# LordLiang/DrawingSpinUp

Measured on AMD Instinct MI355X. Metric: drawings/sec end-to-end (512x512, 6 views, 24 frames), higher is better.
Workload: dtype f16 (diffusion) / f16 table + f32 MLP (NSR) / f32 (stage-1 deformable convolutions, IS-Net, contour) / f32 with bf16 x 3 products (stage-2 convolutions; the reference: cuDNN TF32)

## Files before the change

### drawingspinup_amd/_lib.py

```python
import ctypes as C
import os

import torch

_HERE = os.path.dirname(os.path.abspath(__file__))
LIB_PATH = os.environ.get("DSU_HIP_LIB") or os.path.join(_HERE, "libdsu_hip.so")
MAX_LEVELS = 16
ABI_VERSION = 3

c_i32, c_i64, c_u32, c_f32, c_vp = C.c_int32, C.c_int64, C.c_uint32, C.c_float, C.c_void_p


class HashGridCfg(C.Structure):
    _fields_ = [("n_levels", c_u32), ("n_features", c_u32), ("log2_hashmap_size", c_u32),
                ("base_resolution", c_u32), ("per_level_scale", C.c_double)]


class HashGridLevels(C.Structure):
    _fields_ = [("offsets", c_u32 * (MAX_LEVELS + 1)), ("resolution", c_u32 * MAX_LEVELS),
                ("scale", c_f32 * MAX_LEVELS), ("hashed", c_u32 * MAX_LEVELS)]


class SdfMlp(C.Structure):
    _fields_ = [("w0", c_vp), ("b0", c_vp), ("w1", c_vp), ("b1", c_vp)]


class TexMlp(C.Structure):
    _fields_ = [("w0", c_vp), ("b0", c_vp), ("w1", c_vp), ("b1", c_vp), ("w2", c_vp),
                ("b2", c_vp)]


class PartialReduce(C.Structure):
    _fields_ = [("partials", c_vp), ("map", c_vp), ("base", c_vp), ("nblocks", c_i32),
                ("stride", c_i32), ("n", c_i32)]


class OccRefreshArgs(C.Structure):
    _fields_ = [("occs", c_vp), ("binary", c_vp), ("res", c_i32), ("all_cells", c_i32),
                ("aabb", C.POINTER(c_f32)), ("seed", C.c_uint64), ("step", c_i64),
                ("grid", C.POINTER(HashGridCfg)), ("table_img", c_vp), ("mlp", C.POINTER(SdfMlp)),
                ("inv_s", c_vp), ("radius", c_f32), ("render_step_size", c_f32),
                ("ema_decay", c_f32), ("occ_thre", c_f32), ("active_levels", c_u32),
                ("inj_count", c_i32), ("inj_cells", c_vp), ("inj_rand", c_vp), ("thre_out", c_vp),
                ("workspace", c_vp), ("workspace_bytes", c_i64), ("cells_out", c_vp),
                ("rand_out", c_vp)]


class RenderTexture(C.Structure):
    _fields_ = [("uv", c_vp), ("texels", c_vp), ("tex_size", c_i32), ("filter", c_i32)]


class NormCfg(C.Structure):
    _fields_ = [("batch", c_i32), ("channels", c_i32), ("hw", c_i32), ("instance", c_i32),
                ("act", c_i32), ("stat_updates", c_i32), ("eps", c_f32), ("momentum", c_f32)]


class RayLossCfg(C.Structure):
    _fields_ = [("rgb_p_ratio", C.c_double), ("normal_p_ratio", C.c_double),
                ("mask_p_ratio", C.c_double), ("lambda_rgb_mse", c_f32),
                ("lambda_rgb_l1", c_f32), ("lambda_normal", c_f32), ("lambda_mask", c_f32),
                ("geo_aware", c_i32), ("reserved", c_i32)]


P = c_vp
class AdamwTensor(C.Structure):
    _fields_ = [("p", C.c_void_p), ("g", C.c_void_p), ("m", C.c_void_p), ("v", C.c_void_p),
                ("n", C.c_int64), ("lr", C.c_float), ("bias_correction1", C.c_float),
                ("bias_correction2_sqrt", C.c_float), ("reserved", C.c_float)]


ADAMW_MAX_TENSORS = 24


class NsrDriverCfg(C.Structure):
    _fields_ = [("grid", HashGridCfg), ("radius", c_f32), ("render_step_size", c_f32),
                ("cap_points", c_i32), ("cap_rays", c_i32), ("n_random", c_i32),
                ("sort_bits", c_i32), ("dynamic_ray_sampling", c_i32),
                ("train_num_samples", c_i32),
                ("c2w", c_vp), ("origins", c_vp), ("directions", c_vp), ("images", c_vp),
                ("normals", c_vp), ("masks", c_vp), ("view_weights", c_vp),
                ("V", c_i32), ("H", c_i32), ("W", c_i32), ("image_channels", c_i32),
                ("w0_v", c_vp), ("w0_g", c_vp), ("b0", c_vp), ("w1_v", c_vp), ("w1_g", c_vp),
                ("b1", c_vp), ("tex", c_vp * 6), ("variance", c_vp),
                ("ray_loss", RayLossCfg),
                ("lambda_eikonal", c_f32), ("lambda_sparsity", c_f32), ("sparsity_scale", c_f32),
                ("lambda_smooth", c_f32),
                ("beta1", c_f32), ("beta2", c_f32), ("adam_eps", c_f32), ("weight_decay", c_f32),
                ("seed", C.c_uint64), ("workspace", c_vp), ("workspace_bytes", c_i64)]


class NsrStepArgs(C.Structure):
    _fields_ = [("step", c_i64), ("n_rays", c_i32), ("prefetch_next", c_i32),
                ("active_levels", c_u32), ("eps", c_f32), ("cos_anneal_ratio", c_f32),
                ("lr_geometry", c_f32), ("lr_texture", c_f32), ("lr_variance", c_f32),
                ("adam_step", c_i32), ("randomized", c_i32), ("refresh_effective", c_i32),
                ("occ_res", c_i32), ("occ_binary", c_vp), ("table_img", c_vp),
                ("table_grad", c_vp),
                ("inj_index", c_vp), ("inj_x", c_vp), ("inj_y", c_vp), ("inj_jitter", c_vp),
                ("inj_pts_random", c_vp), ("inj_perturb", c_vp),
                ("inj_rays", c_vp), ("inj_rgb", c_vp), ("inj_normal", c_vp), ("inj_mask", c_vp),
                ("inj_cosines", c_vp), ("inj_view_weights", c_vp),
                ("table_p", c_vp), ("table_m", c_vp), ("table_v", c_vp), ("table_n", c_i64),
                ("table_lr", c_f32), ("table_bc1", c_f32), ("table_bc2_sqrt", c_f32),
                ("table_eps", c_f32), ("table_wd", c_f32),
                ("out_n_samples", c_i32), ("out_max_count", c_i32), ("out_next_n_rays", c_i32),
                ("terms_out", c_vp)]


_PROTOS = {
    "dsu_abi_version": [],
    "dsu_hashgrid_make_levels": [C.POINTER(HashGridCfg), C.POINTER(HashGridLevels)],
    "dsu_hashgrid_encode_fwd": [C.POINTER(HashGridCfg), P, P, c_i64, c_u32, P, P],
    "dsu_hashgrid_encode_bwd": [C.POINTER(HashGridCfg), P, P, c_i64, c_u32, P, P],
    "dsu_sdf_fwd": [C.POINTER(HashGridCfg), P, C.POINTER(SdfMlp), P, c_i64, c_f32, c_u32, c_u32,
                    P, P],
    "dsu_sdf_fd_bwd_workspace_bytes": [C.POINTER(HashGridCfg), c_i64],
    "dsu_sdf_fd_enc_cache_bytes": [c_i64, c_u32],
    "dsu_sdf_fd_fwd_sorted": [C.POINTER(HashGridCfg), P, C.POINTER(SdfMlp), P, P, c_i64, c_f32,
                              c_f32, c_u32, P, P, P, P, P, P],
    "dsu_sdf_fd_bwd_sorted": [C.POINTER(HashGridCfg), P, C.POINTER(SdfMlp), P, P, c_i64, c_f32,
                              c_f32, c_u32, P, P, P, P, P, P, P, P, P, P, c_i64, P, P],
    "dsu_sdf_fd_bwd_sorted_fold": [C.POINTER(HashGridCfg), P, C.POINTER(SdfMlp), P, P, c_i64, c_f32,
                                   c_f32, c_u32, P, P, P, P, P, P, P, P, P, P, c_i64, P, P,
                                   C.POINTER(PartialReduce), P],
    "dsu_texture_partial_map": [P],
    "dsu_texture_bwd_shaded_partials_m": [C.POINTER(TexMlp), P, P, P, P, P, c_i64, c_i64, P, P, P, P, c_i64,
                                          C.POINTER(PartialReduce), P],
    "dsu_texture_bwd_shaded_partials_live": [C.POINTER(TexMlp), P, P, P, P, P, c_i64, c_i64, P, P, P, P, P,
                                             c_i64, C.POINTER(PartialReduce), P],
    "dsu_texture_live_partition": [P, c_i64, c_i32, c_i32, P],
    "dsu_texture_fwd_shaded_m": [C.POINTER(TexMlp), P, P, c_i64, P, P, P, P],
    "dsu_occgrid_refresh_workspace_bytes": [c_i32],
    "dsu_occgrid_refresh": [C.POINTER(OccRefreshArgs), P],
    "dsu_nsr_driver_occ_refresh": [P, C.POINTER(OccRefreshArgs), P],
    "dsu_inpaint_telea_u8c3": [P, P, c_i32, c_i32, c_i32, P],
    "dsu_table_adamw": [P, P, P, P, P, c_i64, c_f32, c_f32, c_f32, c_f32, c_f32, c_f32, c_f32, P],
    "dsu_table_decay": [P, P, c_i64, c_f32, P],
    "dsu_adamw_multi": [P, c_i32, c_f32, c_f32, c_f32, c_f32, P],
    "dsu_smooth_iterate": [P, c_i64, P, P, C.c_double, c_i32, P, P, P],
    "dsu_smooth_energy": [P, c_i64, P, P, P, P],
    "dsu_smooth_energy_partials": [],
    "dsu_smooth_brick_side": [],
    "dsu_smooth_bricks_flags": [P, c_i32, c_i32, c_i32, P, P],
    "dsu_smooth_bricks_gather": [P, P, c_i32, c_i32, c_i32, P, P, c_i32, P, c_i32, P, P, P, P, P, P, P],
    "dsu_smooth_bricks_iterate": [P, P, c_i32, P, P, P, c_i32, C.c_double, c_i32, c_i32, P, P, P],
    "dsu_smooth_bricks_energy": [P, P, c_i32, P, P, P],
    "dsu_smooth_bricks_scatter": [P, P, P, c_i32, c_i32, c_i32, c_i32, P, P],
    "dsu_set_onewave_grid_cap": [c_i32],
    "dsu_set_scatter_grid_cap": [c_i32],
    "dsu_set_nsr_side_stream_priority": [c_i32],
    "dsu_set_nsr_side_stream_pooling": [c_i32],
    "dsu_volume_band_distance_workspace_bytes": [c_i32, c_i32, c_i32],
    "dsu_volume_band_distance": [P, c_i32, c_i32, c_i32, c_i32, P, P, P, P, P, c_i64, P],
    "dsu_mc_cube_index": [P, c_i32, c_i32, c_i32, C.c_double, P, P],
    "dsu_sdf_fwd_lattice": [P, P, P, P, c_i32, c_i32, c_i32, P, P, c_f32, c_u32, P, P],
    "dsu_zgrid_count": [P, c_i64, c_f32, c_f32, c_f32, c_i32, P, P],
    "dsu_zgrid_fill": [P, c_i64, c_f32, c_f32, c_f32, c_i32, P, P, P, P],
    "dsu_zray_cast": [P, P, c_i64, c_f32, c_f32, c_f32, c_i32, P, P, P, c_i64, c_i32, P, P, P, P, P,
                      P, P],
    "dsu_raster_mask": [P, c_i64, c_f32, c_i32, P, P],
    "dsu_erode_ellipse_u8": [P, c_i32, c_i32, c_i32, P, P],
    "dsu_mesh_render_ortho_workspace_bytes": [c_i32, c_i32],
    "dsu_mesh_render_ortho": [c_i32, P, P, P, P, C.POINTER(RenderTexture), c_i32, c_i64, c_i64, C.c_double,
                              C.c_double, C.c_double, c_i32, c_i32, P, c_i64, P, c_i64, P, P, P, P, P, P, P],
    "dsu_mip_levels": [c_i32],
    "dsu_mip_pyramid_texels": [c_i32],
    "dsu_mip_workspace_bytes": [c_i32],
    "dsu_mip_pyramid_build": [P, P, c_i32, c_i32, P, P, c_i64, P],
    "dsu_mip_sample_host": [P, c_i32, P, P, P, c_i64, P],
    "dsu_pos_edge_u8": [P, c_i32, c_i32, c_i32, P, P],
    "dsu_uv_face_labels": [P, P, c_i64, c_i64, P, P, P, P],
    "dsu_uv_components": [P, P, c_i64, P, P, c_i32, c_i32, C.POINTER(c_i32), P],
    "dsu_uv_bake_workspace_bytes": [c_i32],
    "dsu_uv_bake": [c_i32, P, P, P, P, c_i64, c_i64, c_i32, P, c_i64, P, c_i64, P, P, P, P],
    "dsu_uv_dilate": [P, P, c_i32, P, P, P],
    "dsu_uv_project": [P, P, P, c_i64, c_i64, c_i32, P, P, c_f32, c_f32, c_f32, c_i32, P, P, P, P, P, P, c_i32,
                       C.c_double, P, P, P],
    "dsu_uv_field_points": [P, P, P, c_i64, c_i64, c_i32, P, P, c_i64, c_i32, P, P, P],
    "dsu_uv_field_resolve": [P, P, P, c_i64, c_i32, c_i32, P, P],
    "dsu_uv_field_points_host": [P, P, P, c_i64, c_i64, c_i32, P, P, c_i64, c_i32, P, P],
    "dsu_uv_field_resolve_host": [P, P, P, c_i64, c_i32, c_i32, P],
    "dsu_uv_seam_gather": [P, P, P, c_i64, c_i64, c_i64, c_i32, P, P, P, P, P, P, P],
    "dsu_uv_seam_apply": [P, P, P, c_i64, c_i64, c_i64, c_i32, P, P, P, P, P, P, P],
    "dsu_uv_seam_gather_host": [P, P, P, c_i64, c_i64, c_i64, c_i32, P, P, P, P, P, P],
    "dsu_uv_seam_apply_host": [P, P, P, c_i64, c_i64, c_i64, c_i32, P, P, P, P, P, P],
    "dsu_bone_visibility_workspace_bytes": [c_i32, c_i32, c_i32],
    "dsu_bone_visibility": [c_i32, P, P, P, c_i64, c_i64, c_i32, P, C.c_double, C.c_double, C.c_double,
                            C.c_double, c_i32, c_i32, c_i32, P, c_i64, P, c_i64, P, P, P],
    "dsu_spd_cg_block_workspace_bytes": [c_i64, c_i32],
    "dsu_spd_cg_block": [P, P, P, c_i64, c_i64, c_i32, P, P, C.c_double, c_i32, P, c_i64,
                         C.POINTER(c_i32), C.POINTER(C.c_double), P],
    "dsu_skin_lbs": [P, P, P, P, c_i64, c_i32, c_i32, c_i32, P, P],
    "dsu_skin_dqs": [P, P, P, P, c_i64, c_i32, c_i32, c_i32, P, P],
    "dsu_skin_dqs_host": [P, P, P, P, c_i64, c_i32, c_i32, c_i32, P],
    "dsu_corrective_smooth_workspace_bytes": [c_i64, c_i32],
    "dsu_corrective_bind": [P, P, P, c_i64, P, P, c_i64, P, c_i64, c_i64, C.c_double, c_i32, P, c_i64, P, P, P],
    "dsu_corrective_smooth": [P, P, P, P, c_i64, P, P, c_i64, P, c_i64, P, P, c_i64, c_i32, C.c_double, c_i32,
                              P, c_i64, P, P],
    "dsu_corrective_bind_host": [P, P, P, c_i64, P, P, c_i64, P, c_i64, c_i64, C.c_double, c_i32, P, c_i64, P, P],
    "dsu_corrective_smooth_host": [P, P, P, P, c_i64, P, P, c_i64, P, c_i64, P, P, c_i64, c_i32, C.c_double,
                                   c_i32, P, c_i64, P],
    "dsu_point_bin_count": [P, c_i64, c_f32, c_f32, c_f32, c_i32, P, P],
    "dsu_point_bin_fill": [P, c_i64, c_f32, c_f32, c_f32, c_i32, P, P, P, P],
    "dsu_knn8_blend": [P, c_i64, P, P, c_i64, c_f32, c_f32, c_f32, c_i32, P, P, P, P],
    "dsu_umbrella_implicit_solve": [P, P, c_i64, C.c_double, P, P, P, c_i32, P],
    "dsu_mesh_decimate_quadric": [P, c_i64, P, c_i64, c_i64, C.c_double, c_i32, P, P, P, P],
    "dsu_mesh_decimate_quadric_q": [P, c_i64, P, c_i64, c_i64, C.c_double, c_i32, P, P, P, P, P],
    "dsu_mesh_decimate_parallel_workspace_bytes": [c_i64, c_i64],
    "dsu_mesh_decimate_parallel": [P, c_i64, P, c_i64, c_i64, c_i64, C.c_double, c_i32, c_i32, P, P, P, P,
                                   c_i64, P],
    "dsu_distance_transform_l2_5x5": [P, c_i32, c_i32, P],
    "dsu_skeletonize_lee_2d": [P, c_i32, c_i32, P],
    "dsu_nsr_draws": [C.c_uint64, c_i64, c_i32, c_i32, c_i32, c_i32, P, P, P, P, c_i32, P, P, P],
    "dsu_nsr_driver_workspace_bytes": [C.POINTER(NsrDriverCfg)],
    "dsu_nsr_driver_create": [C.POINTER(NsrDriverCfg), C.POINTER(c_vp)],
    "dsu_nsr_driver_destroy": [c_vp],
    "dsu_nsr_driver_step": [c_vp, C.POINTER(NsrStepArgs), P],
    "dsu_nsr_driver_terms": [c_vp],
    "dsu_nsr_driver_adam_moments": [c_vp, c_i32],
    "dsu_nsr_driver_live_halves": [c_vp, c_i64],
    "dsu_nsr_driver_timing": [c_vp, c_i32],
    "dsu_nsr_driver_timing_read": [c_vp, c_i32, C.POINTER(c_i64), C.POINTER(C.c_double),
                                   C.POINTER(C.c_double)],
    "dsu_nsr_driver_timing_flops": [c_vp, c_i32, C.POINTER(C.c_double)],
    "dsu_spatial_sort": [P, c_i64, c_f32, c_i32, P, P, P, c_i64, P],
    "dsu_spatial_sort_workspace_bytes": [c_i64, c_i32],
    "dsu_ray_aabb": [P, P, c_i64, P, P, c_f32, P, P, P],
    "dsu_ray_march_scratch": [P, P, P, P, c_i64, P, P, c_i32, c_f32, c_i32, P, P, P, P],
    "dsu_ray_compact": [P, P, c_i32, P, P, c_i64, P, P, P, P],
    "dsu_ray_compact_points": [P, P, c_i32, P, P, c_i64, P, P, P, P, P, P],
    "dsu_ray_compact_points_cap": [P, P, c_i32, P, P, c_i64, P, P, P, P, P, c_i64, P],
    "dsu_points_tail": [P, c_i64, P, P, P, c_i64, c_f32, P],
    "dsu_spatial_sort_dev": [P, c_i64, P, c_i64, c_f32, c_i32, P, P, P, c_i64, P],
    "dsu_ray_offsets": [P, c_i64, P, P, P],
    "dsu_ortho_ray_batch": [P, P, P, c_i64, P, P, P, P, c_i32, P, P, P, c_i32, c_i32, P, P, P, P, P,
                            P, P],
    "dsu_ortho_ray_batch_split": [P, P, P, c_i64, P, P, P, P, c_i32, P, P, P, c_i32, c_i32, P, P, P, P, P,
                            P, P, P, P],
    "dsu_ray_losses": [P, P, P, P, P, P, c_i32, C.POINTER(RayLossCfg), P, P, P],
    "dsu_sample_losses": [P, P, c_i64, c_i64, c_f32, c_f32, c_f32, c_f32, c_i32, P, P, P, P],
    "dsu_texture_fwd": [C.POINTER(TexMlp), P, c_i64, P, P],
    "dsu_texture_bwd_workspace_bytes": [c_i64],
    "dsu_texture_bwd": [C.POINTER(TexMlp), P, P, P, c_i64, P, P, P, P, P, P, P, P, c_i64, P],
    "dsu_texture_bwd_shaded": [C.POINTER(TexMlp), P, P, P, P, P, c_i64, c_i64, P, P, P, P, P, P, P, P,
                               P, c_i64, P],
    "dsu_weights_from_alpha_fwd": [P, P, P, c_i64, P, P],
    "dsu_weights_from_alpha_bwd": [P, P, P, P, P, c_i64, P, P],
    "dsu_accumulate_fwd": [P, P, c_i32, P, P, c_i64, P, P],
    "dsu_neus_composite_fwd": [P, P, P, P, P, P, P, P, c_i64, P, c_f32, P, P, P, P],
    "dsu_neus_composite_bwd": [P, P, P, P, P, P, P, P, c_i64, P, c_f32, P, P, P, P, P, P, P,
                               P, P],
    "dsu_neus_composite_bwd_live": [P, P, P, P, P, P, P, P, c_i64, P, c_f32, P, P, P, P, P, P, P,
                                    P, P, P],
    "dsu_shade_prep_fwd": [P, P, c_i64, P, P, P],
    "dsu_shade_prep_bwd": [P, P, P, c_i64, P, P, P],
    "dsu_occgrid_ema": [P, P, P, c_i64, c_f32, P, P],
    "dsu_occgrid_binarize": [P, c_i64, c_f32, P, P],
    "dsu_ric_offsets": [c_i32, c_i32, P, P],
    "dsu_deform_conv3x3_fwd": [P, P, c_i64, P, c_i32, c_i32, c_i32, c_i32, c_i32, c_i32, P, P,
                               c_i32, P, P, P],
    "dsu_mv_attention_fwd": [P, P, P, P, P, c_i32, c_i32, c_i32, c_i32, c_i32, c_i32,
                             C.POINTER(c_i64), C.POINTER(c_i64), C.POINTER(c_i64),
                             C.POINTER(c_i64), c_f32, P],
    "dsu_conv2d_nhwc_f16_fwd_fx": [P, P, P, c_i32, c_i32, c_i32, c_i32, c_i32, c_i32, c_i32, c_i32,
                                   c_i32, P, P, P, c_i32, P, c_i64, P, c_i64, P],
    "dsu_gemm_f16_fwd_fx": [P, P, P, c_i64, c_i32, c_i32, P, P, c_i32, c_i32, P, c_i64, P, c_i64, P],
    "dsu_conv2d_nhwc_f16_split_k": [c_i32] * 9,
    "dsu_conv2d_nhwc_f16_workspace_bytes": [c_i32] * 9,
    "dsu_gemm_f16_split_k": [c_i64, c_i32, c_i32],
    "dsu_gemm_f16_workspace_bytes": [c_i64, c_i32, c_i32],
    "dsu_gemm_geglu_fwd": [P, P, P, c_i64, c_i32, c_i32, P, P],
    "dsu_groupnorm_nhwc_f16": [P, P, P, c_i32, c_i32, c_i32, c_i32, c_f32, c_i32, P, P, P],
    "dsu_layernorm_f16": [P, P, P, c_i64, c_i32, c_f32, P, P],
    "dsu_geglu_f16": [P, c_i64, c_i32, P, P],
    "dsu_cfg_model_input": [P, P, c_i32, c_i64, P, P],
    "dsu_ddim_cfg_step": [P, P, P, c_i64, c_f32, c_f32, c_f32, c_f32, c_f32, P, P],
    "dsu_deform_tap_table_bytes": [c_i32, c_i32],
    "dsu_deform_tap_table": [P, c_i32, c_i32, P, P],
    "dsu_conv2d_wgrad_workspace_bytes": [c_i32, c_i32, c_i32, c_i32, c_i32, c_i32, c_i32],
    "dsu_conv2d_wgrad": [P, P, P, c_i32, c_i32, c_i32, c_i32, c_i32, c_i32, c_i32, c_i32, P, P,
                         c_i32, P],
    "dsu_deform_conv3x3_dgrad_gather": [P, P, P, P, c_i64, c_i32, P, P],
    "dsu_norm_train_fwd": [C.POINTER(NormCfg), P, P, P, P, P, P, P, P, P],
    "dsu_norm_train_bwd": [C.POINTER(NormCfg), P, P, P, P, P, P, P, P, P, P],
    "dsu_channel_sum": [P, c_i32, c_i32, c_i32, P, P],
    "dsu_act_fwd": [P, P, c_i64, c_i32, P],
    "dsu_act_bwd": [P, P, P, c_i64, c_i32, P],
    "dsu_maxpool2_fwd": [P, P, c_i64, c_i32, c_i32, P],
    "dsu_maxpool2_bwd": [P, P, P, c_i64, c_i32, c_i32, P],
    "dsu_upsample2_fwd": [P, P, c_i64, c_i32, c_i32, P],
    "dsu_upsample2_bwd": [P, P, c_i64, c_i32, c_i32, P],
    "dsu_pair_loss": [P, P, c_f32, c_i64, c_i32, c_f32, P, P, P],
    "dsu_conv_x3_packed_elems": [c_i32, c_i32, c_i32],
    "dsu_conv_x3_pack_weights": [P, c_i32, c_i32, c_i32, P, P, P],
    "dsu_deform_conv3x3_fwd_x3": [P, P, c_i64, P, P, c_i32, c_i32, c_i32, c_i32, c_i32, c_i32,
                                  P, P, c_i32, P, P, P],
    "dsu_conv2d_fwd_x3": [P, P, P, P, c_i32, c_i32, c_i32, c_i32, c_i32, c_i32, c_i32, c_i32,
                          c_i32, P, P, c_i32, P, P, P],
    "dsu_conv_f32p_pack_weights": [P, c_i32, c_i32, c_i32, P, P],
    "dsu_deform_conv3x3_fwd_f32p": [P, P, c_i64, P, c_i32, c_i32, c_i32, c_i32, c_i32, c_i32,
                                    P, P, c_i32, P, P, P],
    "dsu_conv2d_fwd_f32p": [P, P, P, c_i32, c_i32, c_i32, c_i32, c_i32, c_i32, c_i32, c_i32, c_i32,
                            P, P, c_i32, P, P, P],
    "dsu_conv2d_fwd": [P, P, P, c_i32, c_i32, c_i32, c_i32, c_i32, c_i32, c_i32, c_i32, c_i32,
                       P, P, c_i32, P, P, P],
}

_RESTYPES = {"dsu_nsr_driver_destroy": None, "dsu_nsr_driver_terms": c_vp,
             "dsu_nsr_driver_adam_moments": c_vp, "dsu_nsr_driver_live_halves": c_vp,
             "dsu_conv_x3_packed_elems": C.c_int64, "dsu_mip_pyramid_texels": C.c_int64}

_lib = None


class DsuError(RuntimeError):
    pass


def lib():
    global _lib
    if _lib is None:
        if not os.path.exists(LIB_PATH):
            raise DsuError(
                f"{LIB_PATH} is missing: the HIP extension is not built "
                "(run `python -m drawingspinup_amd.build`). There is no CPU fallback.")
        h = C.CDLL(LIB_PATH)
        h.dsu_strerror.restype = C.c_char_p
        h.dsu_strerror.argtypes = [C.c_int]
        if h.dsu_abi_version() != ABI_VERSION:
            raise DsuError(f"{LIB_PATH} has ABI version {h.dsu_abi_version()}, this package binds version "
                           f"{ABI_VERSION}: rebuild it (`python -m drawingspinup_amd.build`).")
        for name, args in _PROTOS.items():
            fn = getattr(h, name)
            fn.restype = _RESTYPES.get(name, C.c_int64 if name.endswith("_bytes") else C.c_int)
            fn.argtypes = args
        _lib = h
# ... 40 lines not shown
```

### drawingspinup_amd/csrc/capi.hip

```cpp
#include "common.h"
#include <math.h>

int dsu_mv_cfg_model_input_launch(const void* latents, const void* image_latents, int32_t B,
                                  int64_t row_elems, void* out, void* stream);
int dsu_mv_ddim_cfg_step_launch(const void* noise_pred, const void* latents,
                                const void* variance_noise, int64_t n, float guidance_scale,
                                float sqrt_a_t, float sqrt_1m_a_t, float sqrt_a_prev, double dir,
                                float std_dev, void* out, void* stream);

extern "C" {

const char* dsu_strerror(int code) {
  switch (code) {
    case DSU_OK: return "ok";
    case DSU_EINVAL: return "invalid argument";
    case DSU_ELAUNCH: return "HIP launch/runtime error";
    case DSU_EUNSUP: return "configuration not supported by the gfx950 kernels";
    default: return "unknown dsu error";
  }
}

int dsu_abi_version(void) { return 3; }

int32_t dsu_onewave_grid_cap_value = 0;
int32_t dsu_scatter_grid_cap_value = 0;
int dsu_set_scatter_grid_cap(int32_t workgroups) {
  if (workgroups < 0 || workgroups > 4096) return DSU_EINVAL;
  dsu_scatter_grid_cap_value = workgroups;
  return DSU_OK;
}
int32_t dsu_nsr_side_priority_value = 1;
int dsu_set_nsr_side_stream_priority(int32_t level) {
  if (level < 0 || level > 2) return DSU_EINVAL;
  dsu_nsr_side_priority_value = level;
  return DSU_OK;
}
int32_t dsu_nsr_side_pool_value = 0;
int dsu_set_nsr_side_stream_pooling(int32_t on) {
  if (on < 0 || on > 1) return DSU_EINVAL;
  dsu_nsr_side_pool_value = on;
  return DSU_OK;
}
int dsu_set_onewave_grid_cap(int32_t cus) {
  if (cus < 0 || cus > 256) return DSU_EINVAL;
  dsu_onewave_grid_cap_value = cus;
  return DSU_OK;
}

int dsu_cfg_model_input(const void* latents, const void* image_latents, int32_t B,
                        int64_t row_elems, void* out, void* stream) {
  if (!latents || !image_latents || !out || B < 0 || row_elems < 0) return DSU_EINVAL;
  if (out == latents || out == image_latents) return DSU_EINVAL;
  if (B == 0 || row_elems == 0) return DSU_OK;
  if (row_elems > INT64_MAX / 4 / B) return DSU_EINVAL;
  return dsu_mv_cfg_model_input_launch(latents, image_latents, B, row_elems, out, stream);
}

int dsu_ddim_cfg_step(const void* noise_pred, const void* latents, const void* variance_noise,
                      int64_t n, float guidance_scale, float sqrt_a_t, float sqrt_1m_a_t,
                      float sqrt_a_prev, float std_dev, void* out, void* stream) {
  if (!noise_pred || !latents || !out || n < 0 || n > INT64_MAX / 2) return DSU_EINVAL;
  if (out == noise_pred || out == latents || out == variance_noise) return DSU_EINVAL;
  if (!(sqrt_a_t > 0.0f) || !(std_dev >= 0.0f) || !isfinite(guidance_scale) ||
      !isfinite(sqrt_1m_a_t) || !isfinite(sqrt_a_prev))
    return DSU_EINVAL;
  const double rad = 1.0 - (double)sqrt_a_prev * sqrt_a_prev - (double)std_dev * std_dev;
  if (!(rad >= -1e-6)) return DSU_EINVAL;
  if (n == 0) return DSU_OK;
  return dsu_mv_ddim_cfg_step_launch(noise_pred, latents, variance_noise, n, guidance_scale,
                                     sqrt_a_t, sqrt_1m_a_t, sqrt_a_prev,
                                     sqrt(rad > 0.0 ? rad : 0.0), std_dev, out, stream);
}

}
```

### drawingspinup_amd/csrc/nsr_driver.hip

```cpp
#include "common.h"
#include "adamw_dev.h"

#include <math.h>
#include <string.h>

#include <mutex>
#include <vector>

namespace {

constexpr int N_GEO = 64 * 23 + 64 + 13 * 64 + 13;
constexpr int N_TEX = 64 * 16 + 64 + 64 * 64 + 64 + 3 * 64 + 3;
constexpr int N_SMALL = (64 * 23 + 64 + 64) + (13 * 64 + 13 + 13) + N_TEX + 1;

__device__ __forceinline__ uint4 philox(uint4 c, uint2 k) {
#pragma unroll
  for (int i = 0; i < 10; ++i) {
    const uint32_t hi0 = __umulhi(0xD2511F53u, c.x), lo0 = 0xD2511F53u * c.x;
    const uint32_t hi1 = __umulhi(0xCD9E8D57u, c.z), lo1 = 0xCD9E8D57u * c.z;
    c = make_uint4(hi1 ^ c.y ^ k.x, lo1, hi0 ^ c.w ^ k.y, lo0);
    k.x += 0x9E3779B9u;
    k.y += 0xBB67AE85u;
  }
  return c;
// ... 583 lines not shown
    ~Guard() {
      if (!ok) for (int k = 0; k < 3; ++k) d->pf_valid[k] = false;
    }
  } guard{d};
  if (d->initialised && a->step != d->last_step + 1) {
    DSU_HIP(hipMemsetAsync(terms + 4, 0, 3 * sizeof(float), s));
    DSU_HIP(hipMemsetAsync(L.live_halves[a->step & 1], 0, (size_t)L.live_words * sizeof(uint32_t), s));
  }
  if (!d->initialised) {
    DSU_HIP(hipMemsetAsync(L.live_halves[0], 0, 2 * (size_t)L.live_words * sizeof(uint32_t), s));
    DSU_HIP(hipMemsetAsync(L.g_geo, 0, (N_GEO + N_TEX + 1) * sizeof(float), s));
    DSU_HIP(hipMemsetAsync(L.adam_m, 0, N_SMALL * sizeof(float), s));
    DSU_HIP(hipMemsetAsync(L.adam_v, 0, N_SMALL * sizeof(float), s));
    DSU_HIP(hipMemsetAsync(L.terms, 0, 16 * sizeof(float), s));
  }
  if (!d->initialised || a->refresh_effective) {
    DSU_TRY(launch_small_update(d, a, 0, s));
    d->initialised = true;
  }
  const bool injected = a->inj_index || a->inj_x || a->inj_y || a->inj_jitter || a->inj_pts_random ||
                        a->inj_perturb || a->inj_rays;
  if (d->pf_valid[p] && d->pf_step[p] == a->step && d->pf_rays[p] == a->n_rays && !injected &&
      d->pf_randomized[p] == a->randomized && d->pf_occ[p] == a->occ_binary &&
      d->pf_occ_res[p] == a->occ_res) {
    DSU_HIP(hipEventSynchronize(d->ready[p]));
  } else {
    DSU_HIP(hipStreamSynchronize(d->side));
    for (int k = 0; k < 3; ++k) d->pf_valid[k] = false;
    DSU_TRY(enqueue_samples(d, p, a->step, a->n_rays, *a, injected, s));
    DSU_HIP(hipStreamSynchronize(s));
  }
  d->pf_valid[p] = false;
  const int32_t total = d->host_stats[2 * p], cmax = d->host_stats[2 * p + 1];
  a->out_n_samples = total;
  a->out_max_count = cmax;
  if (total > c.cap_points || cmax > d->rowcap) return DSU_EUNSUP;
  const int64_t n_s = total, n_r = c.n_random, n_all = n_s + 2 * n_r;
  int32_t next_rays = a->n_rays;
  if (c.dynamic_ray_sampling && n_s > 0) {
    const int tr = (int)((double)a->n_rays * ((double)c.train_num_samples / (double)n_s));
    const int nr2 = (int)((double)a->n_rays * 0.9 + (double)tr * 0.1);
    next_rays = nr2 < c.cap_rays ? nr2 : c.cap_rays;
    if (next_rays < 1) next_rays = 1;
  }
  a->out_next_n_rays = next_rays;
  if (a->prefetch_next) {
    const int q = (int)((a->step + 1) % 3);
    DSU_HIP(hipStreamWaitEvent(d->side, d->gate, 0));
    dsu_nsr_step_args na = *a;
    na.inj_index = na.inj_x = na.inj_y = nullptr;
    na.inj_jitter = na.inj_pts_random = na.inj_perturb = nullptr;
    na.inj_rays = nullptr;
    DSU_TRY(enqueue_march(d, q, a->step + 1, next_rays, na, false, d->side));
    d->pf_step[q] = a->step + 1;
    d->pf_rays[q] = next_rays;
    d->pf_randomized[q] = a->randomized;
    d->pf_occ[q] = a->occ_binary;
    d->pf_occ_res[q] = a->occ_res;
    DSU_TRY(enqueue_pack(d, q, next_rays, na, false, d->side));
    DSU_HIP(hipEventRecord(d->ready[q], d->side));
    d->pf_valid[q] = true;
  }

  const float* pts = c.sort_bits ? f.sorted : f.points;
  const int32_t* perm = c.sort_bits ? f.perm : nullptr;
  dsu_sdf_mlp mlp{L.w0_eff, c.b0, L.w1_eff, c.b1};
  const double alg_bytes = (double)n_all * (7.0 * a->active_levels * 8 * 4 + 12 + 72);
  const double l0 = 7.0 * 64 * (3 + 2 * a->active_levels), l1 = 64.0 * (13 + 6);
  const double fwd_flops = (double)n_all * 2.0 * (l0 + l1), bwd_flops = (double)n_all * 2.0 * 3.0 * (l0 + l1);
  DSU_TRY(mark(d, 0, s));
  DSU_TRY(dsu_sdf_fd_fwd_sorted(&c.grid, a->table_img, &mlp, pts, perm, n_all, c.radius, a->eps,
                                a->active_levels, L.a_sdf, L.a_grad, L.a_feat, nullptr, L.enc_cache, s));
  DSU_TRY(mark(d, 0, s));
  if (d->timing) { d->work[0] += alg_bytes; d->flops[0] += fwd_flops; }
  if (n_s > 0) {
    dsu_tex_mlp tex{c.tex[0], c.tex[1], c.tex[2], c.tex[3], c.tex[4], c.tex[5]};
    DSU_TRY(dsu_texture_fwd_shaded_m(&tex, L.a_feat, L.a_grad, n_s, L.normal, L.rgb, L.tex_mask, s));
    DSU_TRY(dsu_neus_composite_fwd(L.a_sdf, L.normal, L.rgb, f.rays_d, f.t_starts, f.t_ends,
                                   f.offsets, f.counts, a->n_rays, L.inv_s, a->cos_anneal_ratio,
                                   L.alpha, L.w, L.comp, s));
  } else {
    DSU_HIP(hipMemsetAsync(L.comp, 0, (size_t)a->n_rays * 8 * sizeof(float), s));
  }
  DSU_TRY(dsu_ray_losses(L.comp, f.rgb, f.normal, f.mask, f.cosines, f.vw, a->n_rays, &c.ray_loss,
                         terms, L.d_comp, s));
  dsu_partial_reduce tex_red{};
  bool have_tex_red = false;
  if (n_s > 0) {
    uint32_t* live = L.live_halves[a->step & 1];
    DSU_TRY(dsu_neus_composite_bwd_live(L.a_sdf, L.normal, L.rgb, f.rays_d, f.t_starts, f.t_ends,
                                        f.offsets, f.counts, a->n_rays, L.inv_s, a->cos_anneal_ratio,
                                        L.alpha, L.w, L.d_comp, nullptr, L.d_sdf_all, L.d_normal, L.d_rgb,
                                        L.d_inv, live, s));
    dsu_tex_mlp tex{c.tex[0], c.tex[1], c.tex[2], c.tex[3], c.tex[4], c.tex[5]};
    DSU_TRY(dsu_texture_bwd_shaded_partials_live(&tex, L.a_feat, L.a_grad, L.rgb, L.d_rgb, L.d_normal, n_s,
                                                 2 * n_r, L.d_grad_all, L.d_feat_all, L.tex_mask, live,
                                                 L.tex_ws, L.tex_ws_bytes, &tex_red, s));
    tex_red.map = L.tex_map;
    tex_red.base = L.g_tex;
    have_tex_red = true;
  } else {
    DSU_HIP(hipMemsetAsync(L.d_feat_all, 0, (size_t)(2 * n_r) * 13 * sizeof(float), s));
  }
  DSU_TRY(dsu_sample_losses(L.a_sdf, L.a_grad, n_s, n_r, c.lambda_eikonal, c.lambda_sparsity,
                            c.sparsity_scale, c.lambda_smooth, 1 | 2, L.d_sdf_all, L.d_grad_all,
                            terms + 4, s));
  float* gg = L.g_geo;
  DSU_TRY(mark(d, 1, s));
  DSU_TRY(dsu_sdf_fd_bwd_sorted_fold(&c.grid, a->table_img, &mlp, pts, perm, n_all, c.radius, a->eps,
                                     a->active_levels, L.d_sdf_all, L.d_grad_all, L.d_feat_all, nullptr,
                                     a->table_grad, gg, gg + 64 * 23, gg + 64 * 23 + 64,
                                     gg + 64 * 23 + 64 + 13 * 64, L.sdf_ws, L.sdf_ws_bytes,
                                     L.enc_cache, d->gate, have_tex_red ? &tex_red : nullptr, s));
  DSU_TRY(mark(d, 1, s));
  if (d->timing) { d->work[1] += alg_bytes; d->flops[1] += bwd_flops; }
  DSU_TRY(launch_small_update(d, a, 1, s));
  d->last_step = a->step;
  guard.ok = true;
  return DSU_OK;
}

int dsu_nsr_driver_occ_refresh(dsu_nsr_driver* d, const dsu_occgrid_refresh_args* args,
                               void* main_stream) {
  if (!d || !args) return DSU_EINVAL;
  if (!d->initialised) return DSU_EUNSUP;
  const dsu_nsr_driver_cfg& c = d->cfg;
  DSU_HIP(hipStreamSynchronize(d->side));
  for (int k = 0; k < 3; ++k) d->pf_valid[k] = false;
  dsu_occgrid_refresh_args a = *args;
  const dsu_sdf_mlp mlp{d->L.w0_eff, c.b0, d->L.w1_eff, c.b1};
  a.grid = &c.grid;
  a.mlp = &mlp;
  a.inv_s = d->L.inv_s;
  a.aabb = d->aabb;
  a.seed = c.seed;
  a.radius = c.radius;
  a.render_step_size = c.render_step_size;
  return dsu_occgrid_refresh(&a, main_stream);
}

int dsu_nsr_driver_timing(dsu_nsr_driver* d, int32_t enable) {
  if (!d) return DSU_EINVAL;
  for (int f = 0; f < 2; ++f) {
    for (hipEvent_t e : d->ev[f]) (void)hipEventDestroy(e);
    d->ev[f].clear();
    d->work[f] = 0.0;
    d->flops[f] = 0.0;
  }
  d->timing_stride = enable > 0 ? enable : 0;
  d->timing = false;
  return DSU_OK;
}

int dsu_nsr_driver_timing_read(dsu_nsr_driver* d, int32_t family, int64_t* launches,
                               double* total_ms, double* alg_bytes) {
  if (!d || family < 0 || family > 1 || !launches || !total_ms || !alg_bytes) return DSU_EINVAL;
  const std::vector<hipEvent_t>& ev = d->ev[family];
  double ms = 0.0;
  const size_t pairs = ev.size() / 2;
  for (size_t i = 0; i < pairs; ++i) {
    DSU_HIP(hipEventSynchronize(ev[2 * i + 1]));
    float t = 0.0f;
    DSU_HIP(hipEventElapsedTime(&t, ev[2 * i], ev[2 * i + 1]));
    ms += t;
  }
  *launches = (int64_t)pairs;
  *total_ms = ms;
  *alg_bytes = d->work[family];
  return DSU_OK;
}

int dsu_nsr_driver_timing_flops(dsu_nsr_driver* d, int32_t family, double* mlp_flops) {
  if (!d || family < 0 || family > 1 || !mlp_flops) return DSU_EINVAL;
  *mlp_flops = d->flops[family];
  return DSU_OK;
}

}
```

### drawingspinup_amd/csrc/nsr_render.hip

```cpp
#include "common.h"
#include <math.h>
#include <stdlib.h>

namespace {

struct Aabb {
  float mn[3];
  float mx[3];
  float inv_ext[3];
  int pow2;
};

template <bool P2>
__device__ __forceinline__ float div_ext(float x, const Aabb& a, int d) {
  return P2 ? x * a.inv_ext[d] : x / (a.mx[d] - a.mn[d]);
}
template <bool P2>
__device__ __forceinline__ float div_res(float x, const Aabb& a, int res, float inv_res) {
  return P2 ? x * inv_res : x / (float)res;
}

__device__ __forceinline__ float signf1(float x) { return copysignf(1.0f, x); }

template <bool P2>
// ... 326 lines not shown
  return v;
}
__device__ __forceinline__ float wave_sum(float v) {
#pragma unroll
  for (int o = 32; o > 0; o >>= 1) v += __shfl_xor(v, o);
  return v;
}
__device__ __forceinline__ float sigmoidf_(float x) { return 1.0f / (1.0f + expf(-x)); }

struct AlphaOut {
  float alpha, pc, nc, iter_cos, true_cos;
  bool clipped;
};

__device__ __forceinline__ AlphaOut neus_alpha(float sdf, const float n[3], const float d[3],
                                               float dist, float inv_s, float car) {
  AlphaOut a;
  a.true_cos = d[0] * n[0] + d[1] * n[1] + d[2] * n[2];
  a.iter_cos = -(fmaxf(-a.true_cos * 0.5f + 0.5f, 0.0f) * (1.0f - car) +
                 fmaxf(-a.true_cos, 0.0f) * car);
  const float nx = sdf + a.iter_cos * dist * 0.5f, pv = sdf - a.iter_cos * dist * 0.5f;
  a.pc = sigmoidf_(pv * inv_s);
  a.nc = sigmoidf_(nx * inv_s);
  const float raw = ((a.pc - a.nc) + 1e-5f) / (a.pc + 1e-5f);
  a.clipped = raw < 0.0f || raw > 1.0f;
  a.alpha = fminf(fmaxf(raw, 0.0f), 1.0f);
  return a;
}

__global__ __launch_bounds__(256) void composite_fwd_kernel(
    const float* __restrict__ sdf, const float* __restrict__ normal,
    const float* __restrict__ rgb, const float* __restrict__ rays_d,
    const float* __restrict__ t_starts, const float* __restrict__ t_ends,
    const int32_t* __restrict__ off, const int32_t* __restrict__ cnt, int64_t n_rays,
    const float* __restrict__ inv_s_p, float car, float* __restrict__ alpha_o,
    float* __restrict__ w_o, float* __restrict__ comp) {
  const float inv_s = fminf(fmaxf(*inv_s_p, 1e-6f), 1e6f);
  const int lane = threadIdx.x & 63;
  const int64_t r = blockIdx.x * 4 + (threadIdx.x >> 6);
  if (r >= n_rays) return;
  const int64_t b = off[r];
  const int c = cnt[r];
  const float d[3] = {rays_d[r * 3], rays_d[r * 3 + 1], rays_d[r * 3 + 2]};
  float T = 1.0f;
  float acc[8];
#pragma unroll
  for (int k = 0; k < 8; ++k) acc[k] = 0.0f;
  for (int j0 = 0; j0 < c; j0 += 64) {
    const int j = j0 + lane;
    const bool v = j < c;
    float al = 0.0f, mid = 0.0f, n[3] = {0.f, 0.f, 0.f}, col[3] = {0.f, 0.f, 0.f};
    if (v) {
      const int64_t i = b + j;
      n[0] = normal[i * 3]; n[1] = normal[i * 3 + 1]; n[2] = normal[i * 3 + 2];
      const float ts = t_starts[i], te = t_ends[i];
      mid = (ts + te) / 2.0f;
      al = neus_alpha(sdf[i], n, d, te - ts, inv_s, car).alpha;
      col[0] = rgb[i * 3]; col[1] = rgb[i * 3 + 1]; col[2] = rgb[i * 3 + 2];
    }
    const float incl = wave_incl_scan_mul(1.0f - al, lane);
    float excl = __shfl_up(incl, 1);
    if (lane == 0) excl = 1.0f;
    const float w = al * (T * excl);
    T *= __shfl(incl, 63);
    if (v) {
      alpha_o[b + j] = al;
      w_o[b + j] = w;
      acc[0] += w;
      acc[1] += w * mid;
      acc[2] += w * col[0]; acc[3] += w * col[1]; acc[4] += w * col[2];
      acc[5] += w * n[0]; acc[6] += w * n[1]; acc[7] += w * n[2];
    }
  }
#pragma unroll
  for (int k = 0; k < 8; ++k) acc[k] = wave_sum(acc[k]);
  if (lane < 8) {
    float v = acc[0];
#pragma unroll
    for (int k = 1; k < 8; ++k) v = lane == k ? acc[k] : v;
    comp[r * 8 + lane] = v;
  }
}

__global__ __launch_bounds__(256) void composite_bwd_kernel(
    const float* __restrict__ sdf, const float* __restrict__ normal,
    const float* __restrict__ rgb, const float* __restrict__ rays_d,
    const float* __restrict__ t_starts, const float* __restrict__ t_ends,
    const int32_t* __restrict__ off, const int32_t* __restrict__ cnt, int64_t n_rays,
    const float* __restrict__ inv_s_p, float car, const float* __restrict__ alpha_s,
    const float* __restrict__ w_s,
    const float* __restrict__ d_comp, const float* __restrict__ d_w_extra,
    float* __restrict__ d_sdf, float* __restrict__ d_normal, float* __restrict__ d_rgb,
    float* __restrict__ d_inv_s, uint32_t* __restrict__ live_halves) {
  const float inv_raw = *inv_s_p;
  const float inv_s = fminf(fmaxf(inv_raw, 1e-6f), 1e6f);
  const bool inv_pass = inv_raw >= 1e-6f && inv_raw <= 1e6f;
  const int lane = threadIdx.x & 63;
  const int64_t r = blockIdx.x * 4 + (threadIdx.x >> 6);
  float dinv = 0.0f;
  if (r < n_rays) {
    const int64_t b = off[r];
    const int c = cnt[r];
    const float d[3] = {rays_d[r * 3], rays_d[r * 3 + 1], rays_d[r * 3 + 2]};
    float dc[8];
#pragma unroll
    for (int k = 0; k < 8; ++k) dc[k] = d_comp[r * 8 + k];
    float total = 0.0f;
    for (int j = lane; j < c; j += 64) {
      const int64_t i = b + j;
      const float mid = (t_starts[i] + t_ends[i]) / 2.0f;
      float gw = dc[0] + dc[1] * mid + dc[2] * rgb[i * 3] + dc[3] * rgb[i * 3 + 1] +
                 dc[4] * rgb[i * 3 + 2] + dc[5] * normal[i * 3] + dc[6] * normal[i * 3 + 1] +
                 dc[7] * normal[i * 3 + 2];
      if (d_w_extra) gw += d_w_extra[i];
      total += gw * w_s[i];
    }
    total = wave_sum(total);
    float T = 1.0f, done = 0.0f;
    for (int j0 = 0; j0 < c; j0 += 64) {
      const int j = j0 + lane;
      const bool v = j < c;
      float al = 0.0f, w = 0.0f, gw = 0.0f, n[3] = {0.f, 0.f, 0.f};
      int64_t i = b + (v ? j : 0);
      float mid = 0.0f, dist = 0.0f, s = 0.0f;
      if (v) {
        al = alpha_s[i]; w = w_s[i];
        n[0] = normal[i * 3]; n[1] = normal[i * 3 + 1]; n[2] = normal[i * 3 + 2];
        const float ts = t_starts[i], te = t_ends[i];
        mid = (ts + te) / 2.0f; dist = te - ts; s = sdf[i];
        gw = dc[0] + dc[1] * mid + dc[2] * rgb[i * 3] + dc[3] * rgb[i * 3 + 1] +
             dc[4] * rgb[i * 3 + 2] + dc[5] * n[0] + dc[6] * n[1] + dc[7] * n[2];
        if (d_w_extra) gw += d_w_extra[i];
      }
      const float incl = wave_incl_scan_mul(1.0f - al, lane);
      float excl = __shfl_up(incl, 1);
      if (lane == 0) excl = 1.0f;
      const float Tj = T * excl;
      const float gww = gw * w;
      const float pin = wave_incl_scan_add(gww, lane);
      const float before = done + (pin - gww);
      T *= __shfl(incl, 63);
      done += __shfl(pin, 63);
      bool lit = false;
      if (v) {
        const float accum = total - before;
        const float galpha = (gw * Tj - accum) / fmaxf(1.0f - al, 1e-10f);
        const AlphaOut a = neus_alpha(s, n, d, dist, inv_s, car);
        float dsdf = 0.0f, dn[3] = {0.f, 0.f, 0.f};
        if (!a.clipped) {
          const float den = a.pc + 1e-5f;
          const float d_pc = galpha * (1.0f / den - ((a.pc - a.nc) + 1e-5f) / (den * den));
          const float d_nc = -galpha / den;
          const float d_pv = d_pc * a.pc * (1.0f - a.pc);
          const float d_nx = d_nc * a.nc * (1.0f - a.nc);
          const float pv = s - a.iter_cos * dist * 0.5f, nx = s + a.iter_cos * dist * 0.5f;
          dinv += d_pv * pv + d_nx * nx;
          dsdf = (d_pv + d_nx) * inv_s;
          const float d_ic = (d_nx - d_pv) * inv_s * dist * 0.5f;
          float d_tc = 0.0f;
          if (-a.true_cos * 0.5f + 0.5f > 0.0f) d_tc += 0.5f * (1.0f - car);
          if (-a.true_cos > 0.0f) d_tc += car;
          d_tc *= d_ic;
          dn[0] = d_tc * d[0]; dn[1] = d_tc * d[1]; dn[2] = d_tc * d[2];
        }
        d_sdf[i] = dsdf;
        d_normal[i * 3] = dn[0] + w * dc[5];
        d_normal[i * 3 + 1] = dn[1] + w * dc[6];
        d_normal[i * 3 + 2] = dn[2] + w * dc[7];
        const float c0 = w * dc[2], c1 = w * dc[3], c2 = w * dc[4];
        d_rgb[i * 3] = c0; d_rgb[i * 3 + 1] = c1; d_rgb[i * 3 + 2] = c2;
        lit = c0 != 0.0f || c1 != 0.0f || c2 != 0.0f;
      }
      if (live_halves) {
        const uint64_t m = __ballot(lit);
        if (v && (lane == 0 || (i & 31) == 0)) {
          const int span = 32 - (int)(i & 31);
          const uint64_t part = span >= 64 - lane ? ~0ull << lane : ((1ull << span) - 1ull) << lane;
          if (m & part) atomicOr(&live_halves[i >> 10], 1u << ((i >> 5) & 31));
        }
      }
    }
  }
  dinv = wave_sum(dinv);
  if (lane == 0 && dinv != 0.0f && inv_pass) unsafeAtomicAdd(d_inv_s, dinv);
}

__global__ void shade_prep_fwd_kernel(const float* __restrict__ grad,
                                      const float* __restrict__ feat, int64_t n,
                                      float* __restrict__ normal, float* __restrict__ tex_in) {
  const int64_t i = blockIdx.x * (int64_t)blockDim.x + threadIdx.x;
  if (i >= n) return;
  const float g0 = grad[i * 3], g1 = grad[i * 3 + 1], g2 = grad[i * 3 + 2];
  const float inv = 1.0f / fmaxf(sqrtf(g0 * g0 + g1 * g1 + g2 * g2), 1e-12f);
  const float n0 = g0 * inv, n1 = g1 * inv, n2 = g2 * inv;
  normal[i * 3] = n0; normal[i * 3 + 1] = n1; normal[i * 3 + 2] = n2;
#pragma unroll
  for (int k = 0; k < 13; ++k) tex_in[i * 16 + k] = feat[i * 13 + k];
  tex_in[i * 16 + 13] = n0; tex_in[i * 16 + 14] = n1; tex_in[i * 16 + 15] = n2;
}

__global__ void shade_prep_bwd_kernel(const float* __restrict__ grad,
                                      const float* __restrict__ d_normal,
                                      const float* __restrict__ d_tex_in, int64_t n,
                                      int64_t tail, float* __restrict__ d_grad,
                                      float* __restrict__ d_feat) {
  const int64_t i = blockIdx.x * (int64_t)blockDim.x + threadIdx.x;
  if (i >= n) {
    if (i < n + tail)
      for (int k = 0; k < 13; ++k) d_feat[i * 13 + k] = 0.0f;
    return;
  }
  const float g0 = grad[i * 3], g1 = grad[i * 3 + 1], g2 = grad[i * 3 + 2];
  const float len = sqrtf(g0 * g0 + g1 * g1 + g2 * g2);
  const float inv = 1.0f / fmaxf(len, 1e-12f);
  const float n0 = g0 * inv, n1 = g1 * inv, n2 = g2 * inv;
  float d0 = d_tex_in[i * 16 + 13], d1 = d_tex_in[i * 16 + 14], d2 = d_tex_in[i * 16 + 15];
  if (d_normal) { d0 += d_normal[i * 3]; d1 += d_normal[i * 3 + 1]; d2 += d_normal[i * 3 + 2]; }
  const float dot = n0 * d0 + n1 * d1 + n2 * d2;
  const bool ok = len > 1e-12f;
  d_grad[i * 3] = ok ? (d0 - n0 * dot) * inv : d0 * inv;
  d_grad[i * 3 + 1] = ok ? (d1 - n1 * dot) * inv : d1 * inv;
  d_grad[i * 3 + 2] = ok ? (d2 - n2 * dot) * inv : d2 * inv;
#pragma unroll
  for (int k = 0; k < 13; ++k) d_feat[i * 13 + k] = d_tex_in[i * 16 + k];
}

Aabb make_aabb(const float* a6, int res = 1) {
  Aabb a;
  a.pow2 = (res > 0 && (res & (res - 1)) == 0) ? 1 : 0;
  for (int d = 0; d < 3; ++d) {
    a.mn[d] = a6[d];
    a.mx[d] = a6[3 + d];
    const float ext = a.mx[d] - a.mn[d];
    a.inv_ext[d] = 1.0f / ext;
    if (!is_pow2f(ext)) a.pow2 = 0;
  }
  return a;
}

}

#define DSU_MARCH_ONE(O, P, nr, st, ...)                                                    \
  ray_march_kernel<O, P><<<dsu_blocks_for(nr, 256 / MARCH_G), 256, 0,                       \
                           (hipStream_t)st>>>(__VA_ARGS__)
#define DSU_LAUNCH_MARCH(nr, st, box, occp, ...)                                      \
  do {                                                                                \
    const bool p2_ = (box).pow2 != 0;                                                 \
    if (!(occp)) {                                                                    \
// ... 80 lines not shown
  if (n_rays < 0 || (n_rays && (!offsets || !counts))) return DSU_EINVAL;
  if (n_rays == 0) return DSU_OK;
  weights_fwd_kernel<<<dsu_blocks_for(n_rays, 64), 64, 0, (hipStream_t)stream>>>(
      alpha, offsets, counts, n_rays, weights);
  DSU_CHECK_LAUNCH();
  return DSU_OK;
}

int dsu_weights_from_alpha_bwd(const float* alpha, const float* weights, const float* d_weights,
                               const int32_t* offsets, const int32_t* counts, int64_t n_rays,
                               float* d_alpha, void* stream) {
  if (n_rays < 0 || (n_rays && (!offsets || !counts))) return DSU_EINVAL;
  if (n_rays == 0) return DSU_OK;
  weights_bwd_kernel<<<dsu_blocks_for(n_rays, 64), 64, 0, (hipStream_t)stream>>>(
      alpha, weights, d_weights, offsets, counts, n_rays, d_alpha);
  DSU_CHECK_LAUNCH();
  return DSU_OK;
}

int dsu_accumulate_fwd(const float* weights, const float* values, int32_t channels,
                       const int32_t* offsets, const int32_t* counts, int64_t n_rays,
                       float* out, void* stream) {
  if (n_rays < 0 || channels <= 0 || (n_rays && (!offsets || !counts || !out)))
    return DSU_EINVAL;
  if (n_rays == 0) return DSU_OK;
  accumulate_fwd_kernel<<<dsu_blocks_for(n_rays * channels, 64), 64, 0, (hipStream_t)stream>>>(
      weights, values, channels, offsets, counts, n_rays, out);
  DSU_CHECK_LAUNCH();
  return DSU_OK;
}

int dsu_occgrid_ema(float* occs, const int64_t* idx, const float* occ, int64_t n, float decay,
                    float* scratch, void* stream) {
  if (n < 0 || (n && (!occs || !occ)) || (n && idx && !scratch)) return DSU_EINVAL;
  if (n == 0) return DSU_OK;
  hipStream_t s = (hipStream_t)stream;
  const int blocks = dsu_capped_blocks(n, 256);
  if (!idx) {
    occ_ema_kernel<<<blocks, 256, 0, s>>>(occs, occ, n, decay);
  } else {
    occ_ema_candidates_kernel<<<blocks, 256, 0, s>>>(occs, idx, occ, n, decay, scratch);
    occ_ema_clear_kernel<<<blocks, 256, 0, s>>>(occs, idx, n);
    occ_ema_max_kernel<<<blocks, 256, 0, s>>>(occs, idx, scratch, n);
  }
  DSU_CHECK_LAUNCH();
  return DSU_OK;
}

int dsu_occgrid_binarize(const float* occs, int64_t n_cells, float thre, uint8_t* binary,
                         void* stream) {
  if (n_cells < 0 || (n_cells && (!occs || !binary))) return DSU_EINVAL;
  if (n_cells == 0) return DSU_OK;
  occ_bin_kernel<<<dsu_capped_blocks(n_cells, 256), 256, 0, (hipStream_t)stream>>>(
      occs, n_cells, thre, binary);
  DSU_CHECK_LAUNCH();
  return DSU_OK;
}

int dsu_neus_composite_fwd(const float* sdf, const float* normal, const float* rgb,
                           const float* rays_d, const float* t_starts, const float* t_ends,
                           const int32_t* offsets, const int32_t* counts, int64_t n_rays,
                           const float* inv_s, float cos_anneal_ratio, float* alpha,
                           float* weights, float* comp, void* stream) {
  if (n_rays < 0 || !inv_s || (n_rays && (!rays_d || !offsets || !counts || !comp)))
    return DSU_EINVAL;
  if (n_rays == 0) return DSU_OK;
  composite_fwd_kernel<<<(unsigned)((n_rays + 3) / 4), 256, 0, (hipStream_t)stream>>>(
      sdf, normal, rgb, rays_d, t_starts, t_ends, offsets, counts, n_rays, inv_s,
      cos_anneal_ratio, alpha, weights, comp);
  DSU_CHECK_LAUNCH();
  return DSU_OK;
}

int dsu_neus_composite_bwd(const float* sdf, const float* normal, const float* rgb,
                           const float* rays_d, const float* t_starts, const float* t_ends,
                           const int32_t* offsets, const int32_t* counts, int64_t n_rays,
                           const float* inv_s, float cos_anneal_ratio, const float* alpha,
                           const float* weights, const float* d_comp, const float* d_weights,
                           float* d_sdf, float* d_normal, float* d_rgb, float* d_inv_s,
                           void* stream) {
  if (n_rays < 0 || !inv_s || (n_rays && (!rays_d || !offsets || !counts || !d_comp || !d_inv_s)))
    return DSU_EINVAL;
  if (n_rays == 0) return DSU_OK;
  composite_bwd_kernel<<<(unsigned)((n_rays + 3) / 4), 256, 0, (hipStream_t)stream>>>(
      sdf, normal, rgb, rays_d, t_starts, t_ends, offsets, counts, n_rays, inv_s,
      cos_anneal_ratio, alpha, weights, d_comp, d_weights, d_sdf, d_normal, d_rgb, d_inv_s, nullptr);
  DSU_CHECK_LAUNCH();
  return DSU_OK;
}

int dsu_neus_composite_bwd_live(const float* sdf, const float* normal, const float* rgb,
                                const float* rays_d, const float* t_starts, const float* t_ends,
                                const int32_t* offsets, const int32_t* counts, int64_t n_rays,
                                const float* inv_s, float cos_anneal_ratio, const float* alpha,
                                const float* weights, const float* d_comp, const float* d_weights,
                                float* d_sdf, float* d_normal, float* d_rgb, float* d_inv_s,
                                uint32_t* live_halves, void* stream) {
  if (n_rays < 0 || !inv_s || !live_halves ||
      (n_rays && (!rays_d || !offsets || !counts || !d_comp || !d_inv_s)))
    return DSU_EINVAL;
  if (n_rays == 0) return DSU_OK;
  composite_bwd_kernel<<<(unsigned)((n_rays + 3) / 4), 256, 0, (hipStream_t)stream>>>(
      sdf, normal, rgb, rays_d, t_starts, t_ends, offsets, counts, n_rays, inv_s,
      cos_anneal_ratio, alpha, weights, d_comp, d_weights, d_sdf, d_normal, d_rgb, d_inv_s,
      live_halves);
  DSU_CHECK_LAUNCH();
  return DSU_OK;
}

int dsu_shade_prep_fwd(const float* grad, const float* feature, int64_t n, float* normal,
                       float* tex_in, void* stream) {
  if (n < 0 || (n && (!grad || !feature || !normal || !tex_in))) return DSU_EINVAL;
  if (n == 0) return DSU_OK;
  shade_prep_fwd_kernel<<<dsu_blocks_for(n, 256), 256, 0, (hipStream_t)stream>>>(grad, feature, n,
                                                                               normal, tex_in);
  DSU_CHECK_LAUNCH();
  return DSU_OK;
}

int dsu_shade_prep_bwd(const float* grad, const float* d_normal, const float* d_tex_in, int64_t n,
                       float* d_grad, float* d_feature, void* stream) {
  if (n < 0 || (n && (!grad || !d_tex_in || !d_grad || !d_feature))) return DSU_EINVAL;
  if (n == 0) return DSU_OK;
  shade_prep_bwd_kernel<<<dsu_blocks_for(n, 256), 256, 0, (hipStream_t)stream>>>(
      grad, d_normal, d_tex_in, n,  0, d_grad, d_feature);
  DSU_CHECK_LAUNCH();
  return DSU_OK;
}

}
```

### drawingspinup_amd/csrc/nsr_step.hip

```cpp
#include "common.h"
#include "adamw_dev.h"
#include <math.h>

namespace {

constexpr int RL_THREADS = 1024;

__device__ __forceinline__ uint32_t flipf(float f) {
  const uint32_t u = __float_as_uint(f);
  return (u & 0x80000000u) ? ~u : (u | 0x80000000u);
}
__device__ __forceinline__ float unflipf(uint32_t k) {
  return __uint_as_float((k & 0x80000000u) ? (k & 0x7fffffffu) : ~k);
}

__device__ __forceinline__ float wave_sum(float v) {
#pragma unroll
  for (int o = 32; o > 0; o >>= 1) v += __shfl_xor(v, o);
  return v;
}
__device__ __forceinline__ int wave_sum_i(int v) {
#pragma unroll
  for (int o = 32; o > 0; o >>= 1) v += __shfl_xor(v, o);
  return v;
}

__device__ __forceinline__ float block_sum(float v, float* red) {
  const int lane = threadIdx.x & 63, wave = threadIdx.x >> 6, nw = blockDim.x >> 6;
  v = wave_sum(v);
  __syncthreads();
  if (lane == 0) red[wave] = v;
  __syncthreads();
  float t = 0.0f;
  for (int w = 0; w < nw; ++w) t += red[w];
  return t;
}

__device__ __forceinline__ int block_excl_scan(int v, int* red, int* total) {
  const int lane = threadIdx.x & 63, wave = threadIdx.x >> 6, nw = blockDim.x >> 6;
  int inc = v;
#pragma unroll
  for (int o = 1; o < 64; o <<= 1) {
    const int t = __shfl_up(inc, o);
    if (lane >= o) inc += t;
  }
  __syncthreads();
  if (lane == 63) red[wave] = inc;
  __syncthreads();
  int before = 0, all = 0;
  for (int w = 0; w < nw; ++w) {
    const int t = red[w];
    if (w < wave) before += t;
    all += t;
  }
  *total = all;
  return before + inc - v;
}

__device__ void bitonic_sort(uint64_t* keys, int P) {
  for (int k = 2; k <= P; k <<= 1) {
    for (int j = k >> 1; j > 0; j >>= 1) {
      for (int t = threadIdx.x; t < (P >> 1); t += blockDim.x) {
        const int i = ((t & ~(j - 1)) << 1) | (t & (j - 1));
        const int l = i | j;
        const uint64_t a = keys[i], b = keys[l];
        const bool up = (i & k) == 0;
        if ((a > b) == up) {
          keys[i] = b;
          keys[l] = a;
        }
      }
      __syncthreads();
    }
  }
}

struct RankLds {
  uint64_t* keys;
  int* pos;
  float* gerr;
  float* redf;
  int* redi;
};

template <class ErrF>
__device__ float rank_select(ErrF errf, const float* __restrict__ vw, int R, int P, double ratio,
                             bool mean, const RankLds& lds, int64_t* k_out) {
  for (int i = threadIdx.x; i < P; i += blockDim.x) {
    float e = 0.0f;
    bool valid = false;
    if (i < R) errf(i, e, valid);
    lds.keys[i] = ((uint64_t)flipf(valid ? e : INFINITY) << 32) | (uint32_t)i;
    lds.pos[i] = valid ? 1 : 0;
    lds.gerr[i] = 0.0f;
  }
  __syncthreads();
  const int E = P / blockDim.x;
  int c = 0;
  for (int q = 0; q < E; ++q) c += lds.pos[threadIdx.x * E + q];
  int nvalid;
  int run = block_excl_scan(c, lds.redi, &nvalid);
  for (int q = 0; q < E; ++q) {
    const int i = threadIdx.x * E + q;
    run += lds.pos[i];
    lds.pos[i] = run - 1;
  }
  __syncthreads();
  bitonic_sort(lds.keys, P);
  const int64_t kk = (int64_t)floor(ratio * (double)nvalid);
  float total = 0.0f;
  for (int64_t j = threadIdx.x; j < kk; j += blockDim.x) {
    const uint32_t idx = (uint32_t)lds.keys[j];
    int pj = lds.pos[idx];
    pj = pj < 0 ? 0 : pj;
    const uint64_t kt = lds.keys[pj];
    const float val = unflipf((uint32_t)(kt >> 32));
    const float w = vw ? vw[idx] : 1.0f;
    total += val * w;
    atomicAdd(&lds.gerr[(uint32_t)kt], w);
  }
  total = block_sum(total, lds.redf);
  *k_out = kk;
  return mean ? total / (float)kk : total;
}

__device__ __forceinline__ float signf0(float x) { return x > 0.0f ? 1.0f : (x < 0.0f ? -1.0f : 0.0f); }

__global__ __launch_bounds__(RL_THREADS) void ray_losses_kernel(
    const float* __restrict__ comp, const float* __restrict__ rgb, const float* __restrict__ normal,
    const float* __restrict__ maskf, const float* __restrict__ cosines,
    const float* __restrict__ vw, int R, int P, dsu_ray_loss_cfg cfg, float* __restrict__ terms,
    float* __restrict__ d_comp) {
  extern __shared__ __attribute__((aligned(16))) unsigned char smem[];
  RankLds lds;
  lds.keys = reinterpret_cast<uint64_t*>(smem);
  lds.pos = reinterpret_cast<int*>(smem + (size_t)P * 8);
  lds.gerr = reinterpret_cast<float*>(smem + (size_t)P * 12);
  lds.redf = reinterpret_cast<float*>(smem + (size_t)P * 16);
  lds.redi = reinterpret_cast<int*>(smem + (size_t)P * 16 + 128);
  const int term = blockIdx.x;

  auto fg = [&](int i) {
    const float cb = cosines[i] > -0.1f ? 0.0f : cosines[i];
    return maskf[i] > 0.0f && cb < -0.1f;
  };

  if (term == 0) {
    auto mse = [&](int i, float& e, bool& valid) {
      const float d0 = comp[i * 8 + 2] - rgb[i * 3], d1 = comp[i * 8 + 3] - rgb[i * 3 + 1],
                  d2 = comp[i * 8 + 4] - rgb[i * 3 + 2];
      e = (d0 * d0 + d1 * d1) + d2 * d2;
      valid = fg(i);
    };
    int64_t kk;
    float t = rank_select(mse, nullptr, R, P, cfg.rgb_p_ratio, true, lds, &kk) * cfg.lambda_rgb_mse;
    if (threadIdx.x == 0) terms[0] = t;
    __syncthreads();
    const float c = kk > 0 ? cfg.lambda_rgb_mse / (float)kk : 0.0f;
    for (int i = threadIdx.x; i < R; i += blockDim.x) {
      const float g = lds.gerr[i] * c;
#pragma unroll
      for (int ch = 0; ch < 3; ++ch)
        d_comp[i * 8 + 2 + ch] = 2.0f * (comp[i * 8 + 2 + ch] - rgb[i * 3 + ch]) * g;
    }
    float t1 = 0.0f;
    if (cfg.lambda_rgb_l1 != 0.0f) {
      __syncthreads();
      auto l1 = [&](int i, float& e, bool& valid) {
        const float d0 = comp[i * 8 + 2] - rgb[i * 3], d1 = comp[i * 8 + 3] - rgb[i * 3 + 1],
                    d2 = comp[i * 8 + 4] - rgb[i * 3 + 2];
        e = (fabsf(d0) + fabsf(d1)) + fabsf(d2);
        valid = fg(i);
      };
      t1 = rank_select(l1, nullptr, R, P, cfg.rgb_p_ratio, true, lds, &kk) * cfg.lambda_rgb_l1;
      __syncthreads();
      const float c1 = kk > 0 ? cfg.lambda_rgb_l1 / (float)kk : 0.0f;
      for (int i = threadIdx.x; i < R; i += blockDim.x) {
        const float g = lds.gerr[i] * c1;
#pragma unroll
        for (int ch = 0; ch < 3; ++ch)
          d_comp[i * 8 + 2 + ch] += signf0(comp[i * 8 + 2 + ch] - rgb[i * 3 + ch]) * g;
      }
    }
    if (threadIdx.x == 0) terms[1] = t1;
  } else if (term == 1) {
    float S = 1.0f;
    if (cfg.geo_aware) {
      float s = 0.0f;
      for (int i = threadIdx.x; i < R; i += blockDim.x) {
        const float cb = cosines[i] > -0.1f ? 0.0f : cosines[i];
        s += expf(fabsf(cb));
      }
      S = block_sum(s, lds.redf);
      __syncthreads();
    }
    auto cosim = [&](int i, float& cs, float u[3], float gh[3], float& nn, float& a, float n[3]) {
      const float v0 = comp[i * 8 + 5], v1 = comp[i * 8 + 6], v2 = comp[i * 8 + 7];
      const float nv = sqrtf((v0 * v0 + v1 * v1) + v2 * v2);
      a = fmaxf(nv, 1e-12f);
      n[0] = v0 / a; n[1] = v1 / a; n[2] = v2 / a;
      nn = fmaxf(sqrtf((n[0] * n[0] + n[1] * n[1]) + n[2] * n[2]), 1e-8f);
      const float g0 = normal[i * 3], g1 = normal[i * 3 + 1], g2 = normal[i * 3 + 2];
      const float gn = fmaxf(sqrtf((g0 * g0 + g1 * g1) + g2 * g2), 1e-8f);
      u[0] = n[0] / nn; u[1] = n[1] / nn; u[2] = n[2] / nn;
      gh[0] = g0 / gn; gh[1] = g1 / gn; gh[2] = g2 / gn;
      cs = (u[0] * gh[0] + u[1] * gh[1]) + u[2] * gh[2];
    };
    auto nerr = [&](int i, float& e, bool& valid) {
      float cs, u[3], gh[3], nn, a, n[3];
      cosim(i, cs, u, gh, nn, a, n);
      e = 1.0f - cs;
      if (cfg.geo_aware) {
        const float cb = cosines[i] > -0.1f ? 0.0f : cosines[i];
        e = e * expf(fabsf(cb)) / S;
      }
      valid = fg(i);
    };
    int64_t kk;
    const bool mean = !cfg.geo_aware;
    float t = rank_select(nerr, vw, R, P, cfg.normal_p_ratio, mean, lds, &kk) * cfg.lambda_normal;
    if (threadIdx.x == 0) terms[2] = t;
    __syncthreads();
    const float c = mean ? (kk > 0 ? cfg.lambda_normal / (float)kk : 0.0f) : cfg.lambda_normal;
    for (int i = threadIdx.x; i < R; i += blockDim.x) {
      float cs, u[3], gh[3], nn, a, n[3];
      cosim(i, cs, u, gh, nn, a, n);
      float de = lds.gerr[i] * c;
      if (cfg.geo_aware) {
        const float cb = cosines[i] > -0.1f ? 0.0f : cosines[i];
        de = de / S * expf(fabsf(cb));
      }
      const float dcs = -de;
      const float nv = sqrtf((comp[i * 8 + 5] * comp[i * 8 + 5] + comp[i * 8 + 6] * comp[i * 8 + 6]) +
                             comp[i * 8 + 7] * comp[i * 8 + 7]);
      float dv[3] = {0.0f, 0.0f, 0.0f};
      if (nv > 1e-12f && dcs != 0.0f) {
        float tn[3];
#pragma unroll
        for (int ch = 0; ch < 3; ++ch) tn[ch] = (gh[ch] - cs * u[ch]) / nn * dcs;
        const float nt = (n[0] * tn[0] + n[1] * tn[1]) + n[2] * tn[2];
#pragma unroll
        for (int ch = 0; ch < 3; ++ch) dv[ch] = (tn[ch] - n[ch] * nt) / a;
      }
      d_comp[i * 8 + 5] = dv[0];
      d_comp[i * 8 + 6] = dv[1];
      d_comp[i * 8 + 7] = dv[2];
    }
  } else {
    auto bce = [&](int i, float& e, bool& valid) {
      const float oc = fminf(fmaxf(comp[i * 8], 1e-3f), 1.0f - 1e-3f);
      const float m = maskf[i];
      e = -(m * logf(oc) + (1.0f - m) * logf(1.0f - oc));
      valid = true;
    };
    int64_t kk;
    float t = rank_select(bce, vw, R, P, cfg.mask_p_ratio, true, lds, &kk) * cfg.lambda_mask;
    if (threadIdx.x == 0) terms[3] = t;
    __syncthreads();
    const float c = kk > 0 ? cfg.lambda_mask / (float)kk : 0.0f;
    for (int i = threadIdx.x; i < R; i += blockDim.x) {
      const float o = comp[i * 8];
      const float oc = fminf(fmaxf(o, 1e-3f), 1.0f - 1e-3f);
      const float m = maskf[i];
      const bool pass = o >= 1e-3f && o <= 1.0f - 1e-3f;
      const float g = lds.gerr[i] * c;
      d_comp[i * 8] = pass ? g * (-(m / oc) + (1.0f - m) / (1.0f - oc)) : 0.0f;
      d_comp[i * 8 + 1] = 0.0f;
    }
  }
}

__global__ __launch_bounds__(256) void sample_losses_kernel(
    const float* __restrict__ sdf, const float* __restrict__ grad, int64_t n_s, int64_t n_r,
    float lambda_eik, float lambda_sp, float sp_scale, float lambda_sm, int accumulate_prefix,
    float* __restrict__ d_sdf, float* __restrict__ d_grad, float* __restrict__ terms) {
  float s_eik = 0.0f, s_sp = 0.0f, s_sm = 0.0f;
  const int64_t n = n_s + n_r;
  const float inv_ns = n_s > 0 ? 1.0f / (float)n_s : 0.0f;
  const float inv_nr = n_r > 0 ? 1.0f / (float)n_r : 0.0f;
  const float inv_3nr = n_r > 0 ? 1.0f / (float)(3 * n_r) : 0.0f;
  for (int64_t i = blockIdx.x * (int64_t)blockDim.x + threadIdx.x; i < n;
       i += (int64_t)gridDim.x * blockDim.x) {
    if (i < n_s) {
      const float g0 = grad[i * 3], g1 = grad[i * 3 + 1], g2 = grad[i * 3 + 2];
      const float nrm = sqrtf((g0 * g0 + g1 * g1) + g2 * g2);
      const float dl = nrm - 1.0f;
      s_eik += dl * dl;
      const float cf = nrm > 0.0f ? lambda_eik * 2.0f * dl * inv_ns / nrm : 0.0f;
      if (accumulate_prefix) {
        d_grad[i * 3] += cf * g0;
        d_grad[i * 3 + 1] += cf * g1;
        d_grad[i * 3 + 2] += cf * g2;
      } else {
        d_grad[i * 3] = cf * g0;
        d_grad[i * 3 + 1] = cf * g1;
        d_grad[i * 3 + 2] = cf * g2;
        d_sdf[i] = 0.0f;
      }
    } else {
      const int64_t a = i, b = i + n_r;
      const float x = sdf[a];
      const float ex = expf(-sp_scale * fabsf(x));
      s_sp += ex;
      d_sdf[a] = lambda_sp * inv_nr * ex * (-sp_scale) * signf0(x);
      d_sdf[b] = 0.0f;
#pragma unroll
      for (int c = 0; c < 3; ++c) {
        const float df = grad[a * 3 + c] - grad[b * 3 + c];
        s_sm += fabsf(df);
        const float sg = lambda_sm * inv_3nr * signf0(df);
        d_grad[a * 3 + c] = sg;
        d_grad[b * 3 + c] = -sg;
      }
    }
  }
  __shared__ float red[3][4];
  s_eik = wave_sum(s_eik);
  s_sp = wave_sum(s_sp);
  s_sm = wave_sum(s_sm);
  const int lane = threadIdx.x & 63, wave = threadIdx.x >> 6;
  if (lane == 0) {
    red[0][wave] = s_eik;
    red[1][wave] = s_sp;
    red[2][wave] = s_sm;
  }
  __syncthreads();
  if (threadIdx.x < 3) {
    const float t = (red[threadIdx.x][0] + red[threadIdx.x][1]) +
                    (red[threadIdx.x][2] + red[threadIdx.x][3]);
    const float sc = threadIdx.x == 0 ? inv_ns * lambda_eik
                                      : (threadIdx.x == 1 ? inv_nr * lambda_sp : inv_3nr * lambda_sm);
    if (t != 0.0f) atomicAdd(&terms[threadIdx.x], t * sc);
  }
}

__global__ __launch_bounds__(1024) void ray_offsets_kernel(const int32_t* __restrict__ counts,
                                                           int64_t n, int32_t* __restrict__ offsets,
                                                           int32_t* __restrict__ stats) {
  __shared__ int red[32];
  constexpr int PER = 8;
  int carry = 0, mx = 0;
  for (int64_t base = 0; base < n; base += (int64_t)blockDim.x * PER) {
    const int64_t i0 = base + (int64_t)threadIdx.x * PER;
    int c[PER], tsum = 0;
#pragma unroll
    for (int k = 0; k < PER; ++k) {
      c[k] = i0 + k < n ? counts[i0 + k] : 0;
      mx = max(mx, c[k]);
      tsum += c[k];
    }
    int total;
    int ex = carry + block_excl_scan(tsum, red, &total);
#pragma unroll
    for (int k = 0; k < PER; ++k) {
      if (i0 + k < n) offsets[i0 + k] = ex;
      ex += c[k];
    }
    carry += total;
  }
#pragma unroll
  for (int o = 32; o > 0; o >>= 1) mx = max(mx, __shfl_xor(mx, o));
  __syncthreads();
  if ((threadIdx.x & 63) == 0) red[threadIdx.x >> 6] = mx;
  __syncthreads();
  if (threadIdx.x == 0) {
    int m = 0;
    for (int w = 0; w < (int)(blockDim.x >> 6); ++w) m = max(m, red[w]);
    stats[0] = carry;
    stats[1] = m;
  }
}

__global__ __launch_bounds__(256) void ortho_ray_batch_kernel(
    const int64_t* __restrict__ index, const int64_t* __restrict__ px, const int64_t* __restrict__ py,
    int64_t n, const float* __restrict__ c2w , const float* __restrict__ origins,
    const float* __restrict__ directions, const float* __restrict__ images, int img_c,
    const float* __restrict__ normals, const float* __restrict__ masks,
    const float* __restrict__ vweights, int H, int W, float* __restrict__ rays ,
    float* __restrict__ rgb, float* __restrict__ normal, float* __restrict__ mask,
    float* __restrict__ cosines, float* __restrict__ vw, float* __restrict__ rays_o ,
    float* __restrict__ rays_d) {
  const int64_t i = blockIdx.x * (int64_t)blockDim.x + threadIdx.x;
  if (i >= n) return;
  const int64_t v = index[i];
  const int64_t pix = (v * H + py[i]) * W + px[i];
  const float* M = c2w + v * 12;
  const float o0 = origins[pix * 3], o1 = origins[pix * 3 + 1], o2 = origins[pix * 3 + 2];
  const float d0 = directions[pix * 3], d1 = directions[pix * 3 + 1], d2 = directions[pix * 3 + 2];
  float ro[3], rd[3];
#pragma unroll
  for (int r = 0; r < 3; ++r) {
    rd[r] = (M[r * 4] * d0 + M[r * 4 + 1] * d1) + M[r * 4 + 2] * d2;
    ro[r] = M[r * 4 + 3] + ((M[r * 4] * o0 + M[r * 4 + 1] * o1) + M[r * 4 + 2] * o2);
  }
  const float nx = normals[pix * 3], ny = normals[pix * 3 + 1], nz = normals[pix * 3 + 2];
  const float dn = sqrtf((rd[0] * rd[0] + rd[1] * rd[1]) + rd[2] * rd[2]);
  const float nn = sqrtf((nx * nx + ny * ny) + nz * nz);
  const float da = fmaxf(dn, 1e-6f), na = fmaxf(nn, 1e-6f);
  cosines[i] = ((rd[0] / da) * (nx / na) + (rd[1] / da) * (ny / na)) + (rd[2] / da) * (nz / na);
  const float dz = fmaxf(dn, 1e-12f);
  rays[i * 6 + 0] = ro[0]; rays[i * 6 + 1] = ro[1]; rays[i * 6 + 2] = ro[2];
  rays[i * 6 + 3] = rd[0] / dz; rays[i * 6 + 4] = rd[1] / dz; rays[i * 6 + 5] = rd[2] / dz;
  if (rays_o) {
    rays_o[i * 3] = ro[0]; rays_o[i * 3 + 1] = ro[1]; rays_o[i * 3 + 2] = ro[2];
    rays_d[i * 3] = rd[0] / dz; rays_d[i * 3 + 1] = rd[1] / dz; rays_d[i * 3 + 2] = rd[2] / dz;
  }
  for (int c = 0; c < img_c; ++c) rgb[i * img_c + c] = images[pix * img_c + c];
  normal[i * 3] = nx; normal[i * 3 + 1] = ny; normal[i * 3 + 2] = nz;
  mask[i] = masks[pix];
  vw[i] = vweights[pix];
}


__global__ __launch_bounds__(256) void table_adamw_kernel(dsu_table_adamw_args a) {
  dsu_table_adamw_range(a, blockIdx.x * (int64_t)blockDim.x + threadIdx.x,
// ... 48 lines not shown
      dsu_table_adamw_args{(float4*)p, (float4*)g, (float4*)m, (float4*)v, (__half2*)img_f16, n / 4,
                           lr, beta1, beta2, eps, weight_decay, bias_correction1,
                           bias_correction2_sqrt});
  DSU_CHECK_LAUNCH();
  return DSU_OK;
}

int dsu_adamw_multi(const dsu_adamw_tensor* tensors, int32_t count, float beta1, float beta2,
                    float eps, float weight_decay, void* stream) {
  if (count < 0 || count > DSU_ADAMW_MAX_TENSORS || (count && !tensors)) return DSU_EINVAL;
  if (count == 0) return DSU_OK;
  AdamwMultiArgs a;
  int64_t nmax = 0;
  for (int i = 0; i < count; ++i) {
    const dsu_adamw_tensor& t = tensors[i];
    if (t.n < 0 || (t.n && (!t.p || !t.g || !t.m || !t.v))) return DSU_EINVAL;
    if (!(t.bias_correction1 > 0.0f) || !(t.bias_correction2_sqrt > 0.0f)) return DSU_EINVAL;
    a.t[i] = t;
    if (t.n > nmax) nmax = t.n;
  }
  a.beta1 = beta1; a.beta2 = beta2; a.eps = eps; a.wd = weight_decay;
  if (nmax == 0) return DSU_OK;
  adamw_multi_kernel<<<dim3(dsu_capped_blocks(nmax, 256, 64), count), 256, 0, (hipStream_t)stream>>>(a);
  DSU_CHECK_LAUNCH();
  return DSU_OK;
}

int dsu_table_decay(float* p, void* img_f16, int64_t n, float factor, void* stream) {
  if (n < 0 || (n & 3) || (n && (!p || !img_f16))) return DSU_EINVAL;
  if (n == 0) return DSU_OK;
  table_decay_kernel<<<dsu_capped_blocks(n / 4, 256, 2048), 256, 0, (hipStream_t)stream>>>(
      (float4*)p, (__half2*)img_f16, n / 4, factor);
  DSU_CHECK_LAUNCH();
  return DSU_OK;
}

int dsu_ortho_ray_batch(const int64_t* index, const int64_t* x, const int64_t* y, int64_t n,
                        const float* c2w, const float* origins, const float* directions,
                        const float* images, int32_t image_channels, const float* normals,
                        const float* masks, const float* view_weights, int32_t H, int32_t W,
                        float* rays, float* rgb, float* normal, float* mask, float* cosines,
                        float* vw, void* stream) {
  return dsu_ortho_ray_batch_split(index, x, y, n, c2w, origins, directions, images, image_channels,
                                   normals, masks, view_weights, H, W, rays, rgb, normal, mask,
                                   cosines, vw, nullptr, nullptr, stream);
}

int dsu_ortho_ray_batch_split(const int64_t* index, const int64_t* x, const int64_t* y, int64_t n,
                              const float* c2w, const float* origins, const float* directions,
                              const float* images, int32_t image_channels, const float* normals,
                              const float* masks, const float* view_weights, int32_t H, int32_t W,
                              float* rays, float* rgb, float* normal, float* mask, float* cosines,
                              float* vw, float* rays_o, float* rays_d, void* stream) {
  if (n < 0 || H <= 0 || W <= 0 || image_channels <= 0) return DSU_EINVAL;
  if ((rays_o == nullptr) != (rays_d == nullptr)) return DSU_EINVAL;
  if (n == 0) return DSU_OK;
  if (!index || !x || !y || !c2w || !origins || !directions || !images || !normals || !masks ||
      !view_weights || !rays || !rgb || !normal || !mask || !cosines || !vw)
    return DSU_EINVAL;
  ortho_ray_batch_kernel<<<dsu_blocks_for(n, 256), 256, 0, (hipStream_t)stream>>>(
      index, x, y, n, c2w, origins, directions, images, image_channels, normals, masks, view_weights,
      H, W, rays, rgb, normal, mask, cosines, vw, rays_o, rays_d);
  DSU_CHECK_LAUNCH();
  return DSU_OK;
}

int dsu_ray_losses(const float* comp, const float* rgb, const float* normal, const float* mask,
                   const float* cosines, const float* view_weights, int32_t n_rays,
                   const dsu_ray_loss_cfg* cfg, float* terms, float* d_comp, void* stream) {
  if (!cfg || !terms || n_rays < 0) return DSU_EINVAL;
  if (n_rays && (!comp || !rgb || !normal || !mask || !cosines || !view_weights || !d_comp))
    return DSU_EINVAL;
  if (n_rays > DSU_RAY_LOSS_MAX_RAYS) return DSU_EUNSUP;
  int P = RL_THREADS;
  while (P < n_rays) P <<= 1;
  const size_t shm = (size_t)P * 16 + 256;
  DSU_ENSURE_DYN_LDS(ray_losses_kernel, shm);
  ray_losses_kernel<<<3, RL_THREADS, shm, (hipStream_t)stream>>>(
      comp, rgb, normal, mask, cosines, view_weights, n_rays, P, *cfg, terms, d_comp);
  DSU_CHECK_LAUNCH();
  return DSU_OK;
}

int dsu_sample_losses(const float* sdf_all, const float* grad_all, int64_t n_samples,
                      int64_t n_random, float lambda_eikonal, float lambda_sparsity,
                      float sparsity_scale, float lambda_smooth, int32_t accumulate_prefix,
                      float* d_sdf_all, float* d_grad_all, float* terms, void* stream) {
  if (n_samples < 0 || n_random < 0 || !terms) return DSU_EINVAL;
  const int64_t n = n_samples + n_random;
  if (n && (!sdf_all || !grad_all || !d_sdf_all || !d_grad_all)) return DSU_EINVAL;
  hipStream_t s = (hipStream_t)stream;
  if (!(accumulate_prefix & 2) && hipMemsetAsync(terms, 0, 3 * sizeof(float), s) != hipSuccess)
    return DSU_ELAUNCH;
  if (n == 0) return DSU_OK;
  sample_losses_kernel<<<dsu_capped_blocks(n, 256, 512), 256, 0, s>>>(
      sdf_all, grad_all, n_samples, n_random, lambda_eikonal, lambda_sparsity, sparsity_scale,
      lambda_smooth, accumulate_prefix & 1, d_sdf_all, d_grad_all, terms);
  DSU_CHECK_LAUNCH();
  return DSU_OK;
}

int dsu_ray_offsets(const int32_t* counts, int64_t n_rays, int32_t* offsets, int32_t* stats,
                    void* stream) {
  if (n_rays < 0 || !stats || (n_rays && (!counts || !offsets))) return DSU_EINVAL;
  ray_offsets_kernel<<<1, 1024, 0, (hipStream_t)stream>>>(counts, n_rays, offsets, stats);
  DSU_CHECK_LAUNCH();
  return DSU_OK;
}

}
```

### drawingspinup_amd/csrc/texture_mlp.hip

```cpp
#include <vector>
#include "common.h"
#include "tr_stage.h"
#include "tex_partition.h"

namespace {

typedef float f32x16 __attribute__((ext_vector_type(16)));
typedef __bf16 bf16x8 __attribute__((ext_vector_type(8)));

__device__ __forceinline__ void bf16_split8(const float* x, bf16x8& hi, bf16x8& mid) {
#pragma unroll
  for (int i = 0; i < 8; ++i) {
    const __bf16 hh = (__bf16)x[i];
    hi[i] = hh;
    mid[i] = (__bf16)(x[i] - (float)hh);
  }
}

constexpr int TIN = 16, THID = 64, TOUT = 3;
constexpr int W1_ROW = 65;
constexpr int W0_ROW = 17;
constexpr int L_W1 = 0;
constexpr int L_W0 = L_W1 + THID * W1_ROW;
constexpr int L_W2P = L_W0 + THID * W0_ROW;
// ... 230 lines not shown
    if (valid) {
#pragma unroll
      for (int o = 0; o < TOUT; ++o) rgb[i * TOUT + o] = sigmoidf(out[o] + lds[L_B2 + o]);
    }
  }
}

__device__ __forceinline__ void stage_units_T(uint32_t st, const f32x16 (&X)[2]) {
#pragma unroll
  for (int T = 0; T < 2; ++T)
#pragma unroll
    for (int g = 0; g < 4; ++g) {
      trs::bf16x4 hi, mid;
#pragma unroll
      for (int c = 0; c < 4; ++c) {
        const float x = X[T][4 * g + c];
        const __bf16 hh = (__bf16)x;
        hi[c] = hh;
        mid[c] = (__bf16)(x - (float)hh);
      }
      trs::store_slot(st, 8 * T + 2 * g, 0, hi);
      trs::store_slot(st, 8 * T + 2 * g, ImgU::PART_B, mid);
    }
}
__device__ __forceinline__ void stage_cols_S(uint32_t st, int s, float v0, float v1, float v2, float v3) {
  const float v[4] = {v0, v1, v2, v3};
  trs::bf16x4 hi, mid;
#pragma unroll
  for (int c = 0; c < 4; ++c) {
    const __bf16 hh = (__bf16)v[c];
    hi[c] = hh;
    mid[c] = (__bf16)(v[c] - (float)hh);
  }
  trs::store_slot(st, s, 0, hi);
  trs::store_slot(st, s, ImgS::PART_B, mid);
}
template <int NJ>
__device__ __forceinline__ void gemm_samples_T(f32x16 (&acc0)[NJ], f32x16 (&acc1)[NJ], uint32_t rdA,
                                               uint32_t rdB, int cols_b, int l31) {
  constexpr int CB = 32 * NJ;
  bf16x8 z;
#pragma unroll
  for (int e = 0; e < 8; ++e) z[e] = (__bf16)0.0f;
#pragma unroll
  for (int ks = 0; ks < 2; ++ks) {
    bf16x8 ah[2], am[2], bh[NJ], bm[NJ];
#pragma unroll
    for (int Ti = 0; Ti < 2; ++Ti) {
      ah[Ti] = trs::frag_tr<64>(rdA, ks, Ti);
      am[Ti] = trs::frag_tr<64>(rdA, ks, Ti, ImgU::PART_B);
    }
#pragma unroll
    for (int Tj = 0; Tj < NJ; ++Tj) {
      const bool real = 32 * Tj + l31 < cols_b;
      const bf16x8 vh = trs::frag_tr<CB>(rdB, ks, Tj), vm = trs::frag_tr<CB>(rdB, ks, Tj, trs::Img<CB>::PART_B);
      bh[Tj] = real ? vh : z;
      bm[Tj] = real ? vm : z;
    }
#pragma unroll
    for (int Tj = 0; Tj < NJ; ++Tj) {
      acc0[Tj] = __builtin_amdgcn_mfma_f32_32x32x16_bf16(ah[0], bh[Tj], acc0[Tj], 0, 0, 0);
      acc1[Tj] = __builtin_amdgcn_mfma_f32_32x32x16_bf16(ah[1], bh[Tj], acc1[Tj], 0, 0, 0);
      acc0[Tj] = __builtin_amdgcn_mfma_f32_32x32x16_bf16(ah[0], bm[Tj], acc0[Tj], 0, 0, 0);
      acc1[Tj] = __builtin_amdgcn_mfma_f32_32x32x16_bf16(ah[1], bm[Tj], acc1[Tj], 0, 0, 0);
      acc0[Tj] = __builtin_amdgcn_mfma_f32_32x32x16_bf16(am[0], bh[Tj], acc0[Tj], 0, 0, 0);
      acc1[Tj] = __builtin_amdgcn_mfma_f32_32x32x16_bf16(am[1], bh[Tj], acc1[Tj], 0, 0, 0);
    }
  }
}

struct ShadeOut {
  const float* d_normal;
  float* d_grad;
  float* d_feature;
  int64_t tail;
};

__device__ __forceinline__ int64_t dsu_uniform64(int64_t v) {
  const uint32_t lo = __builtin_amdgcn_readfirstlane((uint32_t)v);
  const uint32_t hi = __builtin_amdgcn_readfirstlane((uint32_t)((uint64_t)v >> 32));
  return (int64_t)(((uint64_t)hi << 32) | lo);
}

__device__ __forceinline__ void shade_grad_out(const ShadeIn& sh, const ShadeOut& so, int64_t si,
                                               float d0, float d1, float d2) {
  const float g0 = sh.grad[si * 3], g1 = sh.grad[si * 3 + 1], g2 = sh.grad[si * 3 + 2];
  const float len = sqrtf(g0 * g0 + g1 * g1 + g2 * g2);
  const float inv = 1.0f / fmaxf(len, 1e-12f);
  const float n0 = g0 * inv, n1 = g1 * inv, n2 = g2 * inv;
  if (so.d_normal) {
    d0 += so.d_normal[si * 3]; d1 += so.d_normal[si * 3 + 1]; d2 += so.d_normal[si * 3 + 2];
  }
  const float dot = n0 * d0 + n1 * d1 + n2 * d2;
  const bool ok = len > 1e-12f;
  so.d_grad[si * 3] = ok ? (d0 - n0 * dot) * inv : d0 * inv;
  so.d_grad[si * 3 + 1] = ok ? (d1 - n1 * dot) * inv : d1 * inv;
  so.d_grad[si * 3 + 2] = ok ? (d2 - n2 * dot) * inv : d2 * inv;
}

template <bool SHADE>
__device__ __forceinline__ void dead_sample_out(const ShadeIn& sh, const ShadeOut& so, float* __restrict__ d_x,
                                                int64_t i) {
  if (SHADE) {
#pragma unroll
    for (int k = 0; k < 13; ++k) so.d_feature[i * 13 + k] = 0.0f;
    shade_grad_out(sh, so, i, 0.0f, 0.0f, 0.0f);
  } else {
#pragma unroll
    for (int q = 0; q < 4; ++q)
      *reinterpret_cast<float4*>(d_x + i * TIN + 4 * q) = make_float4(0.0f, 0.0f, 0.0f, 0.0f);
  }
}

__global__ __launch_bounds__(1024) void texture_live_kernel(const float* __restrict__ d_rgb, int64_t n,
                                                            uint32_t* __restrict__ live_halves) {
  __shared__ uint32_t word;
  if (threadIdx.x == 0) word = 0u;
  __syncthreads();
  const int64_t i = (int64_t)blockIdx.x * 1024 + threadIdx.x;
  const bool lit = i < n && (d_rgb[i * 3] != 0.0f || d_rgb[i * 3 + 1] != 0.0f || d_rgb[i * 3 + 2] != 0.0f);
  const uint64_t m = __ballot(lit);
  if ((threadIdx.x & 63) == 0) {
    const uint32_t two = ((uint32_t)m != 0u ? 1u : 0u) | ((uint32_t)(m >> 32) != 0u ? 2u : 0u);
    if (two) atomicOr(&word, two << (2 * (threadIdx.x >> 6)));
  }
  __syncthreads();
  if (threadIdx.x == 0) live_halves[blockIdx.x] = word;
}

template <bool SHADE, bool L1_MASK = false>
__global__ __launch_bounds__(256) void texture_bwd_kernel(
    dsu_tex_mlp m, const float* __restrict__ x, ShadeIn sh, ShadeOut so,
    const float* __restrict__ rgb, const float* __restrict__ d_rgb, int64_t n,
    float* __restrict__ d_x, float* __restrict__ partials,
    const uint32_t* __restrict__ h1_mask, const uint32_t* __restrict__ live_halves) {
  extern __shared__ __attribute__((aligned(128))) float lds[];
  const int lane = threadIdx.x & 63, wave = threadIdx.x >> 6, l31 = lane & 31, h = lane >> 5;
  asm volatile("" ::: "a223");
  const int64_t halves = (n + 31) / 32;
  const bool scanned = live_halves != nullptr && halves <= 32 * (int64_t)texpart::MAX_WORDS;
  uint32_t* sbits = reinterpret_cast<uint32_t*>(lds + L_SCAN);
  uint32_t* spre = sbits + texpart::MAX_WORDS;
  const int words = scanned ? (int)((halves + 31) / 32) : 0;
  for (int w = threadIdx.x; w < words; w += blockDim.x)
    sbits[w] = texpart::clip_word(live_halves[w], w, (int)halves);
  const uint32_t stg = trs::lds_addr(lds + L_STAGE + wave * STAGE_F);
  const uint32_t stX = stg + SB_X + (ImgU::store_base(l31) ^ (8 * h)), stY = stX + (SB_Y - SB_X);
  const uint32_t stS = stg + SB_S + ImgS::store_base(l31);
  const uint32_t rdX = stg + SB_X + ImgU::read_base(lane), rdY = rdX + (SB_Y - SB_X);
  const uint32_t rdS = stg + SB_S + ImgS::read_base(lane);
  const uint32_t colY = stg + SB_Y + ImgU::col_base(lane);
  load_weights(lds, m);
  __syncthreads();
  if (scanned && wave == 0) {
    const int chunk = (words + 63) / 64, w0 = lane * chunk;
    int sum = 0;
    for (int k = 0; k < chunk; ++k)
      if (w0 + k < words) sum += __popc(sbits[w0 + k]);
    int incl = sum;
#pragma unroll
    for (int d = 1; d < 64; d <<= 1) {
      const int up = __shfl_up(incl, d);
      if (lane >= d) incl += up;
    }
    int before = incl - sum;
    for (int k = 0; k < chunk; ++k)
      if (w0 + k < words) {
        spre[w0 + k] = (uint32_t)before;
        before += __popc(sbits[w0 + k]);
      }
    if (lane == 63) spre[words] = (uint32_t)incl;
  }
  {
    bf16x8* img1 = reinterpret_cast<bf16x8*>(lds + L_IMG1);
    bf16x8* img0 = reinterpret_cast<bf16x8*>(lds + L_IMG0);
    for (int f = threadIdx.x; f < 8 * 64; f += blockDim.x) {
      const int ln = f & 63, c = f >> 6, g = c & 1, Tin = (c >> 1) & 1, To = c >> 2;
      float w[8];
#pragma unroll
      for (int t = 0; t < 8; ++t)
        w[t] = lds[L_W1 + feat_of(Tin, 8 * g + t, ln >> 5) * W1_ROW + 32 * To + (ln & 31)];
      bf16_split8(w, img1[f], img1[8 * 64 + f]);
    }
    for (int f = threadIdx.x; f < 4 * 64; f += blockDim.x) {
      const int ln = f & 63, c = f >> 6, g = c & 1, T = c >> 1;
      float w[8];
#pragma unroll
      for (int t = 0; t < 8; ++t)
        w[t] = (ln & 31) < TIN ? lds[L_W0 + feat_of(T, 8 * g + t, ln >> 5) * W0_ROW + (ln & 31)] : 0.0f;
      bf16_split8(w, img0[f], img0[4 * 64 + f]);
    }
    if constexpr (L1_MASK) {
      bf16x8* imgf = reinterpret_cast<bf16x8*>(lds + L_IMGF);
      for (int f = threadIdx.x; f < 8 * 64; f += blockDim.x) {
        const int ln = f & 63, c = f >> 6, g = c & 1, Tin = (c >> 1) & 1, To = c >> 2;
        float w[8];
#pragma unroll
        for (int t = 0; t < 8; ++t)
          w[t] = lds[L_W1 + (32 * To + (ln & 31)) * W1_ROW + feat_of(Tin, 8 * g + t, ln >> 5)];
        bf16_split8(w, imgf[f], imgf[8 * 64 + f]);
      }
    }
  }
  __syncthreads();

  if (SHADE) {
    for (int64_t t = blockIdx.x * (int64_t)blockDim.x + threadIdx.x; t < so.tail * 13;
         t += (int64_t)gridDim.x * blockDim.x)
      so.d_feature[n * 13 + t] = 0.0f;
  }
  f32x16 gw1[2][2], gw0[2], gw2[2];
  float gb1row = 0.0f;
  float gb2[TOUT] = {0.0f, 0.0f, 0.0f};
#pragma unroll
  for (int T = 0; T < 2; ++T)
#pragma unroll
    for (int r = 0; r < 16; ++r) {
      gw1[T][0][r] = gw1[T][1][r] = 0.0f;
      gw0[T][r] = gw2[T][r] = 0.0f;
    }

  if (scanned) {
    for (int64_t t = blockIdx.x * (int64_t)blockDim.x + threadIdx.x; t < n; t += (int64_t)gridDim.x * blockDim.x) {
      const int64_t hf = t >> 5;
      if (!((sbits[hf >> 5] >> (hf & 31)) & 1u)) dead_sample_out<SHADE>(sh, so, d_x, t);
    }
  }
  int64_t wh0, wh1;
  if (scanned) {
    const texpart::Scan sc{sbits, spre, words, (int)halves};
    const texpart::Run wg = texpart::split(sc, texpart::whole(sc), (int)gridDim.x, (int)blockIdx.x);
    const texpart::Run wr = texpart::split(sc, wg, 4, wave);
    wh0 = wr.h0; wh1 = wr.h1;
  } else {
    const int64_t per = (halves + gridDim.x - 1) / gridDim.x;
    const int64_t b0 = blockIdx.x * per < halves ? blockIdx.x * per : halves;
    const int64_t len = (b0 + per < halves ? b0 + per : halves) - b0;
    wh0 = b0 + wave * len / 4; wh1 = b0 + (wave + 1) * len / 4;
  }
  const int64_t r0 = 32 * dsu_uniform64(wh0);
  const int64_t r1 = 32 * dsu_uniform64(wh1) < n ? 32 * dsu_uniform64(wh1) : n;
  for (int64_t wave_first = r0; wave_first < r1; wave_first += 64) {
    const int64_t i = wave_first + lane;
    const bool valid = i < r1;
    const int64_t ii = valid ? i : r1 - 1;
    bool live0 = true, live1 = true;
    if (scanned) {
      const int64_t hf = wave_first >> 5;
      const uint32_t b0 = sbits[hf >> 5] >> (hf & 31), b1 = hf + 1 < halves ? sbits[(hf + 1) >> 5] >> ((hf + 1) & 31) : 0u;
      live0 = (__builtin_amdgcn_readfirstlane(b0) & 1u) != 0u;
      live1 = (__builtin_amdgcn_readfirstlane(b1) & 1u) != 0u;
      if (!live0 && !live1) continue;
    }
    float dr[TOUT];
#pragma unroll
    for (int o = 0; o < TOUT; ++o) dr[o] = d_rgb[ii * TOUT + o];
    if (!scanned) {
      const uint64_t lit = __ballot(valid && (dr[0] != 0.0f || dr[1] != 0.0f || dr[2] != 0.0f));
      live0 = (uint32_t)lit != 0u;
      live1 = (uint32_t)(lit >> 32) != 0u;
      if (valid && !(h ? live1 : live0)) dead_sample_out<SHADE>(sh, so, d_x, i);
      if (lit == 0ull) continue;
    }
    float in[TIN];
    if (SHADE) {
      float inv_len;
      load_shaded(sh, ii, in, inv_len);
    } else {
#pragma unroll
      for (int q = 0; q < 4; ++q) {
        const float4 v = *reinterpret_cast<const float4*>(x + ii * TIN + 4 * q);
        in[4 * q] = v.x; in[4 * q + 1] = v.y; in[4 * q + 2] = v.z; in[4 * q + 3] = v.w;
      }
    }
    float dz[TOUT];
#pragma unroll
    for (int o = 0; o < TOUT; ++o) {
      const float s = rgb[ii * TOUT + o];
      dz[o] = valid ? dr[o] * s * (1.0f - s) : 0.0f;
      gb2[o] += dz[o];
    }
    uint32_t mk2[2] = {0u, 0u};
    if constexpr (L1_MASK) {
#pragma unroll
      for (int a_ = 0; a_ < 2; ++a_) {
        int64_t si = wave_first + a_ * 32 + l31;
        si = si < r1 ? si : r1 - 1;
        mk2[a_] = h1_mask[si * 2 + h];
      }
    }
#pragma unroll 1
    for (int a = 0; a < 2; ++a) {
      if (wave_first + a * 32 >= r1 || !(a ? live1 : live0)) continue;
      f32x16 H0[2], H1[2];
      forward_half<L1_MASK>(lds, in, a, l31, h, H0, H1);
      const uint32_t mk = a ? mk2[1] : mk2[0];
      if constexpr (L1_MASK) {
#pragma unroll
        for (int T = 0; T < 2; ++T)
#pragma unroll
          for (int r = 0; r < 16; ++r) H1[T][r] = ((mk >> (16 * T + r)) & 1u) ? H1[T][r] : 0.0f;
      }
      float dza[TOUT];
#pragma unroll
      for (int o = 0; o < TOUT; ++o) {
        const float other = __shfl_xor(dz[o], 32);
        dza[o] = h == a ? dz[o] : other;
      }
      f32x16 D1[2];
#pragma unroll
      for (int T = 0; T < 2; ++T)
#pragma unroll
        for (int r = 0; r < 16; ++r) {
          float v = 0.0f;
#pragma unroll
          for (int o = 0; o < TOUT; ++o)
            v = fmaf(lds[L_W2P + (h * TOUT + o) * 32 + T * 16 + r], dza[o], v);
          D1[T][r] = (L1_MASK ? ((mk >> (16 * T + r)) & 1u) != 0u : H1[T][r] > 0.0f) ? v : 0.0f;
        }
      __builtin_amdgcn_wave_barrier();
      stage_units_T(stX, H1);
      if (h == a) stage_cols_S(stS, 0, dz[0], dz[1], dz[2], 0.0f);
      __builtin_amdgcn_wave_barrier();
      {
        f32x16 (&g0)[1] = *reinterpret_cast<f32x16 (*)[1]>(&gw2[0]);
        f32x16 (&g1)[1] = *reinterpret_cast<f32x16 (*)[1]>(&gw2[1]);
        gemm_samples_T<1>(g0, g1, rdX, rdS, TOUT, l31);
      }
      __builtin_amdgcn_wave_barrier();
      stage_units_T(stY, D1);
      stage_units_T(stX, H0);
      __builtin_amdgcn_wave_barrier();
      {
        float srow = 0.0f;
#pragma unroll
        for (int P0 = 0; P0 < 32; P0 += 4) {
          const uint32_t a4 = (colY ^ (uint32_t)ImgU::col_xor(P0)) + P0 * ImgU::ROW_B;
          const trs::bf16x4 vh = trs::read_tr(a4), vm = trs::read_tr(a4 + ImgU::PART_B);
#pragma unroll
          for (int e = 0; e < 4; ++e) srow += (float)vh[e] + (float)vm[e];
        }
        gb1row += srow;
      }
      gemm_samples_T<2>(gw1[0], gw1[1], rdY, rdX, 64, l31);
      f32x16 D0[2];
#pragma unroll
      for (int T = 0; T < 2; ++T)
#pragma unroll
        for (int r = 0; r < 16; ++r) D0[T][r] = 0.0f;
      {
        const bf16x8* img1 = reinterpret_cast<const bf16x8*>(lds + L_IMG1);
        bf16x8 bh[2][2], bm[2][2];
#pragma unroll
        for (int Tin = 0; Tin < 2; ++Tin)
#pragma unroll
          for (int g = 0; g < 2; ++g) {
            float v[8];
#pragma unroll
            for (int t = 0; t < 8; ++t) v[t] = D1[Tin][8 * g + t];
            bf16_split8(v, bh[Tin][g], bm[Tin][g]);
          }
#pragma unroll
        for (int To = 0; To < 2; ++To)
#pragma unroll
          for (int Tin = 0; Tin < 2; ++Tin)
#pragma unroll
            for (int g = 0; g < 2; ++g) {
              const int f = ((To * 2 + Tin) * 2 + g) * 64 + lane;
              const bf16x8 ah = img1[f], am = img1[8 * 64 + f];
              D0[To] = __builtin_amdgcn_mfma_f32_32x32x16_bf16(ah, bh[Tin][g], D0[To], 0, 0, 0);
              D0[To] = __builtin_amdgcn_mfma_f32_32x32x16_bf16(ah, bm[Tin][g], D0[To], 0, 0, 0);
              D0[To] = __builtin_amdgcn_mfma_f32_32x32x16_bf16(am, bh[Tin][g], D0[To], 0, 0, 0);
            }
      }
#pragma unroll
      for (int T = 0; T < 2; ++T)
#pragma unroll
        for (int r = 0; r < 16; ++r) D0[T][r] = H0[T][r] > 0.0f ? D0[T][r] : 0.0f;
      __builtin_amdgcn_wave_barrier();
      stage_units_T(stY, D0);
      if (h == a) {
#pragma unroll
        for (int s = 0; s < TIN / 4; ++s) stage_cols_S(stS, s, in[4 * s], in[4 * s + 1], in[4 * s + 2], in[4 * s + 3]);
        stage_cols_S(stS, TIN / 4, 1.0f, 0.0f, 0.0f, 0.0f);
      }
      __builtin_amdgcn_wave_barrier();
      {
        f32x16 (&g0)[1] = *reinterpret_cast<f32x16 (*)[1]>(&gw0[0]);
        f32x16 (&g1)[1] = *reinterpret_cast<f32x16 (*)[1]>(&gw0[1]);
        gemm_samples_T<1>(g0, g1, rdY, rdS, TIN + 1, l31);
      }
      f32x16 din;
#pragma unroll
      for (int r = 0; r < 16; ++r) din[r] = 0.0f;
      {
        const bf16x8* img0 = reinterpret_cast<const bf16x8*>(lds + L_IMG0);
#pragma unroll
        for (int T = 0; T < 2; ++T)
#pragma unroll
          for (int g = 0; g < 2; ++g) {
            float v[8];
#pragma unroll
            for (int t = 0; t < 8; ++t) v[t] = D0[T][8 * g + t];
            bf16x8 bh, bm;
            bf16_split8(v, bh, bm);
            const int f = (T * 2 + g) * 64 + lane;
            const bf16x8 ah = img0[f], am = img0[4 * 64 + f];
            din = __builtin_amdgcn_mfma_f32_32x32x16_bf16(ah, bh, din, 0, 0, 0);
            din = __builtin_amdgcn_mfma_f32_32x32x16_bf16(ah, bm, din, 0, 0, 0);
            din = __builtin_amdgcn_mfma_f32_32x32x16_bf16(am, bh, din, 0, 0, 0);
          }
      }
      const int64_t si = wave_first + a * 32 + l31;
      if (si < r1) {
        if (SHADE) {
#pragma unroll
          for (int q = 0; q < 2; ++q)
#pragma unroll
            for (int e = 0; e < 4; ++e) {
              const int comp = 8 * q + 4 * h + e;
              if (comp < 13) so.d_feature[si * 13 + comp] = din[4 * q + e];
            }
          if (h == 1) shade_grad_out(sh, so, si, din[5], din[6], din[7]);
        } else {
#pragma unroll
          for (int q = 0; q < 2; ++q)
            *reinterpret_cast<float4*>(d_x + si * TIN + 8 * q + 4 * h) =
                make_float4(din[4 * q], din[4 * q + 1], din[4 * q + 2], din[4 * q + 3]);
        }
      }
    }
  }

  __syncthreads();
  static_assert(4 * PART_STRIDE <= BWD_LDS_F, "four partial images fit the kernel's LDS");
  float gb2s[TOUT];
#pragma unroll
  for (int o = 0; o < TOUT; ++o) {
    float s_ = gb2[o];
#pragma unroll
    for (int k = 32; k > 0; k >>= 1) s_ += __shfl_xor(s_, k);
    gb2s[o] = s_;
  }
  auto store_own = [&](float* dst) {
#pragma unroll
    for (int T = 0; T < 2; ++T)
#pragma unroll
      for (int r = 0; r < 16; ++r) {
        const int row = feat_of(T, r, h);
        dst[P_GW1 + row * 64 + l31] = gw1[T][0][r];
        dst[P_GW1 + row * 64 + 32 + l31] = gw1[T][1][r];
        dst[P_GW0 + row * 32 + l31] = gw0[T][r];
        dst[P_GW2 + row * 32 + l31] = gw2[T][r];
      }
    dst[P_GB1 + lane] = gb1row;
    if (lane == 0) {
#pragma unroll
      for (int o = 0; o < TOUT; ++o) dst[P_GB2 + o] = gb2s[o];
    }
  };
  store_own(lds + wave * PART_STRIDE);
  __syncthreads();
  float* part = partials + (size_t)blockIdx.x * PART_STRIDE;
  for (int v = threadIdx.x; v < PART_N; v += blockDim.x)
    part[v] = (lds[v] + lds[PART_STRIDE + v]) + (lds[2 * PART_STRIDE + v] + lds[3 * PART_STRIDE + v]);
}

__global__ void texture_reduce_kernel(const float* __restrict__ partials, int nblocks,
                                      float* __restrict__ g_w0, float* __restrict__ g_b0,
                                      float* __restrict__ g_w1, float* __restrict__ g_b1,
                                      float* __restrict__ g_w2, float* __restrict__ g_b2) {
  __shared__ float red[16][64];
  const int e = threadIdx.x & 63, sl = threadIdx.x >> 6;
  const int v = blockIdx.x * 64 + e;
  const bool in_range = v < PART_N;
  float acc = 0.0f;
  if (in_range)
    for (int b = sl; b < nblocks; b += 16) acc += partials[(size_t)b * PART_STRIDE + v];
  red[sl][e] = acc;
  __syncthreads();
  if (sl != 0 || !in_range) return;
  float s = 0.0f;
#pragma unroll
  for (int k = 0; k < 16; ++k) s += red[k][e];
  if (v < P_GW0) {
    g_w1[v] += s;
  } else if (v < P_GW2) {
    const int i = (v - P_GW0) >> 5, k = (v - P_GW0) & 31;
    if (k < TIN) g_w0[i * TIN + k] += s;
    else if (k == TIN) g_b0[i] += s;
  } else if (v < P_GB1) {
    const int i = (v - P_GW2) >> 5, o = (v - P_GW2) & 31;
    if (o < TOUT) g_w2[o * THID + i] += s;
  } else if (v < P_GB2) {
    g_b1[v - P_GB1] += s;
  } else {
    g_b2[v - P_GB2] += s;
  }
}

int64_t live_words(int64_t n) { return (n + 1023) / 1024; }

bool mlp_ok(const dsu_tex_mlp* m) {
  return m && m->w0 && m->b0 && m->w1 && m->b1 && m->w2 && m->b2;
}

template <bool SHADE, bool L1_MASK>
int launch_bwd(const dsu_tex_mlp* mlp, const float* x, ShadeIn sh, ShadeOut so, const float* rgb,
               const float* d_rgb, int64_t n, float* d_x, const uint32_t* h1_mask, const uint32_t* live,
               void* workspace, int64_t workspace_bytes, hipStream_t s, int* blocks) {
  if (!workspace || workspace_bytes < dsu_texture_bwd_workspace_bytes(n)) return DSU_EINVAL;
  *blocks = dsu_onewave_blocks(n, 256, TEX_MAX_BLOCKS, 1);
  const int64_t words = live_words(n);
  if (words > texpart::MAX_WORDS) {
    live = nullptr;
  } else if (!live) {
    uint32_t* own = reinterpret_cast<uint32_t*>((float*)workspace +
                                                (size_t)dsu_capped_blocks(n, 256, TEX_MAX_BLOCKS) * PART_STRIDE);
    texture_live_kernel<<<(unsigned)words, 1024, 0, s>>>(d_rgb, n, own);
    live = own;
  }
  const size_t shm = (size_t)BWD_LDS_ALL_F * sizeof(float);
  DSU_ENSURE_DYN_LDS((texture_bwd_kernel<SHADE, L1_MASK>), shm);
  texture_bwd_kernel<SHADE, L1_MASK><<<*blocks, 256, shm, s>>>(*mlp, x, sh, so, rgb, d_rgb, n, d_x,
                                                              (float*)workspace, h1_mask, live);
  return DSU_OK;
}

void launch_reduce(const void* workspace, int blocks, float* g_w0, float* g_b0, float* g_w1,
                   float* g_b1, float* g_w2, float* g_b2, hipStream_t s) {
  texture_reduce_kernel<<<(PART_N + 63) / 64, 1024, 0, s>>>((const float*)workspace, blocks, g_w0,
                                                           g_b0, g_w1, g_b1, g_w2, g_b2);
}

}

extern "C" {

int dsu_texture_fwd(const dsu_tex_mlp* mlp, const float* tex_in, int64_t n, float* rgb,
                    void* stream) {
  if (!mlp_ok(mlp) || n < 0 || (n && (!tex_in || !rgb))) return DSU_EINVAL;
  if (n == 0) return DSU_OK;
  texture_fwd_kernel<false><<<dsu_capped_blocks(n, 256, 2048), 256, 0, (hipStream_t)stream>>>(
      *mlp, tex_in, ShadeIn{nullptr, nullptr}, nullptr, n, rgb, nullptr);
  DSU_CHECK_LAUNCH();
  return DSU_OK;
}

int dsu_texture_fwd_shaded_m(const dsu_tex_mlp* mlp, const float* feature, const float* grad,
                             int64_t n, float* normal, float* rgb, uint32_t* h1_mask, void* stream) {
  if (!mlp_ok(mlp) || n < 0 || (n && (!feature || !grad || !normal || !rgb))) return DSU_EINVAL;
  if (n == 0) return DSU_OK;
  texture_fwd_kernel<true><<<dsu_capped_blocks(n, 256, 2048), 256, 0, (hipStream_t)stream>>>(
      *mlp, nullptr, ShadeIn{feature, grad}, normal, n, rgb, h1_mask);
  DSU_CHECK_LAUNCH();
  return DSU_OK;
}

int64_t dsu_texture_bwd_workspace_bytes(int64_t n) {
  if (n < 0) return DSU_EINVAL;
  const int64_t words = live_words(n) <= texpart::MAX_WORDS ? live_words(n) : 0;
  return ((int64_t)dsu_capped_blocks(n, 256, TEX_MAX_BLOCKS) * PART_STRIDE + words) * (int64_t)sizeof(float);
}

int dsu_texture_bwd(const dsu_tex_mlp* mlp, const float* tex_in, const float* rgb,
                    const float* d_rgb, int64_t n, float* d_tex_in, float* g_w0, float* g_b0,
                    float* g_w1, float* g_b1, float* g_w2, float* g_b2, void* workspace,
                    int64_t workspace_bytes, void* stream) {
  if (!mlp_ok(mlp) || n < 0) return DSU_EINVAL;
  if (!g_w0 || !g_b0 || !g_w1 || !g_b1 || !g_w2 || !g_b2) return DSU_EINVAL;
  if (n && (!tex_in || !rgb || !d_rgb || !d_tex_in)) return DSU_EINVAL;
  if (n == 0) return DSU_OK;
  int blocks;
  const int rc = launch_bwd<false, false>(mlp, tex_in, ShadeIn{nullptr, nullptr},
                                          ShadeOut{nullptr, nullptr, nullptr, 0}, rgb, d_rgb, n, d_tex_in,
                                          nullptr, nullptr, workspace, workspace_bytes, (hipStream_t)stream,
                                          &blocks);
  if (rc != DSU_OK) return rc;
  launch_reduce(workspace, blocks, g_w0, g_b0, g_w1, g_b1, g_w2, g_b2, (hipStream_t)stream);
  DSU_CHECK_LAUNCH();
  return DSU_OK;
}

int dsu_texture_bwd_shaded(const dsu_tex_mlp* mlp, const float* feature, const float* grad,
                           const float* rgb, const float* d_rgb, const float* d_normal, int64_t n,
                           int64_t tail_rows, float* d_grad, float* d_feature, float* g_w0,
                           float* g_b0, float* g_w1,
                           float* g_b1, float* g_w2, float* g_b2, void* workspace,
                           int64_t workspace_bytes, void* stream) {
  if (!mlp_ok(mlp) || n < 0) return DSU_EINVAL;
  if (!g_w0 || !g_b0 || !g_w1 || !g_b1 || !g_w2 || !g_b2) return DSU_EINVAL;
  if (tail_rows < 0 || (n && (!feature || !grad || !rgb || !d_rgb || !d_grad || !d_feature)))
    return DSU_EINVAL;
  if (n == 0) return DSU_EUNSUP;
  int blocks;
  const int rc = launch_bwd<true, false>(mlp, nullptr, ShadeIn{feature, grad},
                                         ShadeOut{d_normal, d_grad, d_feature, tail_rows}, rgb, d_rgb, n,
                                         nullptr, nullptr, nullptr, workspace, workspace_bytes,
                                         (hipStream_t)stream, &blocks);
  if (rc != DSU_OK) return rc;
  launch_reduce(workspace, blocks, g_w0, g_b0, g_w1, g_b1, g_w2, g_b2, (hipStream_t)stream);
  DSU_CHECK_LAUNCH();
  return DSU_OK;
}

int32_t dsu_texture_partial_map(int32_t* map_host) {
  if (map_host) {
    constexpr int O_W0 = 0, O_B0 = THID * TIN, O_W1 = O_B0 + THID, O_B1 = O_W1 + THID * THID,
                  O_W2 = O_B1 + THID, O_B2 = O_W2 + TOUT * THID;
    for (int v = 0; v < PART_N; ++v) {
      int d = -1;
      if (v < P_GW0) {
        d = O_W1 + v;
      } else if (v < P_GW2) {
        const int i = (v - P_GW0) >> 5, k = (v - P_GW0) & 31;
        if (k < TIN) d = O_W0 + i * TIN + k;
        else if (k == TIN) d = O_B0 + i;
      } else if (v < P_GB1) {
        const int i = (v - P_GW2) >> 5, o = (v - P_GW2) & 31;
        if (o < TOUT) d = O_W2 + o * THID + i;
      } else if (v < P_GB2) {
        d = O_B1 + (v - P_GB1);
      } else {
        d = O_B2 + (v - P_GB2);
      }
      map_host[v] = d;
    }
  }
  return PART_N;
}

static int shaded_partials(const dsu_tex_mlp* mlp, const float* feature, const float* grad,
                           const float* rgb, const float* d_rgb, const float* d_normal,
                           int64_t n, int64_t tail_rows, float* d_grad, float* d_feature,
                           const uint32_t* h1_mask, const uint32_t* live, void* workspace,
                           int64_t workspace_bytes, dsu_partial_reduce* red, void* stream) {
  if (!mlp_ok(mlp) || n < 0 || !red) return DSU_EINVAL;
  if (tail_rows < 0 || (n && (!feature || !grad || !rgb || !d_rgb || !d_grad || !d_feature)))
    return DSU_EINVAL;
  if (n == 0) return DSU_EUNSUP;
  const ShadeIn sh{feature, grad};
  const ShadeOut so{d_normal, d_grad, d_feature, tail_rows};
  int blocks;
  const int rc = h1_mask ? launch_bwd<true, true>(mlp, nullptr, sh, so, rgb, d_rgb, n, nullptr, h1_mask, live,
                                                  workspace, workspace_bytes, (hipStream_t)stream, &blocks)
                         : launch_bwd<true, false>(mlp, nullptr, sh, so, rgb, d_rgb, n, nullptr, nullptr, live,
                                                   workspace, workspace_bytes, (hipStream_t)stream, &blocks);
  if (rc != DSU_OK) return rc;
  DSU_CHECK_LAUNCH();
  red->partials = (const float*)workspace;
  red->nblocks = blocks;
  red->stride = PART_STRIDE;
  red->n = PART_N;
  return DSU_OK;
}

int dsu_texture_bwd_shaded_partials_live(const dsu_tex_mlp* mlp, const float* feature, const float* grad,
                                         const float* rgb, const float* d_rgb, const float* d_normal,
                                         int64_t n, int64_t tail_rows, float* d_grad, float* d_feature,
                                         const uint32_t* h1_mask, const uint32_t* live_halves,
                                         void* workspace, int64_t workspace_bytes,
                                         dsu_partial_reduce* red, void* stream) {
  if (!live_halves) return DSU_EINVAL;
  return shaded_partials(mlp, feature, grad, rgb, d_rgb, d_normal, n, tail_rows, d_grad, d_feature, h1_mask,
                         live_halves, workspace, workspace_bytes, red, stream);
}

int dsu_texture_bwd_shaded_partials_m(const dsu_tex_mlp* mlp, const float* feature, const float* grad,
                                      const float* rgb, const float* d_rgb, const float* d_normal,
                                      int64_t n, int64_t tail_rows, float* d_grad, float* d_feature,
                                      const uint32_t* h1_mask, void* workspace, int64_t workspace_bytes,
                                      dsu_partial_reduce* red, void* stream) {
  return shaded_partials(mlp, feature, grad, rgb, d_rgb, d_normal, n, tail_rows, d_grad, d_feature, h1_mask,
                         nullptr, workspace, workspace_bytes, red, stream);
}

int dsu_texture_live_partition(const uint32_t* live_halves, int64_t n_halves, int32_t parts,
                               int32_t waves, int32_t* runs) {
  if (!live_halves || !runs || n_halves < 1 || parts < 1 || waves < 1) return DSU_EINVAL;
  const int64_t words = (n_halves + 31) / 32;
  if (words > texpart::MAX_WORDS) return DSU_EUNSUP;
  std::vector<uint32_t> bits((size_t)words), pre((size_t)words + 1);
  pre[0] = 0;
  for (int64_t w = 0; w < words; ++w) {
    bits[w] = texpart::clip_word(live_halves[w], (int)w, (int)n_halves);
    pre[w + 1] = pre[w] + (uint32_t)texpart::popc(bits[w]);
  }
  const texpart::Scan sc{bits.data(), pre.data(), (int)words, (int)n_halves};
  const texpart::Run all = texpart::whole(sc);
  for (int b = 0; b < parts; ++b) {
    const texpart::Run wg = texpart::split(sc, all, parts, b);
    for (int w = 0; w < waves; ++w) {
      const texpart::Run r = texpart::split(sc, wg, waves, w);
      runs[2 * (b * waves + w)] = r.h0;
      runs[2 * (b * waves + w) + 1] = r.h1;
    }
  }
  return DSU_OK;
}

}
```

### drawingspinup_amd/ops.py

```python
import ctypes as C
from dataclasses import dataclass

import torch

from . import _lib
from ._lib import DsuError, HashGridCfg, NormCfg, SdfMlp, check, lib, ptr, stream


@dataclass(frozen=True)
class HashGridConfig:
    n_levels: int = 10
    n_features_per_level: int = 2
    log2_hashmap_size: int = 19
    base_resolution: int = 32
    per_level_scale: float = 1.3195079107728942

    def c(self):
        return HashGridCfg(self.n_levels, self.n_features_per_level, self.log2_hashmap_size,
                           self.base_resolution, self.per_level_scale)

    def levels(self):
        return _lib.hashgrid_levels(self.c())

    @property
# ... 458 lines not shown
class DeferredSum:

    def __init__(self, record, keep):
        self.record, self.keep = record, keep


def texture_bwd_shaded_partials(params, feature, grad, rgb, d_rgb, d_normal, tail_rows=0, h1_mask=None):
    from ._lib import PartialReduce
    feature, grad, rgb, d_rgb = _f32c(feature), _f32c(grad), _f32c(rgb), _f32c(d_rgb)
    n = rgb.shape[0]
    dev = rgb.device
    d_grad = torch.empty((n, 3), dtype=torch.float32, device=dev)
    d_feat = torch.empty((n + tail_rows, 13), dtype=torch.float32, device=dev)
    flat = torch.zeros(sum(t.numel() for t in params), dtype=torch.float32, device=dev)
    wbytes = int(lib().dsu_texture_bwd_workspace_bytes(n))
    ws = torch.empty(max(wbytes, 4) // 4, dtype=torch.float32, device=dev)
    m = _tex_struct(params)
    dn = None if d_normal is None else _f32c(d_normal)
    rec = PartialReduce()
    check(lib().dsu_texture_bwd_shaded_partials_m(C.byref(m), ptr(feature), ptr(grad), ptr(rgb),
                                                  ptr(d_rgb), ptr(dn), n, int(tail_rows), ptr(d_grad),
                                                  ptr(d_feat), ptr(h1_mask, torch.int32), ptr(ws), wbytes,
                                                  C.byref(rec), stream()),
          "dsu_texture_bwd_shaded_partials_m")
    tmap = torch.from_numpy(texture_partial_map()).to(dev)
    rec.map, rec.base = tmap.data_ptr(), flat.data_ptr()
    return d_grad, d_feat, flat, DeferredSum(rec, (ws, tmap, flat))


def ortho_ray_batch(index, x, y, c2w, origins, directions, images, normals, masks, view_weights):
    n = index.shape[0]
    dev = images.device
    V, H, W, ch = images.shape
    f = lambda *shape: torch.empty(*shape, dtype=torch.float32, device=dev)
    out = {"rays": f(n, 6), "rgb": f(n, ch), "normal": f(n, 3), "mask": f(n), "cosines": f(n),
           "view_weights": f(n)}
    i64 = torch.int64
    check(lib().dsu_ortho_ray_batch(ptr(index, i64), ptr(x, i64), ptr(y, i64), n, ptr(_f32c(c2w)),
                                    ptr(origins, torch.float32), ptr(directions, torch.float32),
                                    ptr(images, torch.float32), ch, ptr(normals, torch.float32),
                                    ptr(masks, torch.float32), ptr(view_weights, torch.float32), H,
                                    W, ptr(out["rays"]), ptr(out["rgb"]), ptr(out["normal"]),
                                    ptr(out["mask"]), ptr(out["cosines"]), ptr(out["view_weights"]),
                                    stream()), "dsu_ortho_ray_batch")
    return out


RAY_LOSS_MAX_RAYS = 8192


def ray_losses(comp, rgb, normal, mask, cosines, view_weights, cfg):
    from ._lib import RayLossCfg
    comp = _f32c(comp)
    r = comp.shape[0]
    c = RayLossCfg(float(cfg["rgb_p_ratio"]), float(cfg["normal_p_ratio"]),
                   float(cfg["mask_p_ratio"]), float(cfg["lambda_rgb_mse"]),
                   float(cfg["lambda_rgb_l1"]), float(cfg["lambda_normal"]),
                   float(cfg["lambda_mask"]), int(bool(cfg["geo_aware"])), 0)
    terms = torch.empty(4, dtype=torch.float32, device=comp.device)
    d_comp = torch.empty_like(comp)
    check(lib().dsu_ray_losses(ptr(comp), ptr(_f32c(rgb)), ptr(_f32c(normal)), ptr(_f32c(mask)),
                               ptr(_f32c(cosines)), ptr(_f32c(view_weights)), r, C.byref(c),
                               ptr(terms), ptr(d_comp), stream()), "dsu_ray_losses")
    return terms, d_comp


def sample_losses(sdf_all, grad_all, n_samples, n_random, lambda_eikonal, lambda_sparsity,
                  sparsity_scale, lambda_smooth, d_sdf_all=None, d_grad_all=None):
    sdf_all, grad_all = _f32c(sdf_all), _f32c(grad_all)
    acc = d_sdf_all is not None
    if not acc:
        d_sdf_all = torch.empty_like(sdf_all)
        d_grad_all = torch.empty_like(grad_all)
    assert sdf_all.shape[0] == n_samples + 2 * n_random
    terms = torch.empty(3, dtype=torch.float32, device=sdf_all.device)
    check(lib().dsu_sample_losses(ptr(sdf_all), ptr(grad_all), n_samples, n_random,
                                  float(lambda_eikonal), float(lambda_sparsity),
                                  float(sparsity_scale), float(lambda_smooth), int(acc),
                                  ptr(d_sdf_all, torch.float32), ptr(d_grad_all, torch.float32),
                                  ptr(terms), stream()), "dsu_sample_losses")
    return terms, d_sdf_all, d_grad_all


def weights_from_alpha_fwd(alpha, offsets, counts):
    alpha = _f32c(alpha)
    w = torch.empty_like(alpha)
    check(lib().dsu_weights_from_alpha_fwd(ptr(alpha), ptr(offsets, torch.int32),
                                           ptr(counts, torch.int32), offsets.shape[0], ptr(w),
                                           stream()), "dsu_weights_from_alpha_fwd")
    return w


def weights_from_alpha_bwd(alpha, weights, d_weights, offsets, counts):
    d_alpha = torch.empty_like(alpha)
    check(lib().dsu_weights_from_alpha_bwd(ptr(_f32c(alpha)), ptr(_f32c(weights)),
                                           ptr(_f32c(d_weights)), ptr(offsets, torch.int32),
                                           ptr(counts, torch.int32), offsets.shape[0],
                                           ptr(d_alpha), stream()), "dsu_weights_from_alpha_bwd")
    return d_alpha


def accumulate_fwd(weights, values, offsets, counts):
    weights = _f32c(weights)
    n_rays = offsets.shape[0]
    ch = 1 if values is None else values.shape[-1]
    v = None if values is None else _f32c(values)
    out = torch.empty((n_rays, ch), dtype=torch.float32, device=weights.device)
    check(lib().dsu_accumulate_fwd(ptr(weights), ptr(v), ch, ptr(offsets, torch.int32),
                                   ptr(counts, torch.int32), n_rays, ptr(out), stream()),
          "dsu_accumulate_fwd")
    return out


def occgrid_ema(occs, idx, occ, decay):
    scratch = torch.empty(occ.shape[0], dtype=torch.float32, device=occs.device) \
        if idx is not None else None
    check(lib().dsu_occgrid_ema(ptr(occs, torch.float32), ptr(idx, torch.int64) if idx is not None
                                else None, ptr(_f32c(occ)), occ.shape[0], float(decay),
                                ptr(scratch) if scratch is not None else None, stream()),
          "dsu_occgrid_ema")


def occgrid_binarize(occs, thre):
    out = torch.empty(occs.shape[0], dtype=torch.uint8, device=occs.device)
    check(lib().dsu_occgrid_binarize(ptr(occs, torch.float32), occs.shape[0], float(thre),
                                     ptr(out), stream()), "dsu_occgrid_binarize")
    return out


ACT = {"none": 0, None: 0, "relu": 1, "leaky_relu": 2, "tanh": 3}


def ric_offsets(H, W, device):
    out = torch.empty((18, H, W), dtype=torch.float32, device=device)
    check(lib().dsu_ric_offsets(H, W, ptr(out), stream()), "dsu_ric_offsets")
    return out


def deform_conv3x3(x, offset, weight, ep_scale=None, ep_shift=None, act=None, residual=None,
                   in_relu=False):
    x, weight, offset = _f32c(x), _f32c(weight), _f32c(offset)
    B, Cin, H, W = x.shape
    O = weight.shape[0]
    assert weight.shape[1:] == (Cin, 3, 3), "dsu deform conv: 3x3, groups=1 only"
    bstride = 0 if offset.dim() == 3 or offset.shape[0] == 1 else 18 * H * W
    out = torch.empty((B, O, H, W), dtype=torch.float32, device=x.device)
    check(lib().dsu_deform_conv3x3_fwd(ptr(x), ptr(offset), bstride, ptr(weight), B, Cin, H, W, O,
                                       int(in_relu), ptr(ep_scale), ptr(ep_shift), ACT[act],
                                       ptr(residual), ptr(out), stream()),
          "dsu_deform_conv3x3_fwd")
    return out


def conv2d(x, weight, bias=None, stride=1, padding=0, ep_scale=None, ep_shift=None, act=None,
           residual=None, in_relu=False):
    x, weight = _f32c(x), _f32c(weight)
    B, Cin, H, W = x.shape
    O, Cw, k, k2 = weight.shape
    assert Cw == Cin and k == k2
    OH = (H + 2 * padding - k) // stride + 1
    OW = (W + 2 * padding - k) // stride + 1
    out = torch.empty((B, O, OH, OW), dtype=torch.float32, device=x.device)
    check(lib().dsu_conv2d_fwd(ptr(x), ptr(weight), ptr(bias), B, Cin, H, W, O, k, stride,
                               padding, int(in_relu), ptr(ep_scale), ptr(ep_shift), ACT[act],
                               ptr(residual),
                               ptr(out), stream()), "dsu_conv2d_fwd")
# ... 438 lines not shown
                                  latents.numel(), float(guidance_scale), float(sqrt_a_t),
                                  float(sqrt_1m_a_t), float(sqrt_a_prev), float(std), ptr(out),
                                  stream()), "dsu_ddim_cfg_step")
    return out


def shade_prep_fwd(grad, feature):
    grad, feature = _f32c(grad), _f32c(feature)
    n = grad.shape[0]
    normal = torch.empty((n, 3), dtype=torch.float32, device=grad.device)
    tex_in = torch.empty((n, 16), dtype=torch.float32, device=grad.device)
    check(lib().dsu_shade_prep_fwd(ptr(grad), ptr(feature), n, ptr(normal), ptr(tex_in), stream()),
          "dsu_shade_prep_fwd")
    return normal, tex_in


def shade_prep_bwd(grad, d_normal, d_tex_in, out=None):
    grad = _f32c(grad)
    n = grad.shape[0]
    if out is None:
        d_grad = torch.empty((n, 3), dtype=torch.float32, device=grad.device)
        d_feat = torch.empty((n, 13), dtype=torch.float32, device=grad.device)
    else:
        d_grad, d_feat = out
        assert d_grad.shape == (n, 3) and d_feat.shape == (n, 13)
    dn = None if d_normal is None else _f32c(d_normal)
    check(lib().dsu_shade_prep_bwd(ptr(grad), ptr(dn), ptr(_f32c(d_tex_in)), n, ptr(d_grad),
                                   ptr(d_feat), stream()), "dsu_shade_prep_bwd")
    return d_grad, d_feat


def neus_composite_fwd(sdf, normal, rgb, rays_d, t_starts, t_ends, offsets, counts, inv_s, car):
    n, n_rays = sdf.shape[0], rays_d.shape[0]
    dev = sdf.device
    alpha = torch.empty(n, dtype=torch.float32, device=dev)
    w = torch.empty(n, dtype=torch.float32, device=dev)
    comp = torch.empty((n_rays, 8), dtype=torch.float32, device=dev)
    check(lib().dsu_neus_composite_fwd(ptr(_f32c(sdf)), ptr(_f32c(normal)), ptr(_f32c(rgb)),
                                       ptr(_f32c(rays_d)), ptr(_f32c(t_starts)), ptr(_f32c(t_ends)),
                                       ptr(offsets, torch.int32), ptr(counts, torch.int32), n_rays,
                                       ptr(inv_s, torch.float32), float(car), ptr(alpha), ptr(w),
                                       ptr(comp), stream()), "dsu_neus_composite_fwd")
    return comp, alpha, w


def neus_composite_bwd(sdf, normal, rgb, rays_d, t_starts, t_ends, offsets, counts, inv_s, car,
                       alpha, weights, d_comp, d_weights=None, d_sdf_out=None):
    n, n_rays = sdf.shape[0], rays_d.shape[0]
    dev = sdf.device
    d_sdf = torch.empty(n, dtype=torch.float32, device=dev) if d_sdf_out is None else d_sdf_out
    assert d_sdf.shape == (n,)
    d_normal = torch.empty((n, 3), dtype=torch.float32, device=dev)
    d_rgb = torch.empty((n, 3), dtype=torch.float32, device=dev)
    d_inv = torch.zeros(1, dtype=torch.float32, device=dev)
    dw = None if d_weights is None else _f32c(d_weights)
    check(lib().dsu_neus_composite_bwd(ptr(_f32c(sdf)), ptr(_f32c(normal)), ptr(_f32c(rgb)),
                                       ptr(_f32c(rays_d)), ptr(_f32c(t_starts)), ptr(_f32c(t_ends)),
                                       ptr(offsets, torch.int32), ptr(counts, torch.int32), n_rays,
                                       ptr(inv_s, torch.float32), float(car), ptr(alpha),
                                       ptr(weights), ptr(_f32c(d_comp)), ptr(dw), ptr(d_sdf),
                                       ptr(d_normal), ptr(d_rgb), ptr(d_inv), stream()),
          "dsu_neus_composite_bwd")
    return d_sdf, d_normal, d_rgb, d_inv


def neus_composite_bwd_live(sdf, normal, rgb, rays_d, t_starts, t_ends, offsets, counts, inv_s, car,
                            alpha, weights, d_comp):
    n, n_rays = sdf.shape[0], rays_d.shape[0]
    dev = sdf.device
    d_sdf = torch.empty(n, dtype=torch.float32, device=dev)
    d_normal = torch.empty((n, 3), dtype=torch.float32, device=dev)
    d_rgb = torch.empty((n, 3), dtype=torch.float32, device=dev)
    d_inv = torch.zeros(1, dtype=torch.float32, device=dev)
    live = torch.zeros((n + 1023) // 1024, dtype=torch.int32, device=dev)
    check(lib().dsu_neus_composite_bwd_live(ptr(_f32c(sdf)), ptr(_f32c(normal)), ptr(_f32c(rgb)),
                                            ptr(_f32c(rays_d)), ptr(_f32c(t_starts)), ptr(_f32c(t_ends)),
                                            ptr(offsets, torch.int32), ptr(counts, torch.int32), n_rays,
                                            ptr(inv_s, torch.float32), float(car), ptr(alpha),
                                            ptr(weights), ptr(_f32c(d_comp)), None, ptr(d_sdf),
                                            ptr(d_normal), ptr(d_rgb), ptr(d_inv), ptr(live, torch.int32),
                                            stream()),
          "dsu_neus_composite_bwd_live")
    return d_sdf, d_normal, d_rgb, d_inv, live


def texture_live_partition(live_words, n_halves, parts, waves=4):
    import numpy as np
    words = np.ascontiguousarray(live_words, dtype=np.uint32)
    assert words.size * 32 >= n_halves
    runs = np.empty((parts, waves, 2), dtype=np.int32)
    check(lib().dsu_texture_live_partition(words.ctypes.data_as(C.c_void_p), int(n_halves), int(parts),
                                           int(waves), runs.ctypes.data_as(C.c_void_p)),
          "dsu_texture_live_partition")
    return runs


class ZGrid:

    def __init__(self, data, lo, hi, points=False, cells_per_axis=None):
        import math
        dev = data.device
        n = data.shape[0]
        g = cells_per_axis or int(min(1024, max(8, math.sqrt(max(n, 1) / 2.0))))
        span = max(float(hi[0] - lo[0]), float(hi[1] - lo[1]), 1e-9)
        self.g, self.cell = g, span / g * (1.0 + 1e-6)
        self.x0, self.y0 = float(lo[0]), float(lo[1])
        count_fn = lib().dsu_point_bin_count if points else lib().dsu_zgrid_count
        fill_fn = lib().dsu_point_bin_fill if points else lib().dsu_zgrid_fill
        counts = torch.zeros(g * g, dtype=torch.int32, device=dev)
        check(count_fn(ptr(data, torch.float32), n, self.x0, self.y0, self.cell, g, ptr(counts),
                       stream()), "grid count")
        self.offsets = torch.zeros(g * g + 1, dtype=torch.int32, device=dev)
        self.offsets[1:] = torch.cumsum(counts, 0)
        total = int(self.offsets[-1])
        self.items = torch.empty(max(total, 1), dtype=torch.int32, device=dev)
        cursor = torch.zeros(g * g, dtype=torch.int32, device=dev)
        check(fill_fn(ptr(data, torch.float32), n, self.x0, self.y0, self.cell, g, ptr(self.offsets),
                      ptr(cursor), ptr(self.items), stream()), "grid fill")
        self.data = data

    def args(self):
        return (self.x0, self.y0, self.cell, self.g, ptr(self.offsets), ptr(self.items))


def zray_cast(grid, faces_i32, origins, sign, self_vertex=None):
    origins = _f32c(origins)
    n = origins.shape[0]
    dev = origins.device
    cnt = torch.empty(n, dtype=torch.int32, device=dev)
    fn, ff = torch.empty_like(cnt), torch.empty_like(cnt)
    tn, tf = torch.empty(n, device=dev), torch.empty(n, device=dev)
    x0, y0, cell, g, off, items = grid.args()
    check(lib().dsu_zray_cast(ptr(grid.data, torch.float32), ptr(faces_i32, torch.int32),
                              grid.data.shape[0], x0, y0, cell, g, off, items, ptr(origins), n,
                              int(sign), ptr(self_vertex, torch.int32), ptr(cnt), ptr(tn), ptr(fn),
                              ptr(tf), ptr(ff), stream()), "dsu_zray_cast")
    return cnt, tn, fn, tf, ff


def raster_mask(tris, scale, res):
    mask = torch.zeros(res, res, dtype=torch.uint8, device=tris.device)
    check(lib().dsu_raster_mask(ptr(tris, torch.float32), tris.shape[0], float(scale), int(res),
                                ptr(mask), stream()), "dsu_raster_mask")
    return mask


def erode_ellipse_u8(mask, ksize):
    out = torch.empty_like(mask)
    check(lib().dsu_erode_ellipse_u8(ptr(mask, torch.uint8), mask.shape[0], mask.shape[1], int(ksize),
                                     ptr(out), stream()), "dsu_erode_ellipse_u8")
    return out


def knn8_blend(query_xy, known_xy, known_rgb):
    q64 = query_xy.to(torch.float64).contiguous()
    k64 = known_xy.to(torch.float64).contiguous()
    known_rgb = _f32c(known_rgb)
    k32 = k64.to(torch.float32).contiguous()
    both = torch.cat([q64.to(torch.float32), k32], 0)
    grid = ZGrid(k32, both.amin(0).tolist(), both.amax(0).tolist(), points=True)
    out = torch.empty(q64.shape[0], 3, device=q64.device)
    x0, y0, cell, g, off, items = grid.args()
    check(lib().dsu_knn8_blend(ptr(q64, torch.float64), q64.shape[0], ptr(k64, torch.float64),
                               ptr(known_rgb), k64.shape[0], x0, y0, cell, g, off, items, ptr(out),
                               stream()), "dsu_knn8_blend")
    return out
# ... 547 lines not shown
```

### include/dsu_hip.h

```cpp
#ifndef DSU_HIP_H
#define DSU_HIP_H

#include <stdint.h>

#ifdef __cplusplus
extern "C" {
#endif

#define DSU_OK 0
#define DSU_EINVAL (-1)
#define DSU_ELAUNCH (-2)
#define DSU_EUNSUP (-3)

#define DSU_MAX_LEVELS 16

const char* dsu_strerror(int code);
int dsu_abi_version(void);
int dsu_set_onewave_grid_cap(int32_t cus);
int dsu_set_scatter_grid_cap(int32_t workgroups);
int dsu_set_nsr_side_stream_priority(int32_t level);
int dsu_set_nsr_side_stream_pooling(int32_t on);

typedef struct {
  uint32_t n_levels;
// ... 81 lines not shown
int dsu_ray_aabb(const float* rays_o, const float* rays_d, int64_t n_rays, const float* aabb6,
                 const float* jitter, float step, float* t_min, float* t_max, void* stream);

int dsu_ray_march_scratch(const float* rays_o, const float* rays_d, const float* t_min,
                          const float* t_max, int64_t n_rays, const float* aabb6,
                          const uint8_t* occ_binary, int32_t res, float step, int32_t capacity,
                          int32_t* num_steps, float* scratch_t_starts, float* scratch_t_ends,
                          void* stream);
int dsu_ray_compact(const float* scratch_t_starts, const float* scratch_t_ends, int32_t capacity,
                    const int32_t* offsets, const int32_t* counts, int64_t n_rays,
                    int64_t* ray_indices, float* t_starts, float* t_ends, void* stream);

int dsu_ray_compact_points(const float* scratch_t_starts, const float* scratch_t_ends,
                           int32_t capacity, const int32_t* offsets, const int32_t* counts,
                           int64_t n_rays, const float* rays_o, const float* rays_d,
                           float* t_starts, float* t_ends, float* positions, void* stream);
int dsu_ray_compact_points_cap(const float* scratch_t_starts, const float* scratch_t_ends,
                           int32_t capacity, const int32_t* offsets, const int32_t* counts,
                           int64_t n_rays, const float* rays_o, const float* rays_d,
                           float* t_starts, float* t_ends, float* positions, int64_t out_capacity,
                               void* stream);
int dsu_ray_offsets(const int32_t* counts, int64_t n_rays, int32_t* offsets, int32_t* stats,
                    void* stream);

int dsu_weights_from_alpha_fwd(const float* alpha, const int32_t* offsets, const int32_t* counts,
                               int64_t n_rays, float* weights, void* stream);
int dsu_weights_from_alpha_bwd(const float* alpha, const float* weights, const float* d_weights,
                               const int32_t* offsets, const int32_t* counts, int64_t n_rays,
                               float* d_alpha, void* stream);

int dsu_accumulate_fwd(const float* weights, const float* values, int32_t channels,
                       const int32_t* offsets, const int32_t* counts, int64_t n_rays,
                       float* out, void* stream);

int dsu_occgrid_ema(float* occs, const int64_t* idx, const float* occ, int64_t n, float decay,
                    float* scratch, void* stream);
int dsu_occgrid_binarize(const float* occs, int64_t n_cells, float thre, uint8_t* binary,
                         void* stream);

typedef struct dsu_occgrid_refresh_args {
  float* occs;
  uint8_t* binary;
  int32_t res, all_cells;
  const float* aabb;
  uint64_t seed;
  int64_t step;
  const dsu_hashgrid_cfg* grid;
  const void* table_img;
  const dsu_sdf_mlp* mlp;
  const float* inv_s;
  float radius, render_step_size, ema_decay, occ_thre;
  uint32_t active_levels;
  int32_t inj_count;
  const int32_t* inj_cells;
  const float* inj_rand;
  float* thre_out;
  void* workspace;
  int64_t workspace_bytes;
  int32_t* cells_out;
  float* rand_out;
} dsu_occgrid_refresh_args;
int64_t dsu_occgrid_refresh_workspace_bytes(int32_t res);
int dsu_occgrid_refresh(const dsu_occgrid_refresh_args* args, void* stream);

int dsu_neus_composite_fwd(const float* sdf, const float* normal, const float* rgb,
                           const float* rays_d, const float* t_starts, const float* t_ends,
                           const int32_t* offsets, const int32_t* counts, int64_t n_rays,
                           const float* inv_s, float cos_anneal_ratio, float* alpha,
                           float* weights, float* comp, void* stream);
int dsu_neus_composite_bwd(const float* sdf, const float* normal, const float* rgb,
                           const float* rays_d, const float* t_starts, const float* t_ends,
                           const int32_t* offsets, const int32_t* counts, int64_t n_rays,
                           const float* inv_s, float cos_anneal_ratio, const float* alpha,
                           const float* weights, const float* d_comp, const float* d_weights,
                           float* d_sdf, float* d_normal, float* d_rgb, float* d_inv_s,
                           void* stream);
int dsu_neus_composite_bwd_live(const float* sdf, const float* normal, const float* rgb,
                                const float* rays_d, const float* t_starts, const float* t_ends,
                                const int32_t* offsets, const int32_t* counts, int64_t n_rays,
                                const float* inv_s, float cos_anneal_ratio, const float* alpha,
                                const float* weights, const float* d_comp, const float* d_weights,
                                float* d_sdf, float* d_normal, float* d_rgb, float* d_inv_s,
                                uint32_t* live_halves, void* stream);
int dsu_shade_prep_fwd(const float* grad, const float* feature, int64_t n, float* normal,
                       float* tex_in, void* stream);
int dsu_shade_prep_bwd(const float* grad, const float* d_normal, const float* d_tex_in, int64_t n,
                       float* d_grad, float* d_feature, void* stream);

typedef struct dsu_tex_mlp {
  const float *w0, *b0, *w1, *b1, *w2, *b2;
} dsu_tex_mlp;
int dsu_texture_fwd(const dsu_tex_mlp* mlp, const float* tex_in, int64_t n, float* rgb,
                    void* stream);
int64_t dsu_texture_bwd_workspace_bytes(int64_t n);
int dsu_texture_bwd(const dsu_tex_mlp* mlp, const float* tex_in, const float* rgb,
                    const float* d_rgb, int64_t n, float* d_tex_in, float* g_w0, float* g_b0,
                    float* g_w1, float* g_b1, float* g_w2, float* g_b2, void* workspace,
                    int64_t workspace_bytes, void* stream);

int dsu_texture_fwd_shaded_m(const dsu_tex_mlp* mlp, const float* feature, const float* grad,
                             int64_t n, float* normal, float* rgb, uint32_t* h1_mask, void* stream);
int dsu_texture_bwd_shaded(const dsu_tex_mlp* mlp, const float* feature, const float* grad,
                           const float* rgb, const float* d_rgb, const float* d_normal, int64_t n,
                           int64_t tail_rows, float* d_grad, float* d_feature, float* g_w0,
                           float* g_b0, float* g_w1, float* g_b1, float* g_w2, float* g_b2,
                           void* workspace, int64_t workspace_bytes, void* stream);

int32_t dsu_texture_partial_map(int32_t* map_host);
int dsu_texture_bwd_shaded_partials_m(const dsu_tex_mlp* mlp, const float* feature, const float* grad,
                                      const float* rgb, const float* d_rgb, const float* d_normal,
                                      int64_t n, int64_t tail_rows, float* d_grad, float* d_feature,
                                      const uint32_t* h1_mask, void* workspace, int64_t workspace_bytes,
                                      dsu_partial_reduce* red, void* stream);
int dsu_texture_bwd_shaded_partials_live(const dsu_tex_mlp* mlp, const float* feature, const float* grad,
                                         const float* rgb, const float* d_rgb, const float* d_normal,
                                         int64_t n, int64_t tail_rows, float* d_grad, float* d_feature,
                                         const uint32_t* h1_mask, const uint32_t* live_halves,
                                         void* workspace, int64_t workspace_bytes,
                                         dsu_partial_reduce* red, void* stream);
int dsu_texture_live_partition(const uint32_t* live_halves, int64_t n_halves, int32_t parts,
                               int32_t waves, int32_t* runs);

int dsu_ortho_ray_batch(const int64_t* index, const int64_t* x, const int64_t* y, int64_t n,
                        const float* c2w, const float* origins, const float* directions,
                        const float* images, int32_t image_channels, const float* normals,
                        const float* masks, const float* view_weights, int32_t H, int32_t W,
                        float* rays, float* rgb, float* normal, float* mask, float* cosines,
                        float* vw, void* stream);

int dsu_ortho_ray_batch_split(const int64_t* index, const int64_t* x, const int64_t* y, int64_t n,
                              const float* c2w, const float* origins, const float* directions,
                              const float* images, int32_t image_channels, const float* normals,
                              const float* masks, const float* view_weights, int32_t H, int32_t W,
                              float* rays, float* rgb, float* normal, float* mask, float* cosines,
                              float* vw, float* rays_o, float* rays_d, void* stream);

#define DSU_RAY_LOSS_MAX_RAYS 8192
typedef struct dsu_ray_loss_cfg {
  double rgb_p_ratio, normal_p_ratio, mask_p_ratio;
  float lambda_rgb_mse, lambda_rgb_l1, lambda_normal, lambda_mask;
  int32_t geo_aware;
  int32_t reserved;
} dsu_ray_loss_cfg;
int dsu_ray_losses(const float* comp, const float* rgb, const float* normal, const float* mask,
                   const float* cosines, const float* view_weights, int32_t n_rays,
                   const dsu_ray_loss_cfg* cfg, float* terms, float* d_comp, void* stream);

int dsu_sample_losses(const float* sdf_all, const float* grad_all, int64_t n_samples,
                      int64_t n_random, float lambda_eikonal, float lambda_sparsity,
                      float sparsity_scale, float lambda_smooth, int32_t accumulate_prefix,
                      float* d_sdf_all, float* d_grad_all, float* terms, void* stream);


int dsu_ric_offsets(int32_t H, int32_t W, float* offsets, void* stream);

int dsu_deform_conv3x3_fwd(const float* input, const float* offset, int64_t offset_batch_stride,
                           const float* weight, int32_t B, int32_t C, int32_t H, int32_t W,
                           int32_t O, int32_t in_relu, const float* ep_scale,
                           const float* ep_shift, int32_t act, const float* residual, float* out,
                           void* stream);

int dsu_conv2d_fwd(const float* input, const float* weight, const float* bias, int32_t B,
                   int32_t C, int32_t H, int32_t W, int32_t O, int32_t k, int32_t stride,
                   int32_t pad, int32_t in_relu, const float* ep_scale, const float* ep_shift,
                   int32_t act, const float* residual, float* out, void* stream);

int64_t dsu_conv_x3_packed_elems(int32_t O, int32_t C, int32_t k);
int dsu_conv_x3_pack_weights(const float* weight, int32_t O, int32_t C, int32_t k, uint16_t* w_hi,
                             uint16_t* w_mid, void* stream);
int dsu_deform_conv3x3_fwd_x3(const float* input, const float* offset, int64_t offset_batch_stride,
                              const uint16_t* w_hi, const uint16_t* w_mid, int32_t B, int32_t C,
                              int32_t H, int32_t W, int32_t O, int32_t in_relu,
                              const float* ep_scale, const float* ep_shift, int32_t act,
                              const float* residual, float* out, void* stream);
int dsu_conv2d_fwd_x3(const float* input, const uint16_t* w_hi, const uint16_t* w_mid,
                      const float* bias, int32_t B, int32_t C, int32_t H, int32_t W, int32_t O,
                      int32_t k, int32_t stride, int32_t pad, int32_t in_relu,
                      const float* ep_scale, const float* ep_shift, int32_t act,
                      const float* residual, float* out, void* stream);

int dsu_conv_f32p_pack_weights(const float* weight, int32_t O, int32_t C, int32_t k, float* w_packed,
                               void* stream);
int dsu_deform_conv3x3_fwd_f32p(const float* input, const float* offset, int64_t offset_batch_stride,
                                const float* w_packed, int32_t B, int32_t C, int32_t H, int32_t W,
                                int32_t O, int32_t in_relu, const float* ep_scale,
                                const float* ep_shift, int32_t act, const float* residual, float* out,
                                void* stream);
int dsu_conv2d_fwd_f32p(const float* input, const float* w_packed, const float* bias, int32_t B,
                        int32_t C, int32_t H, int32_t W, int32_t O, int32_t k, int32_t stride,
                        int32_t pad, int32_t in_relu, const float* ep_scale, const float* ep_shift,
                        int32_t act, const float* residual, float* out, void* stream);


int64_t dsu_deform_tap_table_bytes(int32_t H, int32_t W);
int dsu_deform_tap_table(const float* offset, int32_t H, int32_t W, void* table, void* stream);

int64_t dsu_conv2d_wgrad_workspace_bytes(int32_t deform, int32_t B, int32_t C, int32_t O,
                                         int32_t OH, int32_t OW, int32_t k);
int dsu_conv2d_wgrad(const float* input, const float* dout, const void* tap_table, int32_t B,
                     int32_t C, int32_t H, int32_t W, int32_t O, int32_t k, int32_t stride,
                     int32_t pad, float* workspace, float* dweight, int32_t accumulate,
                     void* stream);

int dsu_deform_conv3x3_dgrad_gather(const float* dcol, const int32_t* rowptr, const int32_t* src,
                                    const float* wgt, int64_t planes, int32_t npix, float* dx,
                                    void* stream);

typedef struct dsu_norm_cfg {
  int32_t batch, channels, hw;
  int32_t instance;
  int32_t act;
  int32_t stat_updates;
  float eps;
  float momentum;
} dsu_norm_cfg;
int dsu_norm_train_fwd(const dsu_norm_cfg* cfg, const float* x, const float* gamma,
                       const float* beta, float* running_mean, float* running_var, float* y,
                       float* save_mean, float* save_invstd, void* stream);
int dsu_norm_train_bwd(const dsu_norm_cfg* cfg, const float* x, const float* y, const float* dy,
                       const float* gamma, const float* save_mean, const float* save_invstd,
                       float* dx, float* dgamma, float* dbeta, void* stream);

int dsu_channel_sum(const float* x, int32_t B, int32_t C, int32_t HW, float* out, void* stream);

int dsu_act_fwd(const float* x, float* y, int64_t n, int32_t act, void* stream);
int dsu_act_bwd(const float* dy, const float* y, float* dx, int64_t n, int32_t act, void* stream);

int dsu_maxpool2_fwd(const float* x, float* y, int64_t planes, int32_t H, int32_t W, void* stream);
int dsu_maxpool2_bwd(const float* x, const float* dy, float* dx, int64_t planes, int32_t H,
                     int32_t W, void* stream);

int dsu_upsample2_fwd(const float* x, float* y, int64_t planes, int32_t H, int32_t W,
                      void* stream);
int dsu_upsample2_bwd(const float* dy, float* dx, int64_t planes, int32_t H, int32_t W,
// ... 332 lines not shown
```

Before: 0.3828.

## Fuse sample losses into ray-loss launch and accumulate gradients in backward kernels

The sample-loss computation (eikonal, sparsity, smoothness) now runs inside the ray-loss launch. Its gradients are written first, and the composite backward and texture backward kernels add into them through new accumulate variants, so the separate sample-loss launch goes away. The rank-select sort in the ray losses also moves from an LDS bitonic sort to a register-resident bitonic sort using warp shuffles, touching shared memory only for long strides. The aims are fewer kernel launches, fewer passes over the gradient buffers and less LDS traffic, at the cost of more complex kernels and a read-modify-write ordering dependency between kernels.

```diff
diff --git a/drawingspinup_amd/_lib.py b/drawingspinup_amd/_lib.py
--- a/drawingspinup_amd/_lib.py
+++ b/drawingspinup_amd/_lib.py
@@ -6,7 +6,7 @@
 _HERE = os.path.dirname(os.path.abspath(__file__))
 LIB_PATH = os.environ.get("DSU_HIP_LIB") or os.path.join(_HERE, "libdsu_hip.so")
 MAX_LEVELS = 16
-ABI_VERSION = 3
+ABI_VERSION = 4
 
 c_i32, c_i64, c_u32, c_f32, c_vp = C.c_int32, C.c_int64, C.c_uint32, C.c_float, C.c_void_p
 
@@ -128,6 +128,8 @@
                                           C.POINTER(PartialReduce), P],
     "dsu_texture_bwd_shaded_partials_live": [C.POINTER(TexMlp), P, P, P, P, P, c_i64, c_i64, P, P, P, P, P,
                                              c_i64, C.POINTER(PartialReduce), P],
+    "dsu_texture_bwd_shaded_partials_live_acc": [C.POINTER(TexMlp), P, P, P, P, P, c_i64, c_i64, P, P, P, P,
+                                                 P, c_i64, C.POINTER(PartialReduce), P],
     "dsu_texture_live_partition": [P, c_i64, c_i32, c_i32, P],
     "dsu_texture_fwd_shaded_m": [C.POINTER(TexMlp), P, P, c_i64, P, P, P, P],
     "dsu_occgrid_refresh_workspace_bytes": [c_i32],
@@ -239,6 +241,8 @@
                             P, P, P, P],
     "dsu_ray_losses": [P, P, P, P, P, P, c_i32, C.POINTER(RayLossCfg), P, P, P],
     "dsu_sample_losses": [P, P, c_i64, c_i64, c_f32, c_f32, c_f32, c_f32, c_i32, P, P, P, P],
+    "dsu_ray_losses_with_samples": [P, P, P, P, P, P, c_i32, C.POINTER(RayLossCfg), P, P, P, P, c_i64,
+                                    c_i64, c_f32, c_f32, c_f32, c_f32, c_i32, P, P, P, P],
     "dsu_texture_fwd": [C.POINTER(TexMlp), P, c_i64, P, P],
     "dsu_texture_bwd_workspace_bytes": [c_i64],
     "dsu_texture_bwd": [C.POINTER(TexMlp), P, P, P, c_i64, P, P, P, P, P, P, P, P, c_i64, P],
@@ -252,6 +256,8 @@
                                P, P],
     "dsu_neus_composite_bwd_live": [P, P, P, P, P, P, P, P, c_i64, P, c_f32, P, P, P, P, P, P, P,
                                     P, P, P],
+    "dsu_neus_composite_bwd_live_acc": [P, P, P, P, P, P, P, P, c_i64, P, c_f32, P, P, P, P, P, P, P,
+                                        P, P, P],
     "dsu_shade_prep_fwd": [P, P, c_i64, P, P, P],
     "dsu_shade_prep_bwd": [P, P, P, c_i64, P, P, P],
     "dsu_occgrid_ema": [P, P, P, c_i64, c_f32, P, P],
diff --git a/drawingspinup_amd/csrc/capi.hip b/drawingspinup_amd/csrc/capi.hip
--- a/drawingspinup_amd/csrc/capi.hip
+++ b/drawingspinup_amd/csrc/capi.hip
@@ -20,7 +20,7 @@
   }
 }
 
-int dsu_abi_version(void) { return 3; }
+int dsu_abi_version(void) { return 4; }
 
 int32_t dsu_onewave_grid_cap_value = 0;
 int32_t dsu_scatter_grid_cap_value = 0;
diff --git a/drawingspinup_amd/csrc/nsr_driver.hip b/drawingspinup_amd/csrc/nsr_driver.hip
--- a/drawingspinup_amd/csrc/nsr_driver.hip
+++ b/drawingspinup_amd/csrc/nsr_driver.hip
@@ -689,29 +689,28 @@
   } else {
     DSU_HIP(hipMemsetAsync(L.comp, 0, (size_t)a->n_rays * 8 * sizeof(float), s));
   }
-  DSU_TRY(dsu_ray_losses(L.comp, f.rgb, f.normal, f.mask, f.cosines, f.vw, a->n_rays, &c.ray_loss,
-                         terms, L.d_comp, s));
+  DSU_TRY(dsu_ray_losses_with_samples(L.comp, f.rgb, f.normal, f.mask, f.cosines, f.vw, a->n_rays,
+                                      &c.ray_loss, terms, L.d_comp, L.a_sdf, L.a_grad, n_s, n_r,
+                                      c.lambda_eikonal, c.lambda_sparsity, c.sparsity_scale,
+                                      c.lambda_smooth, 1, L.d_sdf_all, L.d_grad_all, terms + 4, s));
   dsu_partial_reduce tex_red{};
   bool have_tex_red = false;
   if (n_s > 0) {
     uint32_t* live = L.live_halves[a->step & 1];
-    DSU_TRY(dsu_neus_composite_bwd_live(L.a_sdf, L.normal, L.rgb, f.rays_d, f.t_starts, f.t_ends,
-                                        f.offsets, f.counts, a->n_rays, L.inv_s, a->cos_anneal_ratio,
-                                        L.alpha, L.w, L.d_comp, nullptr, L.d_sdf_all, L.d_normal, L.d_rgb,
-                                        L.d_inv, live, s));
+    DSU_TRY(dsu_neus_composite_bwd_live_acc(L.a_sdf, L.normal, L.rgb, f.rays_d, f.t_starts, f.t_ends,
+                                            f.offsets, f.counts, a->n_rays, L.inv_s, a->cos_anneal_ratio,
+                                            L.alpha, L.w, L.d_comp, nullptr, L.d_sdf_all, L.d_normal,
+                                            L.d_rgb, L.d_inv, live, s));
     dsu_tex_mlp tex{c.tex[0], c.tex[1], c.tex[2], c.tex[3], c.tex[4], c.tex[5]};
-    DSU_TRY(dsu_texture_bwd_shaded_partials_live(&tex, L.a_feat, L.a_grad, L.rgb, L.d_rgb, L.d_normal, n_s,
-                                                 2 * n_r, L.d_grad_all, L.d_feat_all, L.tex_mask, live,
-                                                 L.tex_ws, L.tex_ws_bytes, &tex_red, s));
+    DSU_TRY(dsu_texture_bwd_shaded_partials_live_acc(&tex, L.a_feat, L.a_grad, L.rgb, L.d_rgb, L.d_normal,
+                                                     n_s, 2 * n_r, L.d_grad_all, L.d_feat_all, L.tex_mask,
+                                                     live, L.tex_ws, L.tex_ws_bytes, &tex_red, s));
     tex_red.map = L.tex_map;
     tex_red.base = L.g_tex;
     have_tex_red = true;
   } else {
     DSU_HIP(hipMemsetAsync(L.d_feat_all, 0, (size_t)(2 * n_r) * 13 * sizeof(float), s));
   }
-  DSU_TRY(dsu_sample_losses(L.a_sdf, L.a_grad, n_s, n_r, c.lambda_eikonal, c.lambda_sparsity,
-                            c.sparsity_scale, c.lambda_smooth, 1 | 2, L.d_sdf_all, L.d_grad_all,
-                            terms + 4, s));
   float* gg = L.g_geo;
   DSU_TRY(mark(d, 1, s));
   DSU_TRY(dsu_sdf_fd_bwd_sorted_fold(&c.grid, a->table_img, &mlp, pts, perm, n_all, c.radius, a->eps,
diff --git a/drawingspinup_amd/csrc/nsr_render.hip b/drawingspinup_amd/csrc/nsr_render.hip
--- a/drawingspinup_amd/csrc/nsr_render.hip
+++ b/drawingspinup_amd/csrc/nsr_render.hip
@@ -432,6 +432,7 @@
   }
 }
 
+template <bool ACC>
 __global__ __launch_bounds__(256) void composite_bwd_kernel(
     const float* __restrict__ sdf, const float* __restrict__ normal,
     const float* __restrict__ rgb, const float* __restrict__ rays_d,
@@ -513,7 +514,7 @@
           d_tc *= d_ic;
           dn[0] = d_tc * d[0]; dn[1] = d_tc * d[1]; dn[2] = d_tc * d[2];
         }
-        d_sdf[i] = dsdf;
+        d_sdf[i] = ACC ? d_sdf[i] + dsdf : dsdf;
         d_normal[i * 3] = dn[0] + w * dc[5];
         d_normal[i * 3 + 1] = dn[1] + w * dc[6];
         d_normal[i * 3 + 2] = dn[2] + w * dc[7];
@@ -760,7 +761,7 @@
   if (n_rays < 0 || !inv_s || (n_rays && (!rays_d || !offsets || !counts || !d_comp || !d_inv_s)))
     return DSU_EINVAL;
   if (n_rays == 0) return DSU_OK;
-  composite_bwd_kernel<<<(unsigned)((n_rays + 3) / 4), 256, 0, (hipStream_t)stream>>>(
+  composite_bwd_kernel<false><<<(unsigned)((n_rays + 3) / 4), 256, 0, (hipStream_t)stream>>>(
       sdf, normal, rgb, rays_d, t_starts, t_ends, offsets, counts, n_rays, inv_s,
       cos_anneal_ratio, alpha, weights, d_comp, d_weights, d_sdf, d_normal, d_rgb, d_inv_s, nullptr);
   DSU_CHECK_LAUNCH();
@@ -778,7 +779,26 @@
       (n_rays && (!rays_d || !offsets || !counts || !d_comp || !d_inv_s)))
     return DSU_EINVAL;
   if (n_rays == 0) return DSU_OK;
-  composite_bwd_kernel<<<(unsigned)((n_rays + 3) / 4), 256, 0, (hipStream_t)stream>>>(
+  composite_bwd_kernel<false><<<(unsigned)((n_rays + 3) / 4), 256, 0, (hipStream_t)stream>>>(
+      sdf, normal, rgb, rays_d, t_starts, t_ends, offsets, counts, n_rays, inv_s,
+      cos_anneal_ratio, alpha, weights, d_comp, d_weights, d_sdf, d_normal, d_rgb, d_inv_s,
+      live_halves);
+  DSU_CHECK_LAUNCH();
+  return DSU_OK;
+}
+
+int dsu_neus_composite_bwd_live_acc(const float* sdf, const float* normal, const float* rgb,
+                                    const float* rays_d, const float* t_starts, const float* t_ends,
+                                    const int32_t* offsets, const int32_t* counts, int64_t n_rays,
+                                    const float* inv_s, float cos_anneal_ratio, const float* alpha,
+                                    const float* weights, const float* d_comp, const float* d_weights,
+                                    float* d_sdf, float* d_normal, float* d_rgb, float* d_inv_s,
+                                    uint32_t* live_halves, void* stream) {
+  if (n_rays < 0 || !inv_s || !live_halves ||
+      (n_rays && (!rays_d || !offsets || !counts || !d_comp || !d_inv_s)))
+    return DSU_EINVAL;
+  if (n_rays == 0) return DSU_OK;
+  composite_bwd_kernel<true><<<(unsigned)((n_rays + 3) / 4), 256, 0, (hipStream_t)stream>>>(
       sdf, normal, rgb, rays_d, t_starts, t_ends, offsets, counts, n_rays, inv_s,
       cos_anneal_ratio, alpha, weights, d_comp, d_weights, d_sdf, d_normal, d_rgb, d_inv_s,
       live_halves);
diff --git a/drawingspinup_amd/csrc/nsr_step.hip b/drawingspinup_amd/csrc/nsr_step.hip
--- a/drawingspinup_amd/csrc/nsr_step.hip
+++ b/drawingspinup_amd/csrc/nsr_step.hip
@@ -75,6 +75,64 @@
   }
 }
 
+__device__ __forceinline__ void cmpx(uint64_t& lo, uint64_t& hi, bool up) {
+  const uint64_t a = lo, b = hi;
+  const bool sw = (a > b) == up;
+  lo = sw ? b : a;
+  hi = sw ? a : b;
+}
+
+template <int E, int J0>
+__device__ __forceinline__ void sort_in_thread(uint64_t (&v)[E], int base, int k) {
+#pragma unroll
+  for (int j = J0; j > 0; j >>= 1) {
+#pragma unroll
+    for (int q = 0; q < E; ++q)
+      if ((q & j) == 0) cmpx(v[q], v[q | j], ((base + q) & k) == 0);
+  }
+}
+
+template <int E>
+__device__ __forceinline__ void sort_in_registers(uint64_t (&v)[E], uint64_t* buf0, uint64_t* buf1, int P) {
+  const int base = (int)threadIdx.x * E;
+  sort_in_thread<E, 1>(v, base, 2);
+  if constexpr (E >= 4) sort_in_thread<E, 2>(v, base, 4);
+  if constexpr (E >= 8) sort_in_thread<E, 4>(v, base, 8);
+  static_assert(E == 2 || E == 4 || E == 8, "keys per thread");
+  int turn = 0;
+  for (int k = 2 * E; k <= P; k <<= 1) {
+    const bool up = (base & k) == 0;
+    for (int j = k >> 1; j >= E; j >>= 1) {
+      const bool low = (base & j) == 0;
+      const bool keep_min = low == up;
+      if (j >= 64 * E) {
+        uint64_t* buf = turn ? buf1 : buf0;
+        turn ^= 1;
+#pragma unroll
+        for (int q = 0; q < E; ++q) buf[q * RL_THREADS + threadIdx.x] = v[q];
+        __syncthreads();
+#pragma unroll
+        for (int q = 0; q < E; ++q) {
+          const uint64_t o = buf[q * RL_THREADS + (threadIdx.x ^ (j / E))];
+          const uint64_t mn = o < v[q] ? o : v[q], mx = o < v[q] ? v[q] : o;
+          v[q] = keep_min ? mn : mx;
+        }
+      } else {
+        const int m = j / E;
+#pragma unroll
+        for (int q = 0; q < E; ++q) {
+          const uint32_t olo = (uint32_t)__shfl_xor((int)(uint32_t)v[q], m);
+          const uint32_t ohi = (uint32_t)__shfl_xor((int)(uint32_t)(v[q] >> 32), m);
+          const uint64_t o = ((uint64_t)ohi << 32) | olo;
+          const uint64_t mn = o < v[q] ? o : v[q], mx = o < v[q] ? v[q] : o;
+          v[q] = keep_min ? mn : mx;
+        }
+      }
+    }
+    sort_in_thread<E, E / 2>(v, base, k);
+  }
+}
+
 struct RankLds {
   uint64_t* keys;
   int* pos;
@@ -83,30 +141,8 @@
   int* redi;
 };
 
-template <class ErrF>
-__device__ float rank_select(ErrF errf, const float* __restrict__ vw, int R, int P, double ratio,
-                             bool mean, const RankLds& lds, int64_t* k_out) {
-  for (int i = threadIdx.x; i < P; i += blockDim.x) {
-    float e = 0.0f;
-    bool valid = false;
-    if (i < R) errf(i, e, valid);
-    lds.keys[i] = ((uint64_t)flipf(valid ? e : INFINITY) << 32) | (uint32_t)i;
-    lds.pos[i] = valid ? 1 : 0;
-    lds.gerr[i] = 0.0f;
-  }
-  __syncthreads();
-  const int E = P / blockDim.x;
-  int c = 0;
-  for (int q = 0; q < E; ++q) c += lds.pos[threadIdx.x * E + q];
-  int nvalid;
-  int run = block_excl_scan(c, lds.redi, &nvalid);
-  for (int q = 0; q < E; ++q) {
-    const int i = threadIdx.x * E + q;
-    run += lds.pos[i];
-    lds.pos[i] = run - 1;
-  }
-  __syncthreads();
-  bitonic_sort(lds.keys, P);
+__device__ __forceinline__ float rank_finish(const float* __restrict__ vw, double ratio, bool mean,
+                                             int nvalid, const RankLds& lds, int64_t* k_out) {
   const int64_t kk = (int64_t)floor(ratio * (double)nvalid);
   float total = 0.0f;
   for (int64_t j = threadIdx.x; j < kk; j += blockDim.x) {
@@ -124,21 +160,89 @@
   return mean ? total / (float)kk : total;
 }
 
+template <int E, class ErrF>
+__device__ __forceinline__ float rank_select_regs(ErrF errf, const float* __restrict__ vw, int R, int P,
+                                                  double ratio, bool mean, const RankLds& lds,
+                                                  int64_t* k_out) {
+  const int base = (int)threadIdx.x * E;
+  uint64_t v[E];
+  uint32_t vbits = 0u;
+#pragma unroll
+  for (int q = 0; q < E; ++q) {
+    const int i = base + q;
+    float e = 0.0f;
+    bool valid = false;
+    if (i < R) errf(i, e, valid);
+    v[q] = ((uint64_t)flipf(valid ? e : INFINITY) << 32) | (uint32_t)i;
+    vbits |= valid ? 1u << q : 0u;
+  }
+  sort_in_registers<E>(v, lds.keys, reinterpret_cast<uint64_t*>(lds.pos), P);
+  __syncthreads();
+#pragma unroll
+  for (int q = 0; q < E; ++q) {
+    lds.keys[base + q] = v[q];
+    lds.gerr[base + q] = 0.0f;
+  }
+  int nvalid;
+  int run = block_excl_scan(__popc(vbits), lds.redi, &nvalid);
+#pragma unroll
+  for (int q = 0; q < E; ++q) {
+    run += (int)((vbits >> q) & 1u);
+    lds.pos[base + q] = run - 1;
+  }
+  __syncthreads();
+  return rank_finish(vw, ratio, mean, nvalid, lds, k_out);
+}
+
+template <class ErrF>
+__device__ float rank_select(ErrF errf, const float* __restrict__ vw, int R, int P, double ratio,
+                             bool mean, const RankLds& lds, int64_t* k_out) {
+  if (blockDim.x == RL_THREADS) {
+    switch (P / RL_THREADS) {
+      case 8: return rank_select_regs<8>(errf, vw, R, P, ratio, mean, lds, k_out);
+      case 4: return rank_select_regs<4>(errf, vw, R, P, ratio, mean, lds, k_out);
+      case 2: return rank_select_regs<2>(errf, vw, R, P, ratio, mean, lds, k_out);
+      default: break;
+    }
+  }
+  for (int i = threadIdx.x; i < P; i += blockDim.x) {
+    float e = 0.0f;
+    bool valid = false;
+    if (i < R) errf(i, e, valid);
+    lds.keys[i] = ((uint64_t)flipf(valid ? e : INFINITY) << 32) | (uint32_t)i;
+    lds.pos[i] = valid ? 1 : 0;
+    lds.gerr[i] = 0.0f;
+  }
+  __syncthreads();
+  const int E = P / blockDim.x;
+  int c = 0;
+  for (int q = 0; q < E; ++q) c += lds.pos[threadIdx.x * E + q];
+  int nvalid;
+  int run = block_excl_scan(c, lds.redi, &nvalid);
+  for (int q = 0; q < E; ++q) {
+    const int i = threadIdx.x * E + q;
+    run += lds.pos[i];
+    lds.pos[i] = run - 1;
+  }
+  __syncthreads();
+  bitonic_sort(lds.keys, P);
+  return rank_finish(vw, ratio, mean, nvalid, lds, k_out);
+}
+
 __device__ __forceinline__ float signf0(float x) { return x > 0.0f ? 1.0f : (x < 0.0f ? -1.0f : 0.0f); }
 
-__global__ __launch_bounds__(RL_THREADS) void ray_losses_kernel(
+__device__ __forceinline__ void ray_losses_body(
+    const int term, unsigned char* smem,
     const float* __restrict__ comp, const float* __restrict__ rgb, const float* __restrict__ normal,
     const float* __restrict__ maskf, const float* __restrict__ cosines,
-    const float* __restrict__ vw, int R, int P, dsu_ray_loss_cfg cfg, float* __restrict__ terms,
+    const float* __restrict__ vw, int R, int P, const dsu_ray_loss_cfg& cfg, float* __restrict__ terms,
     float* __restrict__ d_comp) {
-  extern __shared__ __attribute__((aligned(16))) unsigned char smem[];
   RankLds lds;
   lds.keys = reinterpret_cast<uint64_t*>(smem);
   lds.pos = reinterpret_cast<int*>(smem + (size_t)P * 8);
   lds.gerr = reinterpret_cast<float*>(smem + (size_t)P * 12);
   lds.redf = reinterpret_cast<float*>(smem + (size_t)P * 16);
   lds.redi = reinterpret_cast<int*>(smem + (size_t)P * 16 + 128);
-  const int term = blockIdx.x;
 
   auto fg = [&](int i) {
     const float cb = cosines[i] > -0.1f ? 0.0f : cosines[i];
@@ -270,7 +374,18 @@
   }
 }
 
-__global__ __launch_bounds__(256) void sample_losses_kernel(
+__global__ __launch_bounds__(RL_THREADS) void ray_losses_kernel(
+    const float* __restrict__ comp, const float* __restrict__ rgb, const float* __restrict__ normal,
+    const float* __restrict__ maskf, const float* __restrict__ cosines,
+    const float* __restrict__ vw, int R, int P, dsu_ray_loss_cfg cfg, float* __restrict__ terms,
+    float* __restrict__ d_comp) {
+  extern __shared__ __attribute__((aligned(16))) unsigned char smem[];
+  ray_losses_body(blockIdx.x, smem, comp, rgb, normal, maskf, cosines, vw, R, P, cfg, terms, d_comp);
+}
+
+enum { SL_STORE = 0, SL_ADD = 1, SL_STORE_FIRST = 2 };
+__device__ __forceinline__ void sample_losses_body(
+    const int64_t block, const int64_t nblocks,
     const float* __restrict__ sdf, const float* __restrict__ grad, int64_t n_s, int64_t n_r,
     float lambda_eik, float lambda_sp, float sp_scale, float lambda_sm, int accumulate_prefix,
     float* __restrict__ d_sdf, float* __restrict__ d_grad, float* __restrict__ terms) {
@@ -279,15 +394,15 @@
   const float inv_ns = n_s > 0 ? 1.0f / (float)n_s : 0.0f;
   const float inv_nr = n_r > 0 ? 1.0f / (float)n_r : 0.0f;
   const float inv_3nr = n_r > 0 ? 1.0f / (float)(3 * n_r) : 0.0f;
-  for (int64_t i = blockIdx.x * (int64_t)blockDim.x + threadIdx.x; i < n;
-       i += (int64_t)gridDim.x * blockDim.x) {
+  const int tid = threadIdx.x & 255, quarter = threadIdx.x >> 8;
+  for (int64_t i = block < nblocks ? block * 256 + tid : n; i < n; i += nblocks * 256) {
     if (i < n_s) {
       const float g0 = grad[i * 3], g1 = grad[i * 3 + 1], g2 = grad[i * 3 + 2];
       const float nrm = sqrtf((g0 * g0 + g1 * g1) + g2 * g2);
       const float dl = nrm - 1.0f;
       s_eik += dl * dl;
       const float cf = nrm > 0.0f ? lambda_eik * 2.0f * dl * inv_ns / nrm : 0.0f;
-      if (accumulate_prefix) {
+      if (accumulate_prefix == SL_ADD) {
         d_grad[i * 3] += cf * g0;
         d_grad[i * 3 + 1] += cf * g1;
         d_grad[i * 3 + 2] += cf * g2;
@@ -295,7 +410,7 @@
         d_grad[i * 3] = cf * g0;
         d_grad[i * 3 + 1] = cf * g1;
         d_grad[i * 3 + 2] = cf * g2;
-        d_sdf[i] = 0.0f;
+        d_sdf[i] = accumulate_prefix == SL_STORE_FIRST ? -0.0f : 0.0f;
       }
     } else {
       const int64_t a = i, b = i + n_r;
@@ -314,23 +429,50 @@
       }
     }
   }
-  __shared__ float red[3][4];
+  __shared__ float red[RL_THREADS / 256][3][4];
   s_eik = wave_sum(s_eik);
   s_sp = wave_sum(s_sp);
   s_sm = wave_sum(s_sm);
-  const int lane = threadIdx.x & 63, wave = threadIdx.x >> 6;
+  const int lane = tid & 63, wave = tid >> 6;
   if (lane == 0) {
-    red[0][wave] = s_eik;
-    red[1][wave] = s_sp;
-    red[2][wave] = s_sm;
+    red[quarter][0][wave] = s_eik;
+    red[quarter][1][wave] = s_sp;
+    red[quarter][2][wave] = s_sm;
   }
   __syncthreads();
   if (threadIdx.x < 3) {
-    const float t = (red[threadIdx.x][0] + red[threadIdx.x][1]) +
-                    (red[threadIdx.x][2] + red[threadIdx.x][3]);
-    const float sc = threadIdx.x == 0 ? inv_ns * lambda_eik
-                                      : (threadIdx.x == 1 ? inv_nr * lambda_sp : inv_3nr * lambda_sm);
-    if (t != 0.0f) atomicAdd(&terms[threadIdx.x], t * sc);
+    const float sc = tid == 0 ? inv_ns * lambda_eik
+                              : (tid == 1 ? inv_nr * lambda_sp : inv_3nr * lambda_sm);
+    for (int qb = 0; qb < (int)(blockDim.x >> 8); ++qb) {
+      const float t = (red[qb][tid][0] + red[qb][tid][1]) + (red[qb][tid][2] + red[qb][tid][3]);
+      if (t != 0.0f) atomicAdd(&terms[tid], t * sc);
+    }
+  }
+}
+
+__global__ __launch_bounds__(256) void sample_losses_kernel(
+    const float* __restrict__ sdf, const float* __restrict__ grad, int64_t n_s, int64_t n_r,
+    float lambda_eik, float lambda_sp, float sp_scale, float lambda_sm, int accumulate_prefix,
+    float* __restrict__ d_sdf, float* __restrict__ d_grad, float* __restrict__ terms) {
+  sample_losses_body(blockIdx.x, gridDim.x, sdf, grad, n_s, n_r, lambda_eik, lambda_sp, sp_scale,
+                     lambda_sm, accumulate_prefix, d_sdf, d_grad, terms);
+}
+
+__global__ __launch_bounds__(RL_THREADS) void ray_sample_losses_kernel(
+    const float* __restrict__ comp, const float* __restrict__ rgb, const float* __restrict__ normal,
+    const float* __restrict__ maskf, const float* __restrict__ cosines,
+    const float* __restrict__ vw, int R, int P, dsu_ray_loss_cfg cfg, float* __restrict__ terms,
+    float* __restrict__ d_comp,
+    const float* __restrict__ sdf, const float* __restrict__ grad, int64_t n_s, int64_t n_r,
+    float lambda_eik, float lambda_sp, float sp_scale, float lambda_sm,
+    float* __restrict__ d_sdf, float* __restrict__ d_grad, float* __restrict__ sample_terms,
+    int sample_blocks) {
+  extern __shared__ __attribute__((aligned(16))) unsigned char smem[];
+  if (blockIdx.x < 3) {
+    ray_losses_body(blockIdx.x, smem, comp, rgb, normal, maskf, cosines, vw, R, P, cfg, terms, d_comp);
+  } else {
+    sample_losses_body(((int64_t)blockIdx.x - 3) * 4 + (threadIdx.x >> 8), sample_blocks, sdf, grad, n_s, n_r, lambda_eik,
+                       lambda_sp, sp_scale, lambda_sm, SL_STORE_FIRST, d_sdf, d_grad, sample_terms);
   }
 }
 
@@ -545,6 +687,35 @@
   return DSU_OK;
 }
 
+int dsu_ray_losses_with_samples(const float* comp, const float* rgb, const float* normal,
+                                const float* mask, const float* cosines, const float* view_weights,
+                                int32_t n_rays, const dsu_ray_loss_cfg* cfg, float* terms, float* d_comp,
+                                const float* sdf_all, const float* grad_all, int64_t n_samples,
+                                int64_t n_random, float lambda_eikonal, float lambda_sparsity,
+                                float sparsity_scale, float lambda_smooth, int32_t terms_zeroed,
+                                float* d_sdf_all, float* d_grad_all, float* sample_terms, void* stream) {
+  if (!cfg || !terms || n_rays < 0 || n_samples < 0 || n_random < 0 || !sample_terms) return DSU_EINVAL;
+  if (n_rays && (!comp || !rgb || !normal || !mask || !cosines || !view_weights || !d_comp))
+    return DSU_EINVAL;
+  if (n_rays > DSU_RAY_LOSS_MAX_RAYS) return DSU_EUNSUP;
+  const int64_t n = n_samples + n_random;
+  if (n && (!sdf_all || !grad_all || !d_sdf_all || !d_grad_all)) return DSU_EINVAL;
+  hipStream_t s = (hipStream_t)stream;
+  if (!terms_zeroed && hipMemsetAsync(sample_terms, 0, 3 * sizeof(float), s) != hipSuccess)
+    return DSU_ELAUNCH;
+  int P = RL_THREADS;
+  while (P < n_rays) P <<= 1;
+  const size_t shm = (size_t)P * 16 + 256;
+  const int sample_blocks = n ? dsu_capped_blocks(n, 256, 512) : 0;
+  DSU_ENSURE_DYN_LDS(ray_sample_losses_kernel, shm);
+  ray_sample_losses_kernel<<<3 + (sample_blocks + 3) / 4, RL_THREADS, shm, s>>>(
+      comp, rgb, normal, mask, cosines, view_weights, n_rays, P, *cfg, terms, d_comp, sdf_all, grad_all,
+      n_samples, n_random, lambda_eikonal, lambda_sparsity, sparsity_scale, lambda_smooth, d_sdf_all,
+      d_grad_all, sample_terms, sample_blocks);
+  DSU_CHECK_LAUNCH();
+  return DSU_OK;
+}
+
 int dsu_sample_losses(const float* sdf_all, const float* grad_all, int64_t n_samples,
                       int64_t n_random, float lambda_eikonal, float lambda_sparsity,
                       float sparsity_scale, float lambda_smooth, int32_t accumulate_prefix,
diff --git a/drawingspinup_amd/csrc/texture_mlp.hip b/drawingspinup_amd/csrc/texture_mlp.hip
--- a/drawingspinup_amd/csrc/texture_mlp.hip
+++ b/drawingspinup_amd/csrc/texture_mlp.hip
@@ -336,6 +336,7 @@
   return (int64_t)(((uint64_t)hi << 32) | lo);
 }
 
+template <bool ACC = false>
 __device__ __forceinline__ void shade_grad_out(const ShadeIn& sh, const ShadeOut& so, int64_t si,
                                                float d0, float d1, float d2) {
   const float g0 = sh.grad[si * 3], g1 = sh.grad[si * 3 + 1], g2 = sh.grad[si * 3 + 2];
@@ -347,18 +348,28 @@
   }
   const float dot = n0 * d0 + n1 * d1 + n2 * d2;
   const bool ok = len > 1e-12f;
-  so.d_grad[si * 3] = ok ? (d0 - n0 * dot) * inv : d0 * inv;
-  so.d_grad[si * 3 + 1] = ok ? (d1 - n1 * dot) * inv : d1 * inv;
-  so.d_grad[si * 3 + 2] = ok ? (d2 - n2 * dot) * inv : d2 * inv;
-}
-
-template <bool SHADE>
+  const float o0 = ok ? (d0 - n0 * dot) * inv : d0 * inv;
+  const float o1 = ok ? (d1 - n1 * dot) * inv : d1 * inv;
+  const float o2 = ok ? (d2 - n2 * dot) * inv : d2 * inv;
+  if (ACC) {
+    const float p0 = so.d_grad[si * 3], p1 = so.d_grad[si * 3 + 1], p2 = so.d_grad[si * 3 + 2];
+    so.d_grad[si * 3] = p0 + o0;
+    so.d_grad[si * 3 + 1] = p1 + o1;
+    so.d_grad[si * 3 + 2] = p2 + o2;
+  } else {
+    so.d_grad[si * 3] = o0;
+    so.d_grad[si * 3 + 1] = o1;
+    so.d_grad[si * 3 + 2] = o2;
+  }
+}
+
+template <bool SHADE, bool ACC = false>
 __device__ __forceinline__ void dead_sample_out(const ShadeIn& sh, const ShadeOut& so, float* __restrict__ d_x,
                                                 int64_t i) {
   if (SHADE) {
 #pragma unroll
     for (int k = 0; k < 13; ++k) so.d_feature[i * 13 + k] = 0.0f;
-    shade_grad_out(sh, so, i, 0.0f, 0.0f, 0.0f);
+    shade_grad_out<ACC>(sh, so, i, 0.0f, 0.0f, 0.0f);
   } else {
 #pragma unroll
     for (int q = 0; q < 4; ++q)
@@ -382,9 +393,9 @@
   if (threadIdx.x == 0) live_halves[blockIdx.x] = word;
 }
 
-template <bool SHADE, bool L1_MASK = false>
-__global__ __launch_bounds__(256) void texture_bwd_kernel(
-    dsu_tex_mlp m, const float* __restrict__ x, ShadeIn sh, ShadeOut so,
+template <bool SHADE, bool L1_MASK, bool ACC>
+__device__ __forceinline__ void texture_bwd_body(
+    const dsu_tex_mlp& m, const float* __restrict__ x, const ShadeIn& sh, const ShadeOut& so,
     const float* __restrict__ rgb, const float* __restrict__ d_rgb, int64_t n,
     float* __restrict__ d_x, float* __restrict__ partials,
     const uint32_t* __restrict__ h1_mask, const uint32_t* __restrict__ live_halves) {
@@ -477,7 +488,7 @@
   if (scanned) {
     for (int64_t t = blockIdx.x * (int64_t)blockDim.x + threadIdx.x; t < n; t += (int64_t)gridDim.x * blockDim.x) {
       const int64_t hf = t >> 5;
-      if (!((sbits[hf >> 5] >> (hf & 31)) & 1u)) dead_sample_out<SHADE>(sh, so, d_x, t);
+      if (!((sbits[hf >> 5] >> (hf & 31)) & 1u)) dead_sample_out<SHADE, ACC>(sh, so, d_x, t);
     }
   }
   int64_t wh0, wh1;
@@ -513,7 +524,7 @@
       const uint64_t lit = __ballot(valid && (dr[0] != 0.0f || dr[1] != 0.0f || dr[2] != 0.0f));
       live0 = (uint32_t)lit != 0u;
       live1 = (uint32_t)(lit >> 32) != 0u;
-      if (valid && !(h ? live1 : live0)) dead_sample_out<SHADE>(sh, so, d_x, i);
+      if (valid && !(h ? live1 : live0)) dead_sample_out<SHADE, ACC>(sh, so, d_x, i);
       if (lit == 0ull) continue;
     }
     float in[TIN];
@@ -675,7 +686,7 @@
               const int comp = 8 * q + 4 * h + e;
               if (comp < 13) so.d_feature[si * 13 + comp] = din[4 * q + e];
             }
-          if (h == 1) shade_grad_out(sh, so, si, din[5], din[6], din[7]);
+          if (h == 1) shade_grad_out<ACC>(sh, so, si, din[5], din[6], din[7]);
         } else {
 #pragma unroll
           for (int q = 0; q < 2; ++q)
@@ -718,6 +729,23 @@
   float* part = partials + (size_t)blockIdx.x * PART_STRIDE;
   for (int v = threadIdx.x; v < PART_N; v += blockDim.x)
     part[v] = (lds[v] + lds[PART_STRIDE + v]) + (lds[2 * PART_STRIDE + v] + lds[3 * PART_STRIDE + v]);
+}
+
+template <bool SHADE, bool L1_MASK = false>
+__global__ __launch_bounds__(256) void texture_bwd_kernel(
+    dsu_tex_mlp m, const float* __restrict__ x, ShadeIn sh, ShadeOut so,
+    const float* __restrict__ rgb, const float* __restrict__ d_rgb, int64_t n,
+    float* __restrict__ d_x, float* __restrict__ partials,
+    const uint32_t* __restrict__ h1_mask, const uint32_t* __restrict__ live_halves) {
+  texture_bwd_body<SHADE, L1_MASK, false>(m, x, sh, so, rgb, d_rgb, n, d_x, partials, h1_mask, live_halves);
+}
+
+__global__ __launch_bounds__(256) void texture_bwd_add_kernel(
+    dsu_tex_mlp m, ShadeIn sh, ShadeOut so, const float* __restrict__ rgb,
+    const float* __restrict__ d_rgb, int64_t n, float* __restrict__ partials,
+    const uint32_t* __restrict__ h1_mask, const uint32_t* __restrict__ live_halves) {
+  texture_bwd_body<true, true, true>(m, nullptr, sh, so, rgb, d_rgb, n, nullptr, partials, h1_mask,
+                                     live_halves);
 }
 
 __global__ void texture_reduce_kernel(const float* __restrict__ partials, int nblocks,
@@ -759,7 +787,7 @@
   return m && m->w0 && m->b0 && m->w1 && m->b1 && m->w2 && m->b2;
 }
 
-template <bool SHADE, bool L1_MASK>
+template <bool SHADE, bool L1_MASK, bool ACC = false>
 int launch_bwd(const dsu_tex_mlp* mlp, const float* x, ShadeIn sh, ShadeOut so, const float* rgb,
                const float* d_rgb, int64_t n, float* d_x, const uint32_t* h1_mask, const uint32_t* live,
                void* workspace, int64_t workspace_bytes, hipStream_t s, int* blocks) {
@@ -775,9 +803,16 @@
     live = own;
   }
   const size_t shm = (size_t)BWD_LDS_ALL_F * sizeof(float);
-  DSU_ENSURE_DYN_LDS((texture_bwd_kernel<SHADE, L1_MASK>), shm);
-  texture_bwd_kernel<SHADE, L1_MASK><<<*blocks, 256, shm, s>>>(*mlp, x, sh, so, rgb, d_rgb, n, d_x,
-                                                              (float*)workspace, h1_mask, live);
+  if constexpr (ACC) {
+    static_assert(SHADE && L1_MASK, "the adding kernel is the NSR step's");
+    DSU_ENSURE_DYN_LDS(texture_bwd_add_kernel, shm);
+    texture_bwd_add_kernel<<<*blocks, 256, shm, s>>>(*mlp, sh, so, rgb, d_rgb, n, (float*)workspace,
+                                                     h1_mask, live);
+  } else {
+    DSU_ENSURE_DYN_LDS((texture_bwd_kernel<SHADE, L1_MASK>), shm);
+    texture_bwd_kernel<SHADE, L1_MASK><<<*blocks, 256, shm, s>>>(*mlp, x, sh, so, rgb, d_rgb, n, d_x,
+                                                                (float*)workspace, h1_mask, live);
+  }
   return DSU_OK;
 }
 
@@ -888,15 +923,19 @@
                            const float* rgb, const float* d_rgb, const float* d_normal,
                            int64_t n, int64_t tail_rows, float* d_grad, float* d_feature,
                            const uint32_t* h1_mask, const uint32_t* live, void* workspace,
-                           int64_t workspace_bytes, dsu_partial_reduce* red, void* stream) {
+                           int64_t workspace_bytes, dsu_partial_reduce* red, void* stream,
+                           bool acc = false) {
   if (!mlp_ok(mlp) || n < 0 || !red) return DSU_EINVAL;
+  if (acc && (!h1_mask || !live)) return DSU_EINVAL;
   if (tail_rows < 0 || (n && (!feature || !grad || !rgb || !d_rgb || !d_grad || !d_feature)))
     return DSU_EINVAL;
   if (n == 0) return DSU_EUNSUP;
   const ShadeIn sh{feature, grad};
   const ShadeOut so{d_normal, d_grad, d_feature, tail_rows};
   int blocks;
-  const int rc = h1_mask ? launch_bwd<true, true>(mlp, nullptr, sh, so, rgb, d_rgb, n, nullptr, h1_mask, live,
+  const int rc = acc     ? launch_bwd<true, true, true>(mlp, nullptr, sh, so, rgb, d_rgb, n, nullptr, h1_mask, live,
+                                                        workspace, workspace_bytes, (hipStream_t)stream, &blocks)
+                 : h1_mask ? launch_bwd<true, true>(mlp, nullptr, sh, so, rgb, d_rgb, n, nullptr, h1_mask, live,
                                                   workspace, workspace_bytes, (hipStream_t)stream, &blocks)
                          : launch_bwd<true, false>(mlp, nullptr, sh, so, rgb, d_rgb, n, nullptr, nullptr, live,
                                                    workspace, workspace_bytes, (hipStream_t)stream, &blocks);
@@ -920,6 +959,17 @@
                          live_halves, workspace, workspace_bytes, red, stream);
 }
 
+int dsu_texture_bwd_shaded_partials_live_acc(const dsu_tex_mlp* mlp, const float* feature, const float* grad,
+                                             const float* rgb, const float* d_rgb, const float* d_normal,
+                                             int64_t n, int64_t tail_rows, float* d_grad, float* d_feature,
+                                             const uint32_t* h1_mask, const uint32_t* live_halves,
+                                             void* workspace, int64_t workspace_bytes,
+                                             dsu_partial_reduce* red, void* stream) {
+  if (!live_halves || !h1_mask) return DSU_EINVAL;
+  return shaded_partials(mlp, feature, grad, rgb, d_rgb, d_normal, n, tail_rows, d_grad, d_feature, h1_mask,
+                         live_halves, workspace, workspace_bytes, red, stream, true);
+}
+
 int dsu_texture_bwd_shaded_partials_m(const dsu_tex_mlp* mlp, const float* feature, const float* grad,
                                       const float* rgb, const float* d_rgb, const float* d_normal,
                                       int64_t n, int64_t tail_rows, float* d_grad, float* d_feature,
diff --git a/drawingspinup_amd/ops.py b/drawingspinup_amd/ops.py
--- a/drawingspinup_amd/ops.py
+++ b/drawingspinup_amd/ops.py
@@ -564,6 +564,32 @@
     return terms, d_sdf_all, d_grad_all
 
 
+def ray_losses_with_samples(comp, rgb, normal, mask, cosines, view_weights, cfg, sdf_all, grad_all,
+                            n_samples, n_random, lambda_eikonal, lambda_sparsity, sparsity_scale,
+                            lambda_smooth):
+    from ._lib import RayLossCfg
+    comp = _f32c(comp)
+    r = comp.shape[0]
+    c = RayLossCfg(float(cfg["rgb_p_ratio"]), float(cfg["normal_p_ratio"]),
+                   float(cfg["mask_p_ratio"]), float(cfg["lambda_rgb_mse"]),
+                   float(cfg["lambda_rgb_l1"]), float(cfg["lambda_normal"]),
+                   float(cfg["lambda_mask"]), int(bool(cfg["geo_aware"])), 0)
+    sdf_all, grad_all = _f32c(sdf_all), _f32c(grad_all)
+    assert sdf_all.shape[0] == n_samples + 2 * n_random
+    terms = torch.empty(4, dtype=torch.float32, device=comp.device)
+    d_comp = torch.empty_like(comp)
+    sterms = torch.empty(3, dtype=torch.float32, device=comp.device)
+    d_sdf_all = torch.empty_like(sdf_all)
+    d_grad_all = torch.empty_like(grad_all)
+    check(lib().dsu_ray_losses_with_samples(
+        ptr(comp), ptr(_f32c(rgb)), ptr(_f32c(normal)), ptr(_f32c(mask)), ptr(_f32c(cosines)),
+        ptr(_f32c(view_weights)), r, C.byref(c), ptr(terms), ptr(d_comp), ptr(sdf_all), ptr(grad_all),
+        n_samples, n_random, float(lambda_eikonal), float(lambda_sparsity), float(sparsity_scale),
+        float(lambda_smooth), 0, ptr(d_sdf_all, torch.float32), ptr(d_grad_all, torch.float32),
+        ptr(sterms), stream()), "dsu_ray_losses_with_samples")
+    return terms, d_comp, sterms, d_sdf_all, d_grad_all
+
+
 def weights_from_alpha_fwd(alpha, offsets, counts):
     alpha = _f32c(alpha)
     w = torch.empty_like(alpha)
@@ -1168,6 +1194,50 @@
                                             stream()),
           "dsu_neus_composite_bwd_live")
     return d_sdf, d_normal, d_rgb, d_inv, live
+
+
+def neus_composite_bwd_live_acc(sdf, normal, rgb, rays_d, t_starts, t_ends, offsets, counts, inv_s, car,
+                                alpha, weights, d_comp, d_sdf_all):
+    n, n_rays = sdf.shape[0], rays_d.shape[0]
+    dev = sdf.device
+    assert d_sdf_all.dtype == torch.float32 and d_sdf_all.is_contiguous() and d_sdf_all.shape[0] >= n
+    d_normal = torch.empty((n, 3), dtype=torch.float32, device=dev)
+    d_rgb = torch.empty((n, 3), dtype=torch.float32, device=dev)
+    d_inv = torch.zeros(1, dtype=torch.float32, device=dev)
+    live = torch.zeros((n + 1023) // 1024, dtype=torch.int32, device=dev)
+    check(lib().dsu_neus_composite_bwd_live_acc(ptr(_f32c(sdf)), ptr(_f32c(normal)), ptr(_f32c(rgb)),
+                                                ptr(_f32c(rays_d)), ptr(_f32c(t_starts)),
+                                                ptr(_f32c(t_ends)), ptr(offsets, torch.int32),
+                                                ptr(counts, torch.int32), n_rays,
+                                                ptr(inv_s, torch.float32), float(car), ptr(alpha),
+                                                ptr(weights), ptr(_f32c(d_comp)), None, ptr(d_sdf_all),
+                                                ptr(d_normal), ptr(d_rgb), ptr(d_inv),
+                                                ptr(live, torch.int32), stream()),
+          "dsu_neus_composite_bwd_live_acc")
+    return d_normal, d_rgb, d_inv, live
+
+
+def texture_bwd_shaded_partials_live(params, feature, grad, rgb, d_rgb, d_normal, tail_rows, h1_mask, live,
+                                     d_grad_all=None):
+    from ._lib import PartialReduce
+    feature, grad, rgb, d_rgb = _f32c(feature), _f32c(grad), _f32c(rgb), _f32c(d_rgb)
+    n = rgb.shape[0]
+    dev = rgb.device
+    acc = d_grad_all is not None
+    if acc:
+        assert d_grad_all.dtype == torch.float32 and d_grad_all.is_contiguous() and d_grad_all.shape[0] >= n
+    d_grad = d_grad_all if acc else torch.empty((n, 3), dtype=torch.float32, device=dev)
+    d_feat = torch.empty((n + tail_rows, 13), dtype=torch.float32, device=dev)
+    wbytes = int(lib().dsu_texture_bwd_workspace_bytes(n))
+    ws = torch.empty(max(wbytes, 4) // 4, dtype=torch.float32, device=dev)
+    m = _tex_struct(params)
+    rec = PartialReduce()
+    fn = lib().dsu_texture_bwd_shaded_partials_live_acc if acc else lib().dsu_texture_bwd_shaded_partials_live
+    dn = None if d_normal is None else _f32c(d_normal)
+    check(fn(C.byref(m), ptr(feature), ptr(grad), ptr(rgb), ptr(d_rgb), ptr(dn), n,
+             int(tail_rows), ptr(d_grad), ptr(d_feat), ptr(h1_mask, torch.int32), ptr(live, torch.int32),
+             ptr(ws), wbytes, C.byref(rec), stream()), "dsu_texture_bwd_shaded_partials_live")
+    return d_grad, d_feat, DeferredSum(rec, (ws,))
 
 
 def texture_live_partition(live_words, n_halves, parts, waves=4):
diff --git a/include/dsu_hip.h b/include/dsu_hip.h
--- a/include/dsu_hip.h
+++ b/include/dsu_hip.h
@@ -187,6 +187,13 @@
                                 const float* weights, const float* d_comp, const float* d_weights,
                                 float* d_sdf, float* d_normal, float* d_rgb, float* d_inv_s,
                                 uint32_t* live_halves, void* stream);
+int dsu_neus_composite_bwd_live_acc(const float* sdf, const float* normal, const float* rgb,
+                                    const float* rays_d, const float* t_starts, const float* t_ends,
+                                    const int32_t* offsets, const int32_t* counts, int64_t n_rays,
+                                    const float* inv_s, float cos_anneal_ratio, const float* alpha,
+                                    const float* weights, const float* d_comp, const float* d_weights,
+                                    float* d_sdf, float* d_normal, float* d_rgb, float* d_inv_s,
+                                    uint32_t* live_halves, void* stream);
 int dsu_shade_prep_fwd(const float* grad, const float* feature, int64_t n, float* normal,
                        float* tex_in, void* stream);
 int dsu_shade_prep_bwd(const float* grad, const float* d_normal, const float* d_tex_in, int64_t n,
@@ -223,6 +230,12 @@
                                          const uint32_t* h1_mask, const uint32_t* live_halves,
                                          void* workspace, int64_t workspace_bytes,
                                          dsu_partial_reduce* red, void* stream);
+int dsu_texture_bwd_shaded_partials_live_acc(const dsu_tex_mlp* mlp, const float* feature, const float* grad,
+                                             const float* rgb, const float* d_rgb, const float* d_normal,
+                                             int64_t n, int64_t tail_rows, float* d_grad, float* d_feature,
+                                             const uint32_t* h1_mask, const uint32_t* live_halves,
+                                             void* workspace, int64_t workspace_bytes,
+                                             dsu_partial_reduce* red, void* stream);
 int dsu_texture_live_partition(const uint32_t* live_halves, int64_t n_halves, int32_t parts,
                                int32_t waves, int32_t* runs);
 
@@ -255,6 +268,14 @@
                       int64_t n_random, float lambda_eikonal, float lambda_sparsity,
                       float sparsity_scale, float lambda_smooth, int32_t accumulate_prefix,
                       float* d_sdf_all, float* d_grad_all, float* terms, void* stream);
+
+int dsu_ray_losses_with_samples(const float* comp, const float* rgb, const float* normal,
+                                const float* mask, const float* cosines, const float* view_weights,
+                                int32_t n_rays, const dsu_ray_loss_cfg* cfg, float* terms, float* d_comp,
+                                const float* sdf_all, const float* grad_all, int64_t n_samples,
+                                int64_t n_random, float lambda_eikonal, float lambda_sparsity,
+                                float sparsity_scale, float lambda_smooth, int32_t terms_zeroed,
+                                float* d_sdf_all, float* d_grad_all, float* sample_terms, void* stream);
 
 
 int dsu_ric_offsets(int32_t H, int32_t W, float* offsets, void* stream);
```

Measured after the change: 0.3737. 0.976x the previous value.
